# immunogenomics/cna

Measured on AMD Instinct MI355X. Metric: cells*permutations/sec end-to-end cna.tl.association, higher is better.
Workload: dtype f64

## Files before the change

cna_amd/_ffi.py:

```python
import ctypes as C
import os

_HERE = os.path.dirname(os.path.abspath(__file__))
LIB_PATH = os.path.join(_HERE, 'libcna_hip.so')

c_ctx = C.c_void_p
c_i64p = C.POINTER(C.c_int64)
c_i32p = C.POINTER(C.c_int32)
c_f64p = C.POINTER(C.c_double)
c_u8p = C.POINTER(C.c_uint8)

SIGNATURES = {
    'cna_last_error': (C.c_char_p, []),
    'cna_abi_version': (C.c_int, []),
    'cna_device_count': (C.c_int, [C.POINTER(C.c_int)]),
    'cna_ctx_create': (C.c_int, [C.c_int, C.POINTER(c_ctx)]),
    'cna_ctx_destroy': (C.c_int, [c_ctx]),
    'cna_ctx_sync': (C.c_int, [c_ctx]),
    'cna_ctx_device_bytes': (C.c_int, [c_ctx, c_i64p]),
    'cna_set_state_f32': (C.c_int, [c_ctx, C.c_int]),
    'cna_comm_unique_id': (C.c_int, [C.c_void_p]),
    'cna_comm_init': (C.c_int, [c_ctx, C.c_int, C.c_int, C.c_void_p]),
    'cna_graph_upload': (C.c_int, [c_ctx, C.c_int64, C.c_int64, C.c_int64, C.c_void_p, C.c_void_p,
                                   C.c_void_p, C.c_int]),
    'cna_comm_info': (C.c_int, [c_ctx, C.POINTER(C.c_int), C.POINTER(C.c_int)]),
    'cna_comm_selftest': (C.c_int, [c_ctx, C.c_double, C.POINTER(C.c_int)]),
    'cna_comm_init_shm': (C.c_int, [c_ctx, C.c_int, C.c_int, C.c_char_p, C.c_int64]),
    'cna_set_halo': (C.c_int, [c_ctx, C.c_void_p, C.c_void_p, C.c_void_p, C.c_void_p]),
    'cna_set_cell_order': (C.c_int, [c_ctx, C.c_void_p]),
    'cna_graph_reorder': (C.c_int, [c_ctx, C.c_void_p]),
    'cna_set_local_view': (C.c_int, [c_ctx, C.c_int]),
    'cna_colsums': (C.c_int, [c_ctx, C.c_double]),
    'cna_fetch_colsums': (C.c_int, [c_ctx, C.c_void_p]),
    'cna_set_samples': (C.c_int, [c_ctx, C.c_void_p, C.c_int, C.c_void_p]),
    'cna_restart_nam': (C.c_int, [c_ctx]),
    'cna_nam_step': (C.c_int, [c_ctx, C.c_int, C.c_int, C.c_int]),
    'cna_nam_select_hint': (C.c_int, [c_ctx, C.c_void_p, C.c_int]),
    'cna_nam_auto': (C.c_int, [c_ctx, C.c_int, C.POINTER(C.c_int), C.c_void_p]),
    'cna_nam_auto_launch': (C.c_int, [c_ctx, C.c_int]),
    'cna_nam_auto_finish': (C.c_int, [c_ctx, C.POINTER(C.c_int), C.c_void_p]),
    'cna_stat_qc': (C.c_int, [c_ctx, c_f64p, c_f64p, c_i64p]),
    'cna_fetch_cell_stat': (C.c_int, [c_ctx, C.c_void_p, C.c_int64]),
    'cna_load_cell_stat': (C.c_int, [c_ctx, C.c_void_p, C.c_int64]),
    'cna_dense_load': (C.c_int, [c_ctx, C.c_void_p, C.c_int]),
    'cna_dense_step': (C.c_int, [c_ctx]),
    'cna_dense_fetch': (C.c_int, [c_ctx, C.c_void_p]),
    'cna_batch_kurtosis': (C.c_int, [c_ctx, C.c_int, C.c_void_p, C.c_int]),
    'cna_zero_variance': (C.c_int, [c_ctx, C.c_void_p, C.c_int, C.c_void_p, c_i64p]),
    'cna_select': (C.c_int, [c_ctx, C.c_void_p, C.c_int64, C.c_void_p, C.c_int]),
    'cna_set_resid_factors': (C.c_int, [c_ctx, C.c_void_p, C.c_void_p, C.c_int, C.c_int]),
    'cna_select_checked': (C.c_int, [c_ctx, C.c_void_p, C.c_int64, C.c_void_p, C.c_int, C.POINTER(C.c_int64)]),
    'cna_select_standardized': (C.c_int, [c_ctx, C.c_void_p, C.c_int64, C.c_void_p, C.c_int, C.POINTER(C.c_int64),
                                          C.c_void_p, C.POINTER(C.c_double)]),
    'cna_upload_x': (C.c_int, [c_ctx, C.c_void_p, C.c_int64, C.c_int]),
    'cna_resid_apply': (C.c_int, [c_ctx, C.c_void_p, C.c_int]),
    'cna_resid_lowrank': (C.c_int, [c_ctx, C.c_void_p, C.c_void_p, C.c_int, C.c_int, C.c_int, C.c_void_p, c_f64p]),
    'cna_resid_lowrank_bk': (C.c_int, [c_ctx, C.c_void_p, C.c_void_p, C.c_int, C.c_void_p, c_f64p, C.c_void_p, C.c_int, c_f64p]),
    'cna_select_resid_bk': (C.c_int, [c_ctx, C.c_void_p, C.c_void_p, C.c_int, C.c_void_p, c_f64p, C.c_void_p, C.c_int, c_f64p,
                                      c_i64p, c_i64p, C.POINTER(C.c_int)]),
    'cna_standardize': (C.c_int, [c_ctx, C.c_int]),
    'cna_gram': (C.c_int, [c_ctx, C.c_void_p]),
    'cna_gram_launch': (C.c_int, [c_ctx]),
    'cna_gram_fetch': (C.c_int, [c_ctx, C.c_void_p]),
    'cna_project': (C.c_int, [c_ctx, C.c_void_p, C.c_int, C.c_void_p]),
    'cna_x_identity': (C.c_int, [c_ctx, C.POINTER(C.c_int)]),
    'cna_ncorrs': (C.c_int, [c_ctx, C.c_void_p, C.c_void_p, c_f64p]),
    'cna_null_local': (C.c_int, [c_ctx, C.c_void_p, C.c_int, C.c_void_p, C.c_int, C.c_void_p]),
    'cna_condition_phenotypes': (C.c_int, [c_ctx, C.c_void_p, C.c_void_p, C.c_int, C.c_int]),
    'cna_null_local_resident': (C.c_int, [c_ctx, C.c_int, C.c_int, C.c_void_p, C.c_int, C.c_void_p, C.c_void_p]),
    'cna_null_local_launch': (C.c_int, [c_ctx, C.c_int, C.c_int, C.c_void_p, C.c_int, C.c_int, C.c_void_p]),
    'cna_null_local_prepare': (C.c_int, [c_ctx, C.c_int, C.c_void_p, C.c_int, C.c_int, C.c_void_p]),
    'cna_null_local_fetch': (C.c_int, [c_ctx, C.c_void_p, C.c_void_p, C.c_void_p, C.c_void_p]),
    'cna_null_local_discard': (C.c_int, [c_ctx]),
    'cna_gram_pcs_tests': (C.c_int, [c_ctx, C.c_int, C.c_void_p, C.c_int, C.c_int, C.c_int, C.c_double, C.c_double, C.c_void_p,
                                     C.c_void_p, C.POINTER(C.c_int)]),
    'cna_host_top_eig': (C.c_int, [C.c_void_p, C.c_int, C.c_int, C.c_void_p, C.c_void_p, c_f64p, c_f64p]),
    'cna_host_eig_check': (C.c_int, [C.c_void_p, C.c_int, C.c_int, C.c_void_p, C.c_void_p, c_f64p, c_f64p]),
    'cna_null_local_i8_stats': (C.c_int, [c_ctx, C.POINTER(C.c_int), c_i64p, C.POINTER(C.c_int)]),
    'cna_percell_fdr_pinned': (C.c_int, [c_ctx, C.c_void_p, C.c_void_p, C.c_int, C.POINTER(C.c_void_p), C.POINTER(C.c_void_p)]),
    'cna_nam_steps': (C.c_int, [c_ctx, C.c_int]),
    'cna_host_legacy_randn': (C.c_int, [C.c_void_p, C.POINTER(C.c_int), C.POINTER(C.c_int), C.POINTER(C.c_double), C.c_int64, C.c_void_p]),
    'cna_knn_graph': (C.c_int, [c_ctx, C.c_void_p, C.c_int64, C.c_int, C.c_int, C.c_void_p, C.c_void_p, C.c_void_p, c_i64p]),
    'cna_host_hash64': (C.c_uint64, [C.c_void_p, C.c_int64, C.c_int]),
    'cna_host_copy': (C.c_int, [C.c_void_p, C.c_void_p, C.c_int64, C.c_int]),
    'cna_host_expand_u16': (C.c_int, [C.c_void_p, C.c_void_p, C.c_int64, C.c_void_p, C.c_int, C.c_int]),
    'cna_host_permuted_nnz': (C.c_int64, [C.c_void_p, C.c_int64, C.c_int64, C.c_void_p]),
    'cna_host_permute_rows': (C.c_int, [C.c_void_p, C.c_int64, C.c_int64, C.c_void_p, C.c_void_p, C.c_void_p, C.c_int, C.c_void_p,
                                        C.c_void_p, C.c_void_p, C.c_void_p, C.c_int]),
    'cna_host_cluster_order': (C.c_int64, [C.c_int64, C.c_void_p, C.c_void_p, C.c_int, C.c_void_p]),
    'cna_host_cluster_order_mt': (C.c_int64, [C.c_int64, C.c_void_p, C.c_void_p, C.c_int, C.c_int, C.c_void_p]),
    'cna_host_cluster_graph': (C.c_int64, [C.c_int64, C.c_void_p, C.c_void_p, C.c_void_p, C.c_int, C.c_void_p, C.c_void_p, C.c_void_p]),
    'cna_host_set_threads': (None, [C.c_int]),
    'cna_host_argsort_gather': (C.c_int, [C.c_void_p, C.c_int, C.c_int, C.c_void_p, C.c_void_p, C.c_int64, C.c_void_p]),
    'cna_host_draw_start': (C.c_int, [C.c_void_p, C.POINTER(C.c_int), C.c_void_p, C.c_int, C.c_int, C.c_int, C.c_void_p,
                                      C.c_void_p, C.c_void_p, C.c_int64, C.c_int]),
    'cna_host_draw_start_idx': (C.c_int, [C.c_void_p, C.POINTER(C.c_int), C.c_void_p, C.c_int, C.c_int, C.c_int, C.c_void_p,
                                          C.c_void_p, C.c_void_p, C.c_int64, C.c_int, C.c_void_p]),
    'cna_host_gather_rows': (C.c_int, [C.c_void_p, C.c_void_p, C.c_int, C.c_int, C.c_void_p, C.c_int64, C.c_int]),
    'cna_host_draw_wait': (C.c_int, []),
    'cna_host_draw_join': (C.c_int, []),
    'cna_host_draw_times': (None, [C.POINTER(C.c_double)]),
    'cna_assoc_begin': (C.c_int, [c_ctx, C.c_int, C.c_void_p, C.c_int]),
    'cna_assoc_begin_part': (C.c_int, [c_ctx, C.c_int, C.c_int, C.c_int, C.c_void_p, C.c_int]),
    'cna_assoc_finish': (C.c_int, [c_ctx, C.c_void_p, C.c_void_p]),
    'cna_assoc_run': (C.c_int, [c_ctx, C.c_int, C.c_void_p, C.c_int, C.c_void_p, C.c_void_p]),
    'cna_host_draw_then_condition': (C.c_int, [c_ctx, C.c_void_p, C.c_void_p, C.c_int, C.c_int, C.c_void_p]),
    'cna_global_test_launch': (C.c_int, [c_ctx, C.c_void_p, C.c_int, C.c_void_p, C.c_int, C.c_int]),
    'cna_global_test_fetch': (C.c_int, [c_ctx, C.c_void_p, C.c_void_p, C.c_void_p]),
    'cna_select_standardized_fused': (C.c_int, [c_ctx, C.c_void_p, C.c_int64, C.c_void_p, C.c_int, C.POINTER(C.c_int64), C.c_void_p, C.POINTER(C.c_double), C.c_int, C.POINTER(C.c_int), C.c_void_p, C.POINTER(C.c_int), C.POINTER(C.c_int), C.c_int, C.c_void_p, C.POINTER(C.c_int)]),
    'cna_reference_thresholds': (C.c_int, [C.c_double, C.c_int, C.c_void_p, C.c_void_p]),
    'cna_percell_coef_launch': (C.c_int, [c_ctx]),
    'cna_percell_coef_wait': (C.c_int, [c_ctx, C.POINTER(C.c_void_p)]),
    'cna_percell_fdr_copy_early': (C.c_int, [c_ctx, C.c_void_p, C.c_int64, C.c_int, C.POINTER(C.c_int)]),
    'cna_percell_fdr_copied_early': (C.c_int, [c_ctx, C.POINTER(C.c_int)]),
    'cna_fetch_rows': (C.c_int, [c_ctx, C.c_int, C.c_void_p, C.c_int64, C.c_void_p, C.c_int, C.c_void_p, C.c_int]),
    'cna_project_keep': (C.c_int, [c_ctx, C.c_void_p, C.c_int]),
    'cna_stat_median': (C.c_int, [c_ctx, C.POINTER(C.c_double)]),
    'cna_global_test': (C.c_int, [c_ctx, C.c_void_p, C.c_int, C.c_void_p, C.c_int, C.c_int, C.c_void_p, C.c_void_p,
                                  C.c_void_p]),
    'cna_obs_counts': (C.c_int, [c_ctx, C.c_void_p, C.c_void_p, C.c_int, C.c_void_p, C.c_void_p]),
    'cna_percell_fdr': (C.c_int, [c_ctx, C.c_void_p, C.c_void_p, C.c_int, C.c_void_p, C.c_void_p]),
    'cna_matrix_shape': (C.c_int, [c_ctx, C.c_int, c_i64p, C.POINTER(C.c_int)]),
    'cna_fetch_matrix': (C.c_int, [c_ctx, C.c_int, C.c_void_p, C.c_int]),
    'cna_allgather_host': (C.c_int, [c_ctx, C.c_void_p, C.c_int64, C.c_void_p, C.c_int64]),
    'cna_prof_enable': (C.c_int, [c_ctx, C.c_int]),
    'cna_prof_reset': (C.c_int, [c_ctx]),
    'cna_prof_get': (C.c_int, [c_ctx, C.c_int, c_f64p, c_i64p]),
    'cna_kernel_name': (C.c_char_p, [C.c_int]),
    'cna_expr_upload_dense': (C.c_int, [c_ctx, C.c_void_p, C.c_int64, C.c_int64, C.c_int]),
    'cna_expr_upload_sparse': (C.c_int, [c_ctx, C.c_void_p, C.c_void_p, C.c_void_p, C.c_int64, C.c_int64, C.c_int64,
                                         C.c_int, C.c_int, C.c_int]),
    'cna_expr_drop': (C.c_int, [c_ctx]),
    'cna_expr_shape': (C.c_int, [c_ctx, c_i64p, c_i64p, c_i64p, C.POINTER(C.c_int), C.POINTER(C.c_int), c_i64p]),
    'cna_gene_corr': (C.c_int, [c_ctx, C.c_void_p, C.c_int, C.c_void_p]),
    'cna_expr_to_bins': (C.c_int, [c_ctx, C.c_void_p, C.c_int, C.c_int, C.c_void_p, C.c_void_p]),
    'cna_expr_cross': (C.c_int, [c_ctx, C.c_void_p, C.c_int64, C.c_void_p, C.c_void_p, C.c_void_p, C.c_void_p,
                                 C.POINTER(C.c_int64)]),
    'cna_coef_strata': (C.c_int, [c_ctx, C.c_void_p, C.c_void_p, C.c_void_p, C.c_int64, C.c_int, C.c_int, C.c_int, C.c_double,
                                  C.c_double] + [C.c_void_p] * 10),
    'cna_gene_corr_by': (C.c_int, [c_ctx, C.c_void_p, C.c_int, C.c_void_p, C.c_int, C.c_void_p, C.c_void_p, C.c_void_p]),
    'cna_x_generation': (C.c_int, [c_ctx, C.POINTER(C.c_int64)]),
    'cna_matrix_to_bins': (C.c_int, [c_ctx, C.c_int, C.c_void_p, C.c_void_p, C.c_int, C.c_int64, C.c_int, C.c_void_p, C.c_void_p]),
    'cna_enrichment_extremes': (C.c_int, [c_ctx, C.c_void_p, C.c_int64, C.c_int64, C.c_void_p, C.c_void_p, C.c_int, C.c_int,
                                          C.c_void_p, C.c_void_p, C.c_void_p, C.c_void_p]),
    'cna_expr_cross_by': (C.c_int, [c_ctx, C.c_void_p, C.c_void_p, C.c_int64, C.c_int, C.c_int, C.c_int, C.c_void_p, C.c_void_p,
                                    C.c_void_p, C.c_void_p]),
    'cna_gram_by': (C.c_int, [c_ctx, C.c_void_p, C.c_void_p, C.c_int64, C.c_int, C.c_void_p, C.c_void_p]),
}

MAT_NAM, MAT_X, MAT_PROJ = 0, 1, 2
ASSOC_DONE, ASSOC_GENERAL, ASSOC_NEED_PCS, ASSOC_STALE = 0, 1, 2, 3
ASSOC_MAXT = 512


class AssocArgs(C.Structure):
    _fields_ = [('colmap', C.c_void_p), ('n_sel', C.c_int32), ('r', C.c_int32), ('y', C.c_void_p), ('M', C.c_void_p),
                ('resid_C', C.c_void_p), ('resid_W', C.c_void_p), ('ks', C.c_void_p), ('K', C.c_int32), ('Nnull', C.c_int32),
                ('table', C.c_void_p), ('draw_pending', C.c_int32), ('conditioned', C.c_int32), ('use_native_eig', C.c_int32),
                ('coef_first', C.c_int32), ('resid_tol', C.c_double), ('gap_tol', C.c_double), ('coef_dst', C.c_void_p),
                ('fdr_dst', C.c_void_p), ('n_dst', C.c_int64), ('copy_threads', C.c_int32), ('n_verify', C.c_int32),
                ('verify_ptr', C.c_void_p * 4), ('verify_bytes', C.c_int64 * 4), ('verify_hash', C.c_uint64 * 4),
                ('verify_threads', C.c_int32), ('reserved', C.c_int32),
                ('G', C.c_void_p), ('U', C.c_void_p), ('minp', C.c_void_p), ('r2', C.c_void_p), ('kidx', C.c_void_p)]


class AssocOut(C.Structure):
    _fields_ = [('status', C.c_int32), ('T', C.c_int32), ('eig_accepted', C.c_int32), ('null_fused', C.c_int32),
                ('coef_in_dst', C.c_int32), ('fdr_in_dst', C.c_int32), ('n_zero', C.c_int64), ('max_abs', C.c_double),
                ('coef_ptr', C.c_void_p), ('fdr_ptr', C.c_void_p), ('t_ms', C.c_double * 16),
                ('thr', C.c_double * ASSOC_MAXT), ('fdr', C.c_double * ASSOC_MAXT), ('runmin', C.c_double * ASSOC_MAXT),
                ('tail_sums', C.c_int64 * ASSOC_MAXT), ('ranks', C.c_int64 * ASSOC_MAXT), ('num_detected', C.c_int64 * ASSOC_MAXT)]

KERNELS = ['colsum', 'nam_first', 'nam_step', 'batch_kurtosis', 'zero_variance', 'select', 'resid_xb',
           'standardize', 'gram', 'gram_reduce', 'ncorrs', 'null_local', 'obs_counts', 'percell_fdr',
           'project_xb', 'transpose', 'rccl', 'condition', 'global_test', 'nam_step_sparse', 'halo_exchange', 'halo_wait',
           'matrix_bins_sort', 'matrix_bins_sum', 'enrich_positions', 'enrich_extremes', 'expr_cross_by', 'gram_by']

_lib = None


class CnaHipError(RuntimeError):
    """A libcna_hip.so entry point returned a non-zero status."""


def load():
    global _lib
    if _lib is not None:
        return _lib
    if not os.path.exists(LIB_PATH):
        raise CnaHipError(
            'libcna_hip.so is not built (%s).  cna_amd has no CPU path; build the HIP library with '
            '`python -c "import __graft_entry__ as g; g.build()"` or `make -C cna_amd/csrc`.' % LIB_PATH)
    lib = C.CDLL(LIB_PATH)
    for name, (res, args) in SIGNATURES.items():
        fn = getattr(lib, name)
        fn.restype = res
        fn.argtypes = args
    _lib = lib
    return lib


def check(status, what):
    if status != 0:
        msg = load().cna_last_error()
        raise CnaHipError('%s failed (status %d): %s' % (what, status, msg.decode() if msg else '?'))


def ptr(a):
    return None if a is None else a.ctypes.data_as(C.c_void_p)
```

cna_amd/csrc/c_api.hip:

```cpp
#include "common.h"
#include <sched.h>
#include <chrono>
#include <cmath>
#include <cstring>

int comm_destroy(cna_ctx* c);

static thread_local std::string g_err;
void cna_set_error(const std::string& msg) { g_err = msg; }

int dev_alloc(cna_ctx* c, void** p, size_t bytes) {
  std::lock_guard<std::recursive_mutex> lk(c->alloc_mu);
  *p = nullptr;
  if (bytes == 0) bytes = 256;
  hipError_t e = hipMalloc(p, bytes);
  if (e != hipSuccess) {
    cna_set_error(std::string("hipMalloc(") + std::to_string(bytes) + "): " + hipGetErrorString(e));
    return CNA_ENOMEM;
  }
  c->dev_bytes += (int64_t)bytes;
  return 0;
}
int dev_free(cna_ctx* c, void* p, size_t bytes) {
  std::lock_guard<std::recursive_mutex> lk(c->alloc_mu);
  if (p) {
    (void)hipFree(p);
    c->dev_bytes -= (int64_t)(bytes ? bytes : 256);
  }
  return 0;
}
static void halo_clear(cna_ctx* c);

int dev_reserve(cna_ctx* c, void** p, int64_t* cap, int64_t need) {
  std::lock_guard<std::recursive_mutex> lk(c->alloc_mu);
  if (need <= *cap && *p) return 0;
  if (*p) {
    HIP_TRY(hipStreamSynchronize(c->stream));
    dev_free(c, *p, (size_t)*cap);
    *p = nullptr;
    *cap = 0;
  }
  if (need < 256) need = 256;
  CNA_TRY(dev_alloc(c, p, (size_t)need));
  *cap = need;
  return 0;
}

static hipEvent_t ev_get(cna_ctx* c) {
  if (!c->ev_pool.empty()) {
    hipEvent_t e = c->ev_pool.back();
    c->ev_pool.pop_back();
    return e;
  }
  hipEvent_t e;
  (void)hipEventCreate(&e);
  return e;
}
void prof_begin(cna_ctx* c, int kid, hipStream_t st) {
  std::lock_guard<std::mutex> lock(c->prof_mu);
  ProfSpan s;
  s.kid = kid;
  s.a = ev_get(c);
  s.b = ev_get(c);
  (void)hipEventRecord(s.a, st);
  c->prof_pending.push_back(s);
}
void prof_end(cna_ctx* c, int kid, hipStream_t st) {
  std::lock_guard<std::mutex> lock(c->prof_mu);
  for (size_t i = c->prof_pending.size(); i-- > 0;) {
    if (c->prof_pending[i].kid == kid) {
      (void)hipEventRecord(c->prof_pending[i].b, st);
      return;
    }
  }
}
static void prof_flush(cna_ctx* c) {
  (void)hipStreamSynchronize(c->stream);
  (void)hipStreamSynchronize(c->copy_stream);
  if (c->coef_stream) (void)hipStreamSynchronize(c->coef_stream);
  if (c->gram_stream) (void)hipStreamSynchronize(c->gram_stream);
  if (c->halo_stream) (void)hipStreamSynchronize(c->halo_stream);
  std::lock_guard<std::mutex> lock(c->prof_mu);
  if (c->prof_pending.empty()) return;
  for (auto& s : c->prof_pending) {
    float ms = 0.f;
    if (hipEventElapsedTime(&ms, s.a, s.b) == hipSuccess) {
      c->prof_ms[s.kid] += ms;
      c->prof_n[s.kid] += 1;
    }
    c->ev_pool.push_back(s.a);
    c->ev_pool.push_back(s.b);
  }
  c->prof_pending.clear();
}

static const char* kKernelNames[CNA_K_COUNT] = {
    "colsum", "nam_first", "nam_step", "batch_kurtosis", "zero_variance", "select", "resid_xb",
    "standardize", "gram", "gram_reduce", "ncorrs", "null_local", "obs_counts", "percell_fdr",
    "project_xb", "transpose", "rccl", "condition", "global_test", "nam_step_sparse", "halo_exchange", "halo_wait",
    "matrix_bins_sort", "matrix_bins_sum", "enrich_positions", "enrich_extremes", "expr_cross_by", "gram_by"};

#define AUTO_FINISH(c)                                                   \
  do {                                                                   \
    if ((c)->auto_pending) CNA_TRY(cna_nam_auto_finish((c), nullptr, nullptr)); \
  } while (0)

static void void_x(cna_ctx* c) {
  c->x_valid = c->x_from_nam = c->x_ident = false;
  c->ncorrs_valid = c->xq_valid = c->byp_valid = c->gram_pre = c->proj_valid = false;
  c->gram_n = 0;
  c->cells.coef_early = false;
  c->cells.fdr_inline = false;
  c->x_gen = c->x_gen + 1;
}
static void void_walk(cna_ctx* c) {
  c->t_valid = c->nam_valid = c->nam_lazy = false;
  c->steps_done = 0;
  c->t_f32[0] = c->t_f32[1] = false;
  void_x(c);
}
static void void_cells(cna_ctx* c) {
  c->cellinfo_valid = false;
  void_walk(c);
}

static int x_begin(cna_ctx* c, const char* who) {
  NO_NULL_PENDING(c, who);
  void_x(c);
  return 0;
}
int x_ld(int Nx) {
  int ld = round_up(Nx, 4);
  if (ld > 128 && (ld * 8) % 256 == 0 && ld + 4 <= 256) ld += 4;
  return ld;
}
static int x_begin(cna_ctx* c, const char* who, int64_t nx, int Nx, const int64_t* keep_idx) {
  CNA_TRY(x_begin(c, who));
  c->nx = nx;
  c->Nx = Nx;
  c->ldx = x_ld(Nx);
  void* xp = c->X;
  CNA_TRY(dev_reserve(c, &xp, &c->x_cap, (int64_t)sizeof(double) * std::max<int64_t>(nx, 1) * c->ldx));
  c->X = (double*)xp;
  c->keep_idx = nullptr;
  if (keep_idx) {
    void* kp = c->keep_store;
    CNA_TRY(dev_reserve(c, &kp, &c->keep_cap, 8 * std::max<int64_t>(nx, 1)));
    c->keep_store = (int64_t*)kp;
    HIP_TRY(hipMemcpyAsync(c->keep_store, keep_idx, 8 * nx, hipMemcpyHostToDevice, c->stream));
    c->keep_idx = c->keep_store;
  }
  return 0;
}
static void x_commit(cna_ctx* c, bool from_nam, bool ncorrs, bool xq, bool ident) {
  c->x_valid = true;
  c->x_from_nam = from_nam;
  c->ncorrs_valid = ncorrs;
  c->xq_valid = xq;
  c->x_ident = ident;
}


static int ragged_gather(cna_ctx* c, const double* src_dev, int64_t count_local, double* out, int64_t n_expected) {
  NO_NULL_PENDING(c, "cna_fetch_cell_stat / cna_allgather_host");
  CNA_TRY(dev_reserve(c, &c->scratch, &c->scratch_cap, 256 * 2 + 8 * c->nranks));
  int64_t* cnt_dev = (int64_t*)c->scratch;
  std::vector<int64_t> cnt(c->nranks, 0);
  cnt[c->rank] = count_local;
  HIP_TRY(hipMemcpyAsync(cnt_dev, cnt.data(), 8 * c->nranks, hipMemcpyHostToDevice, c->stream));
  CNA_TRY(comm_allreduce_i64_sum(c, cnt_dev, c->nranks));
  HIP_TRY(hipMemcpyAsync(cnt.data(), cnt_dev, 8 * c->nranks, hipMemcpyDeviceToHost, c->stream));
  HIP_TRY(hipStreamSynchronize(c->stream));
  int64_t mx = 1, tot = 0;
  for (auto v : cnt) { mx = std::max(mx, v); tot += v; }
  if (tot != n_expected) CNA_FAIL(CNA_EINVAL, "ragged gather: expected total does not match the ranks' counts");
  CNA_TRY(dev_reserve(c, &c->scratch2, &c->scratch2_cap, 8 * mx * c->nranks));
  double* all = (double*)c->scratch2;
  if (count_local > 0)
    HIP_TRY(hipMemcpyAsync(all + mx * c->rank, src_dev, 8 * count_local, hipMemcpyDeviceToDevice, c->stream));
  CNA_TRY(comm_allgather_bytes(c, all + mx * c->rank, all, 8 * mx));
  std::vector<double> host(mx * c->nranks);
  HIP_TRY(hipMemcpyAsync(host.data(), all, 8 * mx * c->nranks, hipMemcpyDeviceToHost, c->stream));
  HIP_TRY(hipStreamSynchronize(c->stream));
  int64_t o = 0;
  for (int r = 0; r < c->nranks; ++r) {
    std::memcpy(out + o, host.data() + mx * r, 8 * cnt[r]);
    o += cnt[r];
  }
  return 0;
}

int halo_settle(cna_ctx* c) {
  if (!c->halo_wait_pending) return 0;
  c->halo_wait_pending = false;
  ProfScope ps(c, CNA_K_HALO_WAIT);
  HIP_TRY(hipStreamWaitEvent(c->stream, c->halo_e2, 0));
  return 0;
}

extern "C" {

const char* cna_last_error(void) { return g_err.c_str(); }
int cna_abi_version(void) { return 1; }
const char* cna_kernel_name(int k) { return (k >= 0 && k < CNA_K_COUNT) ? kKernelNames[k] : "?"; }

int cna_device_count(int* count) {
  int n = 0;
  hipError_t e = hipGetDeviceCount(&n);
  if (e != hipSuccess) {
    *count = 0;
    cna_set_error(std::string("hipGetDeviceCount: ") + hipGetErrorString(e));
    return (int)e;
  }
  *count = n;
  return 0;
}

int cna_ctx_create(int device, cna_ctx** out) {
  if (!out) CNA_FAIL(CNA_EINVAL, "null out pointer");
  *out = nullptr;
  int n = 0;
  CNA_TRY(cna_device_count(&n));
  if (n <= 0) CNA_FAIL(CNA_EINVAL, "no HIP device visible: cna_amd has no CPU fallback");
  if (device < 0 || device >= n) CNA_FAIL(CNA_EINVAL, "device index out of range");
  HIP_TRY(hipSetDevice(device));
  cna_ctx* c = new cna_ctx();
  c->device = device;
  hipError_t e = hipStreamCreateWithFlags(&c->stream, hipStreamNonBlocking);
  if (e == hipSuccess) {
    int lo = 0, hi = 0;
    (void)hipDeviceGetStreamPriorityRange(&lo, &hi);
    e = hipStreamCreateWithPriority(&c->copy_stream, hipStreamNonBlocking, hi);
    if (e == hipSuccess) e = hipStreamCreateWithFlags(&c->coef_stream, hipStreamNonBlocking);
  }
  if (e == hipSuccess) e = hipEventCreateWithFlags(&c->gram_done, hipEventDisableTiming);
  if (e == hipSuccess) e = hipEventCreateWithFlags(&c->cells.coef_ready, hipEventDisableTiming);
  if (e == hipSuccess) e = hipEventCreateWithFlags(&c->gt_done, hipEventDisableTiming);
  if (e == hipSuccess) e = hipEventCreateWithFlags(&c->scal_ready, hipEventDisableTiming);
  if (e == hipSuccess) e = hipEventCreateWithFlags(&c->stage_done, hipEventDisableTiming);
  if (e == hipSuccess) e = hipEventCreateWithFlags(&c->cells.coef_copied, hipEventDisableTiming);
  if (e == hipSuccess) e = hipEventCreateWithFlags(&c->null_done, hipEventDisableTiming);
  if (e == hipSuccess) e = hipEventCreateWithFlags(&c->cells.bins_copied, hipEventDisableTiming);
  if (e != hipSuccess) {
    delete c;
    cna_set_error(std::string("hipStreamCreate: ") + hipGetErrorString(e));
    return (int)e;
  }
  *out = c;
  return 0;
}

int cna_ctx_destroy(cna_ctx* c) {
  if (!c) return 0;
  (void)hipSetDevice(c->device);
  (void)hipStreamSynchronize(c->stream);
  if (c->gram_stream) (void)hipStreamSynchronize(c->gram_stream);
  if (c->auto_state) { (void)hipFree(c->auto_state); c->auto_state = nullptr; }
  if (c->byp_buf) { (void)hipFree(c->byp_buf); c->byp_buf = nullptr; }
  if (c->pair_buf) { (void)hipFree(c->pair_buf); c->pair_buf = nullptr; }
  prof_flush(c);
  comm_destroy(c);
  expr_destroy(c);
  void* bufs[] = {c->halo_rows_safe, c->halo_rows_need, c->idx_t, c->i8_buf, c->xq, c->xq_scale, c->cells.coef_dev, c->proj, c->sp_pair, c->sp_cnt, c->null_part, c->rp16_buf, c->halo_send_idx, c->halo_recv_idx, c->halo_rows_b, c->halo_rows_i, c->halo_sbuf, c->halo_rbuf, c->orig_idx, c->indptr, c->indices, c->data, c->colsum, c->sid, c->counts, c->T[0], c->T[1], c->dense_s,
                  c->nam, c->X, c->X2, c->resid_f, c->keep_store, c->stat, c->ncorrs, c->scratch, c->scratch2, c->cellinfo, c->zc, c->gt, c->gram_tiles_ptr, c->gram_buf, c->gram_part, c->cells.bins_dev};
  for (void* b : bufs)
    if (b) (void)hipFree(b);
  for (auto e : c->ev_pool) (void)hipEventDestroy(e);
  (void)hipStreamDestroy(c->stream);
  if (c->copy_stream) (void)hipStreamDestroy(c->copy_stream);
  if (c->coef_stream) (void)hipStreamDestroy(c->coef_stream);
  if (c->gram_done) (void)hipEventDestroy(c->gram_done);
  if (c->gt_done) (void)hipEventDestroy(c->gt_done);
  if (c->scal_ready) (void)hipEventDestroy(c->scal_ready);
  if (c->stage_done) (void)hipEventDestroy(c->stage_done);
  if (c->h_gt) (void)hipHostFree(c->h_gt);
  if (c->null_done) (void)hipEventDestroy(c->null_done);
  if (c->gram_stream) (void)hipStreamDestroy(c->gram_stream);
  for (hipEvent_t e : {c->gram_pre_done, c->range_done, c->cells.coef_ready, c->cells.coef_copied, c->cells.bins_copied})
    if (e) (void)hipEventDestroy(e);
  if (c->halo_stream) (void)hipStreamDestroy(c->halo_stream);
  if (c->halo_e1) (void)hipEventDestroy(c->halo_e1);
  if (c->halo_e2) (void)hipEventDestroy(c->halo_e2);
  if (c->cells.h_bins) (void)hipHostFree(c->cells.h_bins);
  if (c->cells.h_tab) (void)hipHostFree(c->cells.h_tab);
  if (c->h_res) (void)hipHostFree(c->h_res);
  if (c->h_scal) (void)hipHostFree(c->h_scal);
  if (c->h_gram) (void)hipHostFree(c->h_gram);
  if (c->h_hint) (void)hipHostFree(c->h_hint);
  if (c->cells.h_cell) (void)hipHostFree(c->cells.h_cell);
  delete c;
  return 0;
}

int cna_ctx_sync(cna_ctx* c) {
  CHECK_CTX(c);
  AUTO_FINISH(c);
  CNA_TRY(halo_settle(c));
  HIP_TRY(hipStreamSynchronize(c->stream));
  if (c->gram_stream && c->gram_pre_pending) HIP_TRY(hipStreamSynchronize(c->gram_stream));
  return 0;
}

int cna_ctx_device_bytes(cna_ctx* c, int64_t* bytes) {
  if (!c || !bytes) CNA_FAIL(CNA_EINVAL, "null argument");
  *bytes = c->dev_bytes.load();
  return 0;
}

int cna_x_generation(cna_ctx* c, int64_t* gen) {
  if (!c || !gen) CNA_FAIL(CNA_EINVAL, "null argument");
  *gen = c->x_gen;
  return 0;
}

int cna_set_state_f32(cna_ctx* c, int on) {
  CHECK_CTX(c);
  c->state_f32_mode = on != 0;
  return 0;
}

int cna_graph_upload(cna_ctx* c, int64_t n_global, int64_t row0, int64_t n_local, const int64_t* indptr,
                     const int32_t* indices, const void* data, int data_is_f64) {
  CHECK_CTX(c);
  AUTO_FINISH(c);
  if (n_global <= 0 || n_local < 0 || row0 < 0 || row0 + n_local > n_global || !indptr)
    CNA_FAIL(CNA_EINVAL, "cna_graph_upload: bad shape");
  const int64_t rpr = (n_global + c->nranks - 1) / c->nranks;
  if (row0 != (int64_t)c->rank * rpr && !(n_local == 0))
    CNA_FAIL(CNA_EINVAL, "cna_graph_upload: row0 must be rank*ceil(n/nranks)");
  const int64_t want_local = std::max<int64_t>(0, std::min(rpr, n_global - (int64_t)c->rank * rpr));
  if (n_local != want_local) CNA_FAIL(CNA_EINVAL, "cna_graph_upload: n_local must be the rank's block size");
  if (indptr[0] != 0) CNA_FAIL(CNA_EINVAL, "cna_graph_upload: indptr must be rebased to start at 0");
  const int64_t nnz = indptr[n_local];
  HIP_TRY(hipStreamSynchronize(c->stream));
  void_cells(c);
  if (c->indptr) dev_free(c, c->indptr, sizeof(int64_t) * (c->n_local + 1));
  if (c->indices) dev_free(c, c->indices, sizeof(int32_t) * c->nnz);
  if (c->data) dev_free(c, c->data, (c->data_f64 ? 8 : 4) * c->nnz);
  if (c->colsum) dev_free(c, c->colsum, sizeof(double) * c->n_pad);
  if (c->stat) dev_free(c, c->stat, sizeof(double) * c->n_pad);
  if (c->orig_idx) dev_free(c, c->orig_idx, sizeof(int64_t) * c->n_local);
  c->indptr = nullptr; c->indices = nullptr; c->data = nullptr; c->colsum = nullptr; c->stat = nullptr;
  c->orig_idx = nullptr;
  halo_clear(c);
  c->n_global = n_global;
  c->row0 = (int64_t)c->rank * rpr;
  c->n_local = n_local;
  c->rows_per_rank = rpr;
  c->n_pad = rpr * c->nranks;
  c->nnz = nnz;
  c->data_f64 = data_is_f64 ? 1 : 0;
  const size_t vb = data_is_f64 ? 8 : 4;
  CNA_TRY(dev_alloc(c, (void**)&c->indptr, sizeof(int64_t) * (n_local + 1)));
  CNA_TRY(dev_alloc(c, (void**)&c->indices, sizeof(int32_t) * nnz));
  CNA_TRY(dev_alloc(c, (void**)&c->data, vb * nnz));
  CNA_TRY(dev_alloc(c, (void**)&c->colsum, sizeof(double) * c->n_pad));
  CNA_TRY(dev_alloc(c, (void**)&c->stat, sizeof(double) * c->n_pad));
  HIP_TRY(hipMemcpy(c->indptr, indptr, sizeof(int64_t) * (n_local + 1), hipMemcpyHostToDevice));
  if (nnz > 0) {
    HIP_TRY(hipMemcpy(c->indices, indices, sizeof(int32_t) * nnz, hipMemcpyHostToDevice));
    HIP_TRY(hipMemcpy(c->data, data, vb * nnz, hipMemcpyHostToDevice));
  }
  HIP_TRY(hipMemset(c->stat, 0, sizeof(double) * c->n_pad));
  c->have_colsum = false;
  return 0;
}

int cna_set_cell_order(cna_ctx* c, const int64_t* orig_index) {
  CHECK_CTX(c);
  if (!c->indptr) CNA_FAIL(CNA_ESTATE, "cna_set_cell_order before cna_graph_upload");
  HIP_TRY(hipStreamSynchronize(c->stream));
  if (!orig_index) {
    if (c->orig_idx) dev_free(c, c->orig_idx, sizeof(int64_t) * c->n_local);
    c->orig_idx = nullptr;
    return 0;
  }
  const int64_t lim = c->local_view ? c->n_local : c->n_global;
  for (int64_t i = 0; i < c->n_local; ++i)
    if (orig_index[i] < 0 || orig_index[i] >= lim)
      CNA_FAIL(CNA_EINVAL, "cna_set_cell_order: index out of range");
  if (!c->orig_idx && c->n_local > 0) CNA_TRY(dev_alloc(c, (void**)&c->orig_idx, sizeof(int64_t) * c->n_local));
  if (c->n_local > 0)
    HIP_TRY(hipMemcpy(c->orig_idx, orig_index, sizeof(int64_t) * c->n_local, hipMemcpyHostToDevice));
  return 0;
}

int cna_graph_reorder(cna_ctx* c, const int64_t* perm) {
  CHECK_CTX(c);
  AUTO_FINISH(c);
  if (!c->indptr || !perm) CNA_FAIL(CNA_ESTATE, "cna_graph_reorder before cna_graph_upload");
  if (c->nranks != 1 || c->halo_on || c->local_view || c->n_local != c->n_global || c->n_pad != c->n_global)
    CNA_FAIL(CNA_ESTATE, "cna_graph_reorder: one rank holding the whole graph only");
  if (c->orig_idx) CNA_FAIL(CNA_ESTATE, "cna_graph_reorder: the resident graph already has a device cell order");
  CNA_TRY(halo_settle(c));
  HIP_TRY(hipStreamSynchronize(c->stream));
  if (c->gram_stream && c->gram_pre_pending) HIP_TRY(hipStreamSynchronize(c->gram_stream));
  const int64_t n = c->n_global;
  int64_t* pd = nullptr;
  CNA_TRY(dev_alloc(c, (void**)&pd, sizeof(int64_t) * n));
  hipError_t e = hipMemcpyAsync(pd, perm, sizeof(int64_t) * n, hipMemcpyHostToDevice, c->stream);
  int rc = e == hipSuccess ? graph_reorder_device(c, pd) : (int)e;
  if (rc) {
    (void)hipStreamSynchronize(c->stream);
    dev_free(c, pd, sizeof(int64_t) * n);
    if (e != hipSuccess) cna_set_error(hipGetErrorString(e));
    return rc;
  }
  c->orig_idx = pd;
  HIP_TRY(hipMemsetAsync(c->stat, 0, sizeof(double) * c->n_pad, c->stream));
  void_cells(c);
  return 0;
}

int cna_set_local_view(cna_ctx* c, int on) {
  CHECK_CTX(c);
  HIP_TRY(hipStreamSynchronize(c->stream));
  if ((on != 0) != c->local_view) {
    void_x(c);
    if (c->orig_idx) dev_free(c, c->orig_idx, sizeof(int64_t) * c->n_local);
    c->orig_idx = nullptr;
  }
  c->local_view = on != 0;
  return 0;
}

int cna_colsums(cna_ctx* c, double self_weight) {
  CHECK_CTX(c);
  if (!c->indptr) CNA_FAIL(CNA_ESTATE, "cna_colsums before cna_graph_upload");
  c->self_weight = self_weight;
  CNA_TRY(launch_colsum(c));
  CNA_TRY(comm_allreduce_f64_sum(c, c->colsum, (size_t)c->n_pad));
  CNA_TRY(launch_add_scalar(c, c->colsum, c->n_global, self_weight));
  c->have_colsum = true;
  c->cellinfo_valid = false;
  return 0;
}

int cna_fetch_colsums(cna_ctx* c, double* out) {
  CHECK_CTX(c);
  if (!c->have_colsum) CNA_FAIL(CNA_ESTATE, "colsums not computed");
  HIP_TRY(hipMemcpyAsync(out, c->colsum, sizeof(double) * c->n_global, hipMemcpyDeviceToHost, c->stream));
  HIP_TRY(hipStreamSynchronize(c->stream));
  return 0;
}

static int64_t state_rows(const cna_ctx* c) { return c->t_compact ? c->t_rows : c->n_pad; }

static int ensure_T(cna_ctx* c, int ld) {
  const int64_t need = (int64_t)sizeof(double) * (state_rows(c) * ld + 64);
  if (need > c->t_cap || !c->T[0] || (c->t_compact && c->t_cap > need + need / 2 + (1 << 20))) {
    HIP_TRY(hipStreamSynchronize(c->stream));
    if (c->halo_wait_pending && c->halo_stream) { HIP_TRY(hipStreamSynchronize(c->halo_stream)); c->halo_wait_pending = false; }
    for (int i = 0; i < 2; ++i) {
      if (c->T[i]) dev_free(c, c->T[i], (size_t)c->t_cap);
      c->T[i] = nullptr;
    }
    for (int i = 0; i < 2; ++i) {
      CNA_TRY(dev_alloc(c, (void**)&c->T[i], (size_t)need));
      HIP_TRY(hipMemsetAsync(c->T[i], 0, (size_t)need, c->stream));
    }
    c->t_cap = need;
  }
  return 0;
}

static int ensure_sparse_state(cna_ctx* c) {
  int min_n = 96;
  if (const char* e = getenv("CNA_SPARSE_MIN_N")) min_n = atoi(e);
  const bool multi = c->nranks > 1 || comm_active(c);
  const bool want = min_n > 0 && c->N >= min_n && (!multi || c->halo_on);
  if (!want) {
    if (c->sp_cnt) {
      HIP_TRY(hipStreamSynchronize(c->stream));
      dev_free(c, c->sp_pair, 16 * 64 * (size_t)c->sp_pair_rows);
      dev_free(c, c->sp_cnt, (size_t)c->sp_rows);
      c->sp_pair = c->sp_cnt = nullptr;
      c->sp_rows = c->sp_pair_rows = 0;
    }
    return 0;
  }
  const int64_t cnt_rows = state_rows(c), pair_rows = c->t_compact ? std::max<int64_t>(c->n_local, 1) : c->n_pad;
  if (c->sp_cnt && c->sp_rows == cnt_rows && c->sp_pair_rows == pair_rows) return 0;
  if (c->sp_cnt) {
    HIP_TRY(hipStreamSynchronize(c->stream));
    dev_free(c, c->sp_pair, 16 * 64 * (size_t)c->sp_pair_rows);
    dev_free(c, c->sp_cnt, (size_t)c->sp_rows);
    c->sp_pair = c->sp_cnt = nullptr;
  }
  c->sp_rows = cnt_rows;
  c->sp_pair_rows = pair_rows;
  CNA_TRY(dev_alloc(c, &c->sp_pair, 16 * 64 * (size_t)c->sp_pair_rows));
  CNA_TRY(dev_alloc(c, &c->sp_cnt, (size_t)c->sp_rows));
  HIP_TRY(hipMemsetAsync(c->sp_cnt, 0xff, (size_t)c->sp_rows, c->stream));
  return 0;
}

int cna_set_samples(cna_ctx* c, const int32_t* codes, int n_samples, const double* counts) {
  CHECK_CTX(c);
  AUTO_FINISH(c);
  if (!c->indptr) CNA_FAIL(CNA_ESTATE, "cna_set_samples before cna_graph_upload");
  if (n_samples < 1 || n_samples > 1024) CNA_FAIL(CNA_EINVAL, "n_samples must be in [1, 1024]");
  HIP_TRY(hipStreamSynchronize(c->stream));
  if (!c->sid || !c->counts || c->N != n_samples || c->sid_n != c->n_global) {
    if (c->sid) dev_free(c, c->sid, sizeof(int32_t) * c->sid_n);
    if (c->counts) dev_free(c, c->counts, sizeof(double) * c->N);
    c->sid = nullptr; c->counts = nullptr;
    CNA_TRY(dev_alloc(c, (void**)&c->sid, sizeof(int32_t) * c->n_global));
    CNA_TRY(dev_alloc(c, (void**)&c->counts, sizeof(double) * n_samples));
    c->sid_n = c->n_global;
  }
  c->N = n_samples;
  int ld_align = 4;
  c->ld = round_up(n_samples, ld_align);
  HIP_TRY(hipMemcpyAsync(c->sid, codes, sizeof(int32_t) * c->n_global, hipMemcpyHostToDevice, c->stream));
  HIP_TRY(hipMemcpyAsync(c->counts, counts, sizeof(double) * n_samples, hipMemcpyHostToDevice, c->stream));
  HIP_TRY(hipStreamSynchronize(c->stream));
  void_cells(c);
  CNA_TRY(ensure_T(c, c->ld));
  void* nm = c->nam;
  CNA_TRY(dev_reserve(c, &nm, &c->nam_cap, (int64_t)sizeof(double) * std::max<int64_t>(c->n_local, 1) * c->ld));
  c->nam = (double*)nm;
  c->t_width = c->N;
  c->t_ld = c->ld;
  c->t_cur = 0;
  CNA_TRY(ensure_sparse_state(c));
  return 0;
}

int cna_restart_nam(cna_ctx* c) {
  CHECK_CTX(c);
  AUTO_FINISH(c);
  if (!c->sid || !c->counts) CNA_FAIL(CNA_ESTATE, "cna_restart_nam needs cna_set_samples first");
  void_walk(c);
  CNA_TRY(ensure_T(c, c->ld));
  c->t_width = c->N;
  c->t_ld = c->ld;
  c->t_cur = 0;
  return 0;
}

static void halo_clear(cna_ctx* c) {
  if (c->halo_wait_pending && c->halo_stream) (void)hipStreamSynchronize(c->halo_stream);
  c->halo_wait_pending = false;
  if (c->halo_rows_safe) dev_free(c, c->halo_rows_safe, sizeof(int32_t) * std::max<int64_t>(c->halo_nsafe, 1));
  if (c->halo_rows_need) dev_free(c, c->halo_rows_need, sizeof(int32_t) * std::max<int64_t>(c->halo_nneed, 1));
  c->halo_rows_safe = c->halo_rows_need = nullptr;
  c->halo_nsafe = c->halo_nneed = 0;
  if (c->idx_t) dev_free(c, c->idx_t, sizeof(int32_t) * std::max<int64_t>(c->idx_t_n, 1));
  c->idx_t = nullptr;
  c->idx_t_n = 0;
  if (c->t_compact) {
    c->t_compact = false;
    c->t_rows = 0;
    void_cells(c);
  }
  if (c->halo_send_idx) dev_free(c, c->halo_send_idx, sizeof(int64_t) * std::max<int64_t>(c->halo_ns, 1));
  if (c->halo_recv_idx) dev_free(c, c->halo_recv_idx, sizeof(int64_t) * std::max<int64_t>(c->halo_nr, 1));
  c->halo_send_idx = c->halo_recv_idx = nullptr;
  c->halo_ns = c->halo_nr = 0;
  c->halo_on = false;
  if (c->halo_rows_b) dev_free(c, c->halo_rows_b, sizeof(int32_t) * std::max<int64_t>(c->halo_nb, 1));
  if (c->halo_rows_i) dev_free(c, c->halo_rows_i, sizeof(int32_t) * std::max<int64_t>(c->halo_ni, 1));
  c->halo_rows_b = c->halo_rows_i = nullptr;
  c->halo_nb = c->halo_ni = 0;
}

int cna_set_halo(cna_ctx* c, const int64_t* send_rows, const int64_t* send_counts, const int64_t* recv_rows,
                 const int64_t* recv_counts) {
  CHECK_CTX(c);
  if (!c->indptr) CNA_FAIL(CNA_ESTATE, "cna_set_halo before cna_graph_upload");
  HIP_TRY(hipStreamSynchronize(c->stream));
  halo_clear(c);
  if (!send_counts || !recv_counts) return 0;
  if (!comm_active(c)) CNA_FAIL(CNA_ESTATE, "cna_set_halo needs cna_comm_init");
  int64_t ns = 0, nr = 0;
  for (int p = 0; p < c->nranks; ++p) {
    if (send_counts[p] < 0 || recv_counts[p] < 0) CNA_FAIL(CNA_EINVAL, "cna_set_halo: negative count");
    ns += send_counts[p];
    nr += recv_counts[p];
  }
  if ((ns > 0 && !send_rows) || (nr > 0 && !recv_rows)) CNA_FAIL(CNA_EINVAL, "cna_set_halo: missing row list");
  for (int64_t k = 0; k < ns; ++k)
    if (send_rows[k] < 0 || send_rows[k] >= c->n_local) CNA_FAIL(CNA_EINVAL, "cna_set_halo: send row outside the local block");
  for (int64_t k = 0; k < nr; ++k)
    if (recv_rows[k] < 0 || recv_rows[k] >= c->n_global) CNA_FAIL(CNA_EINVAL, "cna_set_halo: recv row out of range");
  CNA_TRY(dev_alloc(c, (void**)&c->halo_send_idx, sizeof(int64_t) * std::max<int64_t>(ns, 1)));
  c->halo_ns = ns;
// ... 1404 lines not shown
```

cna_amd/csrc/common.h:

```cpp
#pragma once
#include <hip/hip_runtime.h>
#include <stdint.h>
#include <string>
#include <mutex>
#include <atomic>
#include <vector>
#include "../../include/cna_hip.h"

#define WAVE 64
#define I8_QMAX 8355000.0

void cna_set_error(const std::string& msg);

#define HIP_TRY(expr)                                                                      \
  do {                                                                                     \
    hipError_t _e = (expr);                                                                \
    if (_e != hipSuccess) {                                                                \
      cna_set_error(std::string(#expr) + ": " + hipGetErrorString(_e) + " (" + __FILE__ +  \
                    ":" + std::to_string(__LINE__) + ")");                               \
      return (int)_e;                                                                      \
    }                                                                                      \
  } while (0)

#define CNA_TRY(expr)            \
  do {                           \
    int _r = (expr);             \
    if (_r != 0) return _r;      \
  } while (0)

#define CNA_FAIL(code, msg)      \
  do {                           \
    cna_set_error(msg);          \
    return (code);               \
  } while (0)

static inline int round_up(int x, int m) { return (x + m - 1) / m * m; }
static inline int64_t round_up64(int64_t x, int64_t m) { return (x + m - 1) / m * m; }

struct ProfSpan {
  int kid;
  hipEvent_t a, b;
};

struct GramPlan {
  int Nx = 0, nt = 0, ntri = 0, ldp = 0, slab_rows = 32, nblocks = 1, nw = 16;
  bool use_blk = false;
  int64_t nslab = 0;
  int32_t* tiles_dev = nullptr;
  double* partial = nullptr;
  size_t smem = 0;
};

struct NullCarve {
  double *cuts, *obs_edges, *obs_thr;
  unsigned long long *hist, *obs_hist;
  int64_t *tails, *sums, *obs_tails;
};
struct NullHostLayout { int64_t sums = 0, tails = 0, obs = 0, stage = 0, status = 0, bytes = 0; };
enum NullPhase : int { NULL_IDLE = 0, NULL_PREPARED, NULL_PENDING };
struct NullPass {
  int P = 0, T = 0, col0 = 0, has_tails = 0, has_obs = 0;
  double cut0 = 0, inv_step = 0, eps = 0;
  double thr0 = 0, thr_step = 0;
  bool i8_last = false;
  NullHostLayout host;
  std::atomic<int> phase{NULL_IDLE};
  std::atomic<int64_t> status_off{-1};
};
struct CellColumns {
  std::atomic<bool> coef_early{false};
  std::atomic<bool> fdr_inline{false};
  std::atomic<bool> fdr_early_copied{false};
  std::atomic<bool> fdr_early_served{false};
  std::atomic<int> fdr_early_inflight{0};
  double* fdr_early_dst = nullptr;
  double* coef_dev = nullptr;
  unsigned short* bins_dev = nullptr;
  unsigned short* h_bins = nullptr;
  bool bins_pending = false;
  double* h_tab = nullptr;
  void* h_cell = nullptr;
  int64_t coef_dev_cap = 0, bins_cap = 0, h_bins_cap = 0, h_cell_cap = 0;
  hipEvent_t coef_ready = nullptr, coef_copied = nullptr, bins_copied = nullptr;
};

struct cna_ctx {
  int device = 0;
  hipStream_t stream = nullptr;
  hipStream_t copy_stream = nullptr;
  hipStream_t coef_stream = nullptr;
  hipEvent_t gram_done = nullptr;
  hipEvent_t scal_ready = nullptr;
  double* gram_buf = nullptr;
  hipEvent_t null_done = nullptr;
  void* h_hint = nullptr;
  void* h_gram = nullptr;
  int64_t h_gram_cap = 0;
  double* gram_mirror = nullptr;
  bool gram_mirrored = false;
  double t_gram_fetched = 0.0;
  void* h_scal = nullptr;
  void* h_res = nullptr;
  int64_t h_res_cap = 0;
  NullPass null;
  CellColumns cells;
  int64_t gram_cap = 0;
  int gram_n = 0;
  std::atomic<int64_t> dev_bytes{0};
  std::recursive_mutex alloc_mu;

  int rank = 0, nranks = 1;
  void* comm = nullptr;
  void* comm_halo = nullptr;
  void* shm = nullptr;
  bool halo_on = false;
  int64_t* halo_send_idx = nullptr;
  int64_t* halo_recv_idx = nullptr;
  std::vector<int64_t> halo_send_cnt, halo_recv_cnt;
  int64_t halo_ns = 0, halo_nr = 0;
  int32_t* halo_rows_b = nullptr;
  int32_t* halo_rows_i = nullptr;
  int64_t halo_nb = 0, halo_ni = 0;
  hipStream_t halo_stream = nullptr;
  hipEvent_t halo_e1 = nullptr, halo_e2 = nullptr;
  void* halo_sbuf = nullptr;
  void* halo_rbuf = nullptr;
  int64_t halo_sbuf_cap = 0, halo_rbuf_cap = 0;

  int64_t n_global = 0, row0 = 0, n_local = 0, rows_per_rank = 0, n_pad = 0, nnz = 0;
  int64_t* indptr = nullptr;
  int32_t* indices = nullptr;
  void* data = nullptr;
  int data_f64 = 0;
  double self_weight = 1.0;
  double* colsum = nullptr;
  int64_t* orig_idx = nullptr;
  bool local_view = false;
  bool have_colsum = false;

  int N = 0, ld = 0;
  int32_t* sid = nullptr;
  int64_t sid_n = 0;
  double* counts = nullptr;
  void* cellinfo = nullptr;
  int64_t cellinfo_cap = 0;
  bool cellinfo_valid = false;

  bool t_compact = false;
  int64_t t_rows = 0;
  int32_t* idx_t = nullptr;
  int64_t idx_t_n = 0;
  int32_t* halo_rows_safe = nullptr;
  int32_t* halo_rows_need = nullptr;
  int64_t halo_nsafe = 0, halo_nneed = 0;
  bool halo_wait_pending = false;
  bool halo_safe_launch = false;
  bool sp_dense_interior_off = false;
  int64_t sp_pair_rows = 0;
  double* T[2] = {nullptr, nullptr};
  int64_t t_cap = 0;
  int t_cur = 0, t_width = 0, t_ld = 0, steps_done = 0;
  bool t_valid = false;
  bool state_f32_mode = false;
  bool t_f32[2] = {false, false};
  double* dense_s = nullptr;
  int64_t dense_cap = 0;

  double* nam = nullptr;
  int64_t nam_cap = 0;
  bool nam_valid = false;

  double* X = nullptr;
  int64_t x_cap = 0;
  double* resid_f = nullptr;
  int64_t resid_f_cap = 0;
  int resid_rk = 0, resid_n = 0;
  double* X2 = nullptr;
  int64_t x2_cap = 0;
  int64_t nx = 0;
  int Nx = 0, ldx = 0;
  int64_t* keep_idx = nullptr;
  int64_t* keep_store = nullptr;
  int64_t keep_cap = 0;
  bool x_valid = false, x_from_nam = false;
  int64_t x_gen = 0;
  bool x_ident = false;
  std::vector<double> byp_hint;
  std::vector<double> byp_y;
  bool byp_valid = false;
  bool byp_with_q = false;
  bool byp_skip_nam = false;
  bool nam_lazy = false;
  int lazy_steps_before = 0;
  bool byp_arm = false;
  void* pair_buf = nullptr;
  void* byp_buf = nullptr;

  double* stat = nullptr;
  int stat_space = -1;
  void* auto_state = nullptr;
  const int* auto_stop = nullptr;
  bool auto_pending = false;
  int auto_max = 0, auto_queued = 0;
  double* ncorrs = nullptr;
  int64_t ncorrs_cap = 0;
  bool ncorrs_valid = false;

  double* zc = nullptr;
  int64_t zc_cap = 0;
  int zc_ld = 0, zc_cols = 0, zc_rows = 0;
  void* gt = nullptr;
  int64_t gt_cap = 0;

  void* scratch = nullptr;
  int64_t scratch_cap = 0;
  void* proj = nullptr;
  int64_t proj_cap = 0, proj_rows = 0;
  int proj_ld = 0, proj_cols = 0;
  bool proj_valid = false;
  void* h_gt = nullptr;
  int64_t h_gt_cap = 0;
  hipEvent_t gt_done = nullptr;
  hipEvent_t stage_done = nullptr;
  int gt_pending_P = 0;
  int64_t gt_off_out = 0;
  void* sp_pair = nullptr;
  void* sp_cnt = nullptr;
  int64_t sp_rows = 0;
  void* i8_buf = nullptr;
  int64_t i8_cap = 0;
  void* xq = nullptr;
  int64_t xq_cap = 0;
  void* xq_scale = nullptr;
  int64_t xq_scale_cap = 0;
  bool xq_valid = false;
  int64_t xq_rows = 0;
  int xq_KS = 0;
  unsigned long long* i8_qcount = nullptr;
  void* null_part = nullptr;
  int64_t null_part_cap = 0;
  void* rp16_buf = nullptr;
  int64_t rp16_cap = 0;
  void* scratch2 = nullptr;
  int64_t scratch2_cap = 0;
  hipStream_t gram_stream = nullptr;
  int gram_stream_state = 0;
  hipEvent_t gram_pre_done = nullptr, range_done = nullptr;
  bool gram_pre = false;
  bool gram_pre_pending = false;
  void* gram_part = nullptr;
  int64_t gram_part_cap = 0;
  GramPlan gram_pre_plan;
  int gram_tiles_nt = -1;
  void* gram_tiles_ptr = nullptr;
  int64_t gram_tiles_cap = 0;

  void* expr = nullptr;

  bool prof = false;
  uint64_t prof_mask = ~0ull;
  double prof_ms[CNA_K_COUNT] = {0};
  int64_t prof_n[CNA_K_COUNT] = {0};
  std::vector<ProfSpan> prof_pending;
  std::vector<hipEvent_t> ev_pool;
  std::mutex prof_mu;
};

void prof_begin(cna_ctx* c, int kid, hipStream_t st);
void prof_end(cna_ctx* c, int kid, hipStream_t st);
struct ProfScope {
  cna_ctx* c;
  int kid;
  hipStream_t st;
  ProfScope(cna_ctx* c_, int k, hipStream_t s = nullptr) : c(c_), kid(k), st(s ? s : c_->stream) {
    if (c->prof && kid >= 0 && (c->prof_mask >> kid & 1)) prof_begin(c, kid, st);
  }
  ~ProfScope() { if (c->prof && kid >= 0 && (c->prof_mask >> kid & 1)) prof_end(c, kid, st); }
};

int dev_alloc(cna_ctx* c, void** p, size_t bytes);
int dev_free(cna_ctx* c, void* p, size_t bytes);
int dev_reserve(cna_ctx* c, void** p, int64_t* cap_bytes, int64_t need_bytes);

#define CHECK_CTX(c)                                        \
  do {                                                      \
    if (!(c)) CNA_FAIL(CNA_EINVAL, "null context");         \
    HIP_TRY(hipSetDevice((c)->device));                     \
  } while (0)

#define NO_NULL_PENDING(c, who)                                                                      \
  do {                                                                                               \
    if ((c)->null.phase == NULL_PENDING)                                                             \
      CNA_FAIL(CNA_ESTATE, std::string(who) + ": a local-null pass is still pending: fetch it first"); \
  } while (0)

struct Carver {
  char* base;
  int64_t off = 0;
  explicit Carver(void* p) : base((char*)p) {}
  template <typename T>
  T* take(int64_t count) {
    T* r = (T*)(base + off);
    off += round_up64((int64_t)sizeof(T) * count, 256);
    return r;
  }
};
inline int64_t carve_bytes(std::initializer_list<int64_t> sizes) {
  int64_t t = 0;
  for (auto s : sizes) t += round_up64(s, 256);
  return t;
}

int x_ld(int Nx);
int null_local_prepare(cna_ctx* c, int P, const double* edges, int T, int want_tails, const double* thr);
int null_local_go(cna_ctx* c, int col0);

void expr_destroy(cna_ctx* c);

inline bool comm_active(const cna_ctx* c) { return c->comm != nullptr || c->shm != nullptr; }
int comm_halo_exchange(cna_ctx* c, const double* sendbuf, double* recvbuf, int64_t doubles_per_row, hipStream_t st = nullptr);
int halo_settle(cna_ctx* c);
int launch_rows_need_halo(cna_ctx* c, unsigned char* flags_dev);
int launch_remap_indices(cna_ctx* c, const int64_t* recv_rows_dev, int64_t nr, int32_t* out, int* bad);
int launch_pack_rows(cna_ctx* c, const double* src, const int64_t* idx, int64_t nrows, int ld, double* dst, hipStream_t st = nullptr);
int launch_unpack_rows(cna_ctx* c, const double* src, const int64_t* idx, int64_t nrows, int ld, double* dst, hipStream_t st = nullptr);
int comm_allreduce_f64_sum(cna_ctx* c, double* buf, size_t count);
int comm_allreduce_f64_max(cna_ctx* c, double* buf, size_t count);
int comm_allreduce_i64_sum(cna_ctx* c, int64_t* buf, size_t count);
int comm_allgather_bytes(cna_ctx* c, const void* send, void* recv, size_t bytes_per_rank);

int launch_colsum(cna_ctx* c);
int graph_reorder_device(cna_ctx* c, const int64_t* perm_dev);
int launch_add_scalar(cna_ctx* c, double* v, int64_t n, double s);
int launch_nam_step(cna_ctx* c, bool first, bool want_kurt, bool write_t, bool write_nam, bool dense,
                    const int32_t* rows = nullptr, int64_t n_rows = 0,
                    int64_t base = 0, int64_t count = -1,
                    hipStream_t st = nullptr, bool timed = true);
int64_t nam_step_turn_rows(const cna_ctx* c, int64_t n_rows);
int launch_scale_rows(cna_ctx* c, const double* s_local, double* t_global, int m, int ld);
int launch_batch_kurtosis(cna_ctx* c, const double* mat, int64_t rows, int ncols, int ld,
                          const int32_t* order_dev, const int32_t* boff_dev, int n_batches, double* out);
int launch_zero_variance(cna_ctx* c, const int32_t* colmap_dev, int n_sel, uint8_t* flags_dev,
                         unsigned long long* count_dev);
int launch_select(cna_ctx* c, const int32_t* colmap_dev);
int launch_select_zv(cna_ctx* c, const int32_t* colmap_dev, unsigned long long* count_dev);
int launch_gather_rows(cna_ctx* c, const double* src, int ld, const int64_t* rows_dev, int64_t n_out,
                       const int32_t* cols_dev, int n_cols, double* dst, int transposed);
int launch_digit_hist(cna_ctx* c, const double* v, int64_t n, unsigned long long prefix, int shift,
                      unsigned long long* hist_dev);
int launch_max_fold(cna_ctx* c, const unsigned long long* blockmax, int nblocks, unsigned long long* out);
int launch_pair_pack(cna_ctx* c, const unsigned long long* cnt, const unsigned long long* maxbits, unsigned long long* slot);
int launch_pair_fold(cna_ctx* c, const unsigned long long* slots, int nranks, unsigned long long* cnt, unsigned long long* maxbits);
int launch_auto_median(cna_ctx* c, const double* v, int64_t n, void* state, unsigned long long* hist, int step, int min_steps,
                       bool sum_over_ranks = false);
int launch_qc_count(cna_ctx* c, const double* v, int64_t n, void* state);
int auto_state_result_offset();
size_t auto_state_bytes();
int auto_state_stopped_offset();
int launch_select_std(cna_ctx* c, const int32_t* colmap_dev, unsigned long long* nzero_dev, const double* y_dev,
                      unsigned long long* maxbits_dev, const double* W_dev, const double* Ct_dev, int rk,
                      unsigned char* xq = nullptr, void* xscale = nullptr, int Kp = 0);
int launch_standardize(cna_ctx* c, int center);
int launch_ncorrs(cna_ctx* c, const double* y_dev, unsigned long long* maxbits_dev);
int launch_resid_lowrank(cna_ctx* c, const double* W_dev, const double* Ct_dev, int r, int center, int standardize,
                         const double* y_dev, unsigned long long* maxbits_dev, const int32_t* bk_order = nullptr,
                         const int32_t* bk_boff = nullptr, int nb = 0, double* bk_out = nullptr);
int launch_obs_counts(cna_ctx* c, const double* edges_dev, const double* thr_dev, int T, double thr0,
                      double inv_step, unsigned long long* hist_dev );
int launch_suffix_sum(cna_ctx* c, const unsigned long long* hist, int P, int T, int64_t* tails);
int launch_tail_sums(cna_ctx* c, const int64_t* tails, int P, int T, int64_t* sums);
int launch_fdr_table(cna_ctx* c, const int64_t* sums, const int64_t* ranks, int T, int P, double* fdr, double* runmin);
int launch_rowpass16(cna_ctx* c, const double* src, int lds, double* dst, int ldd, int64_t nrows, int N, const double* W_dev,
                     const double* Ct_dev, int r, int center, int standardize, int write_out, const double* y_dev,
                     unsigned long long* maxword, const int32_t* bk_order, const int32_t* bk_boff, int nb, double* bk_out,
                     unsigned long long* qc_counters = nullptr);
int launch_percell_bins(cna_ctx* c, hipStream_t st, const double* coef_local, const double* thr_dev, int T, double thr0,
                        double inv_step, unsigned short* bins);
extern "C" int cna_host_expand_u16(double* dst, const uint16_t* bins, int64_t n, const double* runmin, int T, int nthreads);
int launch_unpermute2(cna_ctx* c, const double* a, const double* b, const int64_t* idx, int64_t n, double* oa,
                      double* ob);
int launch_percell_fdr(cna_ctx* c, const double* thr_dev, const double* runmin_dev, int T, double thr0,
                       double inv_step, double* coef_local, double* fdr_local);
int launch_transpose(cna_ctx* c, const double* in, int64_t rows, int cols, int ld, double* out);
int launch_xb(cna_ctx* c, const double* B_dev, int ldb, int n_out, bool center, double* out, int ld_out);
int launch_gram(cna_ctx* c, double* G_dev);
int launch_copy_f64(cna_ctx* c, const double* src, double* dst, int64_t n);
int gram_pre_begin(cna_ctx* c, int64_t* unit_rows);
int gram_pre_range(cna_ctx* c, int64_t row0, int64_t row1, hipStream_t st);
int gram_pre_finish(cna_ctx* c, double* G_dev, hipStream_t st);
bool gram_fused_ok(const cna_ctx* c, int Nx, int ldx, int Kp);
int launch_selgram(cna_ctx* c, double* G_dev, unsigned long long* nzero, const double* y, unsigned long long* maxbits,
                   unsigned char* xq, void* xscale, int Kp);
int launch_null_local(cna_ctx* c, const double* Yc_dev, int ldy, int P, const double* cuts_dev, int T,
                      double cut0, double inv_step, double eps, unsigned long long* hist_dev, const int* guard = nullptr);
bool null_i8_eligible(const cna_ctx* c, int P, int T, double cut0, double inv_step, double eps);
bool null_i8_enabled();
int ensure_xq(cna_ctx* c, int KS);
int launch_null_local_i8(cna_ctx* c, const double* Yc_dev, int ldy, int P, const double* cuts_dev, int T, double cut0,
                         double inv_step, double eps, int64_t** sums_out, int** status_out);

int launch_condition(cna_ctx* c, hipStream_t st, const double* M_dev, const double* Y_dev, int N, int P,
                     double* Zc_dev, int ldy);
int64_t global_test_scratch_doubles(int P, int kmax, int K);
int launch_global_test(cna_ctx* c, hipStream_t st, const double* Zc_dev, int ldy, int N, int P, const double* U_dev,
                       int kmax, const int32_t* ks_dev, int K, int r, double* work, double* minp_dev, double* r2_dev,
                       int32_t* kidx_dev);

#ifdef __HIPCC__
__device__ __forceinline__ double dpp_add(double v, const int ctrl_sel) {
  int lo = __double2loint(v), hi = __double2hiint(v);
  int lo2, hi2;
  switch (ctrl_sel) {
    case 0: lo2 = __builtin_amdgcn_update_dpp(0, lo, 0xB1, 0xF, 0xF, true); hi2 = __builtin_amdgcn_update_dpp(0, hi, 0xB1, 0xF, 0xF, true); break;
    case 1: lo2 = __builtin_amdgcn_update_dpp(0, lo, 0x4E, 0xF, 0xF, true); hi2 = __builtin_amdgcn_update_dpp(0, hi, 0x4E, 0xF, 0xF, true); break;
    case 2: lo2 = __builtin_amdgcn_update_dpp(0, lo, 0x141, 0xF, 0xF, true); hi2 = __builtin_amdgcn_update_dpp(0, hi, 0x141, 0xF, 0xF, true); break;
    default: lo2 = __builtin_amdgcn_update_dpp(0, lo, 0x140, 0xF, 0xF, true); hi2 = __builtin_amdgcn_update_dpp(0, hi, 0x140, 0xF, 0xF, true); break;
  }
  return v + __hiloint2double(hi2, lo2);
}
__device__ __forceinline__ double dpp_partner(double v, const int ctrl_sel) {
  int lo = __double2loint(v), hi = __double2hiint(v);
  int lo2, hi2;
  switch (ctrl_sel) {
    case 0: lo2 = __builtin_amdgcn_update_dpp(0, lo, 0xB1, 0xF, 0xF, true); hi2 = __builtin_amdgcn_update_dpp(0, hi, 0xB1, 0xF, 0xF, true); break;
    case 1: lo2 = __builtin_amdgcn_update_dpp(0, lo, 0x4E, 0xF, 0xF, true); hi2 = __builtin_amdgcn_update_dpp(0, hi, 0x4E, 0xF, 0xF, true); break;
    case 2: lo2 = __builtin_amdgcn_update_dpp(0, lo, 0x141, 0xF, 0xF, true); hi2 = __builtin_amdgcn_update_dpp(0, hi, 0x141, 0xF, 0xF, true); break;
    default: lo2 = __builtin_amdgcn_update_dpp(0, lo, 0x140, 0xF, 0xF, true); hi2 = __builtin_amdgcn_update_dpp(0, hi, 0x140, 0xF, 0xF, true); break;
  }
  return __hiloint2double(hi2, lo2);
}
__device__ __forceinline__ double wave_max_d(double v) {
  v = fmax(v, dpp_partner(v, 0));
  v = fmax(v, dpp_partner(v, 1));
  v = fmax(v, dpp_partner(v, 2));
  v = fmax(v, dpp_partner(v, 3));
  const int lo = __double2loint(v), hi = __double2hiint(v);
  const double r0 = __hiloint2double(__builtin_amdgcn_readlane(hi, 0), __builtin_amdgcn_readlane(lo, 0));
  const double r1 = __hiloint2double(__builtin_amdgcn_readlane(hi, 16), __builtin_amdgcn_readlane(lo, 16));
  const double r2 = __hiloint2double(__builtin_amdgcn_readlane(hi, 32), __builtin_amdgcn_readlane(lo, 32));
  const double r3 = __hiloint2double(__builtin_amdgcn_readlane(hi, 48), __builtin_amdgcn_readlane(lo, 48));
  return fmax(fmax(r0, r1), fmax(r2, r3));
}
__device__ __forceinline__ double wave_sum(double v) {
  v = dpp_add(v, 0);
  v = dpp_add(v, 1);
  v = dpp_add(v, 2);
  v = dpp_add(v, 3);
  const int lo = __double2loint(v), hi = __double2hiint(v);
  const double r0 = __hiloint2double(__builtin_amdgcn_readlane(hi, 0), __builtin_amdgcn_readlane(lo, 0));
  const double r1 = __hiloint2double(__builtin_amdgcn_readlane(hi, 16), __builtin_amdgcn_readlane(lo, 16));
  const double r2 = __hiloint2double(__builtin_amdgcn_readlane(hi, 32), __builtin_amdgcn_readlane(lo, 32));
  const double r3 = __hiloint2double(__builtin_amdgcn_readlane(hi, 48), __builtin_amdgcn_readlane(lo, 48));
  return (r0 + r1) + (r2 + r3);
}
__device__ __forceinline__ double row16_sum(double v) {
  v = dpp_add(v, 0);
  v = dpp_add(v, 1);
  v = dpp_add(v, 2);
  return dpp_add(v, 3);
}
__device__ __forceinline__ double row16_max(double v) {
  v = fmax(v, dpp_partner(v, 0));
  v = fmax(v, dpp_partner(v, 1));
  v = fmax(v, dpp_partner(v, 2));
  return fmax(v, dpp_partner(v, 3));
}
__device__ __forceinline__ int64_t uniform64(int64_t v) {
  int lo = __builtin_amdgcn_readfirstlane((int)(v & 0xffffffffll));
  int hi = __builtin_amdgcn_readfirstlane((int)(v >> 32));
  return ((int64_t)hi << 32) | (uint32_t)lo;
}
__device__ __forceinline__ void digits3(int q, unsigned& d0, unsigned& d1, unsigned& d2) {
  const int q1 = (q + 128) >> 8;
  d0 = (unsigned)q & 255u;
  d1 = (unsigned)q1 & 255u;
  d2 = (unsigned)((q1 + 128) >> 8) & 255u;
}
#endif
```

cna_amd/csrc/host_graph.c:

```c
#include <pthread.h>
#include <sched.h>
#include <stdint.h>
#include <stdlib.h>
#include <string.h>

#define P1 0x9E3779B185EBCA87ull
#define P2 0xC2B2AE3D27D4EB4Full
#define P3 0x165667B19E3779F9ull

static inline uint64_t rotl(uint64_t x, int r) { return (x << r) | (x >> (64 - r)); }
static inline uint64_t mixin(uint64_t acc, uint64_t w) { return rotl(acc + w * P2, 31) * P1; }
static inline uint64_t fin(uint64_t h) {
  h ^= h >> 33; h *= P2; h ^= h >> 29; h *= P3; h ^= h >> 32;
  return h;
}

static uint64_t hash_chunk(const unsigned char* p, size_t n, uint64_t seed) {
  uint64_t a = seed + P1, b = seed ^ P2, c = seed + P3, d = seed - P1;
  size_t i = 0;
  for (; i + 32 <= n; i += 32) {
    uint64_t w[4];
    memcpy(w, p + i, 32);
    a = mixin(a, w[0]); b = mixin(b, w[1]); c = mixin(c, w[2]); d = mixin(d, w[3]);
  }
  uint64_t h = rotl(a, 1) + rotl(b, 7) + rotl(c, 12) + rotl(d, 18) + (uint64_t)n;
  for (; i + 8 <= n; i += 8) {
    uint64_t w;
    memcpy(&w, p + i, 8);
    h = mixin(h, w);
  }
  for (; i < n; ++i) h = mixin(h, (uint64_t)p[i] + 0x100);
  return fin(h);
}

#define HASH_CHUNK ((size_t)1 << 20)

struct hash_job {
  const unsigned char* p;
  size_t n, nchunks;
  uint64_t* out;
  int tid, nthreads;
};

static void* hash_worker(void* arg) {
  struct hash_job* j = (struct hash_job*)arg;
  for (size_t c = (size_t)j->tid; c < j->nchunks; c += (size_t)j->nthreads) {
    const size_t off = c * HASH_CHUNK;
    const size_t len = j->n - off < HASH_CHUNK ? j->n - off : HASH_CHUNK;
    j->out[c] = hash_chunk(j->p + off, len, (uint64_t)c);
  }
  return NULL;
}

uint64_t cna_host_hash64(const void* p, int64_t nbytes, int nthreads) {
  if (nbytes <= 0 || !p) return fin(P3);
  const size_t n = (size_t)nbytes;
  const size_t nchunks = (n + HASH_CHUNK - 1) / HASH_CHUNK;
  uint64_t* dig = (uint64_t*)malloc(8 * nchunks);
  if (!dig) return 0;
  if (nthreads > 64) nthreads = 64;
  if ((size_t)nthreads > nchunks) nthreads = (int)nchunks;
  if (nthreads < 1) nthreads = 1;
  struct hash_job jobs[64];
  pthread_t th[64];
  int started[64];
  for (int t = 0; t < nthreads; ++t) {
    jobs[t].p = (const unsigned char*)p; jobs[t].n = n; jobs[t].nchunks = nchunks; jobs[t].out = dig;
    jobs[t].tid = t; jobs[t].nthreads = nthreads;
    started[t] = 0;
  }
  for (int t = 1; t < nthreads; ++t) started[t] = pthread_create(&th[t], NULL, hash_worker, &jobs[t]) == 0;
  hash_worker(&jobs[0]);
  for (int t = 1; t < nthreads; ++t) {
    if (started[t]) pthread_join(th[t], NULL);
    else hash_worker(&jobs[t]);
  }
  uint64_t h = P1 ^ (uint64_t)n;
  for (size_t c = 0; c < nchunks; ++c) h = mixin(h, dig[c]);
  free(dig);
  return fin(h);
}

struct copy_job { char* d; const char* s; size_t n; };
static void* copy_worker(void* a) {
  struct copy_job* j = (struct copy_job*)a;
  memcpy(j->d, j->s, j->n);
  return NULL;
}
int cna_host_copy(void* dst, const void* src, int64_t nbytes, int nthreads) {
  if (nbytes <= 0) return 0;
  if (!dst || !src) return 1;
  if (nthreads > 16) nthreads = 16;
  if ((int64_t)nthreads > nbytes / (1 << 20)) nthreads = (int)(nbytes / (1 << 20));
  if (nthreads < 1) nthreads = 1;
  struct copy_job jobs[16];
  pthread_t th[16];
  int started[16];
  const size_t part = (((size_t)nbytes / nthreads) + 63) & ~(size_t)63;
  for (int t = 0; t < nthreads; ++t) {
    const size_t b = (size_t)t * part;
    jobs[t].d = (char*)dst + b; jobs[t].s = (const char*)src + b;
    jobs[t].n = b >= (size_t)nbytes ? 0 : ((size_t)nbytes - b < part || t == nthreads - 1 ? (size_t)nbytes - b : part);
    started[t] = 0;
  }
  for (int t = 1; t < nthreads; ++t) started[t] = pthread_create(&th[t], NULL, copy_worker, &jobs[t]) == 0;
  copy_worker(&jobs[0]);
  for (int t = 1; t < nthreads; ++t) {
    if (started[t]) pthread_join(th[t], NULL);
    else copy_worker(&jobs[t]);
  }
  return 0;
}

struct expand_job { double* d; const uint16_t* b; size_t n; const double* tab; int T; };
#ifndef CNA_NO_CLONES
__attribute__((target_clones("avx2", "default")))
#endif
static void expand_span(double* d, const uint16_t* b, size_t n, const double* t2) {
  for (size_t i = 0; i < n; ++i) d[i] = t2[b[i] & 1023u];
}
static void* expand_worker(void* a) {
  struct expand_job* j = (struct expand_job*)a;
  expand_span(j->d, j->b, j->n, j->tab);
  return NULL;
}
int cna_host_expand_u16(double* dst, const uint16_t* bins, int64_t n, const double* runmin, int T, int nthreads) {
  if (n <= 0) return 0;
  if (!dst || !bins || !runmin) return 1;
  if (nthreads > 16) nthreads = 16;
  if ((int64_t)nthreads > n / (1 << 17)) nthreads = (int)(n / (1 << 17));
  if (nthreads < 1) nthreads = 1;
  struct expand_job jobs[16];
  pthread_t th[16];
  int started[16];
  double t2[1024];
  for (int h = 0; h < 1024; ++h) t2[h] = (h > 0 && h <= T && h <= 512) ? runmin[h - 1] : 1.0;
  const size_t part = (((size_t)n / nthreads) + 63) & ~(size_t)63;
  for (int t = 0; t < nthreads; ++t) {
    const size_t b = (size_t)t * part;
    jobs[t].d = dst + b; jobs[t].b = bins + b; jobs[t].tab = t2; jobs[t].T = T;
    jobs[t].n = b >= (size_t)n ? 0 : ((size_t)n - b < part || t == nthreads - 1 ? (size_t)n - b : part);
    started[t] = 0;
  }
  for (int t = 1; t < nthreads; ++t) started[t] = pthread_create(&th[t], NULL, expand_worker, &jobs[t]) == 0;
  expand_worker(&jobs[0]);
  for (int t = 1; t < nthreads; ++t) {
    if (started[t]) pthread_join(th[t], NULL);
    else expand_worker(&jobs[t]);
  }
  return 0;
}

int64_t cna_host_cluster_order(int64_t n, const int64_t* indptr, const int32_t* indices, int B, int64_t* order_out) {
  if (n <= 0) return 0;
  if (B < 1) B = 1;
  int32_t* state = (int32_t*)calloc((size_t)n, 4);
  int32_t* touched = (int32_t*)malloc(4 * (size_t)n);
  int32_t* fifo = (int32_t*)malloc(4 * (size_t)n);
  unsigned char* queued = (unsigned char*)calloc((size_t)n, 1);
  int64_t* shorts = (int64_t*)malloc(8 * (size_t)n);
  int32_t* members = (int32_t*)malloc(4 * (size_t)B);
  int32_t** level = (int32_t**)calloc((size_t)B + 2, sizeof(int32_t*));
  int64_t* lsize = (int64_t*)calloc((size_t)B + 2, 8);
  int64_t* lcap = (int64_t*)calloc((size_t)B + 2, 8);
  int64_t n_full = 0, n_short = 0, fifo_head = 0, fifo_tail = 0, next_index = 0;
  int64_t rc = -1;
  if (!state || !touched || !fifo || !queued || !shorts || !members || !level || !lsize || !lcap) goto done;
  for (;;) {
    int64_t seed = -1;
    while (fifo_head < fifo_tail) {
      const int32_t c = fifo[fifo_head++];
      if (state[c] >= 0) { seed = c; break; }
    }
    if (seed < 0) {
      while (next_index < n && state[next_index] < 0) ++next_index;
      if (next_index >= n) break;
      seed = next_index;
    }
    int m = 0, top = 0;
    int64_t ntouched = 0;
    int32_t cur = (int32_t)seed;
    for (;;) {
      if (state[cur] == 0) touched[ntouched++] = cur;
      state[cur] = -1;
      members[m++] = cur;
      if (m == B) break;
      for (int64_t e = indptr[cur]; e < indptr[cur + 1]; ++e) {
        const int32_t j = indices[e];
        if (j < 0 || j >= n) continue;
        const int32_t sj = state[j];
        if (sj < 0) continue;
        if (sj == 0) touched[ntouched++] = j;
        state[j] = sj + 1;
        const int c = sj + 1 > B + 1 ? B + 1 : sj + 1;
        if (lsize[c] == lcap[c]) {
          lcap[c] = lcap[c] ? 2 * lcap[c] : 256;
          int32_t* grown = (int32_t*)realloc(level[c], 4 * (size_t)lcap[c]);
          if (!grown) goto done;
          level[c] = grown;
        }
        level[c][lsize[c]++] = j;
        if (c > top) top = c;
      }
      int32_t pick = -1;
      while (top > 0) {
        if (lsize[top] == 0) { --top; continue; }
        const int32_t j = level[top][--lsize[top]];
        const int32_t sj = state[j];
        if (sj >= 0 && (sj > B + 1 ? B + 1 : sj) == top) { pick = j; break; }
      }
      if (pick < 0) break;
      cur = pick;
    }
    for (int c = 0; c <= B + 1; ++c) lsize[c] = 0;
    for (int64_t t = 0; t < ntouched; ++t) {
      const int32_t j = touched[t];
      if (state[j] >= 0) {
        state[j] = 0;
        if (!queued[j]) { queued[j] = 1; fifo[fifo_tail++] = j; }
      }
    }
    if (m == B) {
      for (int i = 0; i < m; ++i) order_out[n_full + i] = members[i];
      n_full += m;
    } else {
      for (int i = 0; i < m; ++i) shorts[n_short + i] = members[i];
      n_short += m;
    }
  }
  for (int64_t i = 0; i < n_short; ++i) order_out[n_full + i] = shorts[i];
  rc = n_full;
done:
  if (level) for (int c = 0; c <= B + 1; ++c) free(level[c]);
  free(level); free(lsize); free(lcap); free(state); free(touched); free(fifo); free(queued);
  free(shorts); free(members);
  return rc;
}

struct co_shared {
  int64_t n; const int64_t* indptr; const int32_t* indices; int B, P, nthreads;
  int32_t* region; int32_t* cand;
  int32_t* frontier; int64_t nfront;
  int32_t** next; int64_t* nnext; int64_t* capnext;
  pthread_barrier_t bar;
  int64_t* rstart; int32_t* members;
  int32_t* state; unsigned char* queued;
  int64_t* out_full; int64_t* n_full; int64_t* out_short; int64_t* n_short;
  volatile int failed; volatile int64_t next_region;
  int gate;
};
struct co_job { struct co_shared* sh; int tid; };

static int co_grow(struct co_shared* sh, int p) {
  const int B = sh->B;
  const int64_t r0 = sh->rstart[p], cnt = sh->rstart[p + 1] - r0;
  if (cnt == 0) { sh->n_full[p] = sh->n_short[p] = 0; return 0; }
  const int32_t* mem = sh->members + r0;
  int32_t* state = sh->state;
  const int32_t* region = sh->region;
  int32_t* touched = (int32_t*)malloc(4 * (size_t)cnt);
  int32_t* fifo = (int32_t*)malloc(4 * (size_t)cnt);
  int32_t* cl = (int32_t*)malloc(4 * (size_t)B);
  int32_t** level = (int32_t**)calloc((size_t)B + 2, sizeof(int32_t*));
  int64_t* lsize = (int64_t*)calloc((size_t)B + 2, 8);
  int64_t* lcap = (int64_t*)calloc((size_t)B + 2, 8);
  int64_t* full = sh->out_full + r0;
  int64_t* shorts = sh->out_short + r0;
  int64_t n_full = 0, n_short = 0, fifo_head = 0, fifo_tail = 0, next_i = 0;
  int rc = -1;
  if (!touched || !fifo || !cl || !level || !lsize || !lcap) goto done;
  for (;;) {
    int64_t seed = -1;
    while (fifo_head < fifo_tail) {
      const int32_t c = fifo[fifo_head++];
      if (state[c] >= 0) { seed = c; break; }
    }
    if (seed < 0) {
      while (next_i < cnt && state[mem[next_i]] < 0) ++next_i;
      if (next_i >= cnt) break;
      seed = mem[next_i];
    }
    int m = 0, top = 0;
    int64_t ntouched = 0;
    int32_t cur = (int32_t)seed;
    for (;;) {
      if (state[cur] == 0) touched[ntouched++] = cur;
      state[cur] = -1;
      cl[m++] = cur;
      if (m == B) break;
      for (int64_t e = sh->indptr[cur]; e < sh->indptr[cur + 1]; ++e) {
        const int32_t j = sh->indices[e];
        if (j < 0 || j >= sh->n || region[j] != p) continue;
        const int32_t sj = state[j];
        if (sj < 0) continue;
        if (sj == 0) touched[ntouched++] = j;
        state[j] = sj + 1;
        const int c = sj + 1 > B + 1 ? B + 1 : sj + 1;
        if (lsize[c] == lcap[c]) {
          lcap[c] = lcap[c] ? 2 * lcap[c] : 256;
          int32_t* grown = (int32_t*)realloc(level[c], 4 * (size_t)lcap[c]);
          if (!grown) goto done;
          level[c] = grown;
        }
        level[c][lsize[c]++] = j;
        if (c > top) top = c;
      }
      int32_t pick = -1;
      while (top > 0) {
        if (lsize[top] == 0) { --top; continue; }
        const int32_t j = level[top][--lsize[top]];
        const int32_t sj = state[j];
        if (sj >= 0 && (sj > B + 1 ? B + 1 : sj) == top) { pick = j; break; }
      }
      if (pick < 0) break;
      cur = pick;
    }
    for (int c = 0; c <= B + 1; ++c) lsize[c] = 0;
    for (int64_t t = 0; t < ntouched; ++t) {
      const int32_t j = touched[t];
      if (state[j] >= 0) {
        state[j] = 0;
        if (!sh->queued[j]) { sh->queued[j] = 1; fifo[fifo_tail++] = j; }
      }
    }
    if (m == B) { for (int i = 0; i < m; ++i) full[n_full + i] = cl[i]; n_full += m; }
    else { for (int i = 0; i < m; ++i) shorts[n_short + i] = cl[i]; n_short += m; }
  }
  sh->n_full[p] = n_full;
  sh->n_short[p] = n_short;
  rc = 0;
done:
  if (level) for (int c = 0; c <= B + 1; ++c) free(level[c]);
  free(level); free(lsize); free(lcap); free(touched); free(fifo); free(cl);
  return rc;
}

static void* co_worker(void* arg) {
  struct co_job* jb = (struct co_job*)arg;
  struct co_shared* sh = jb->sh;
  const int t = jb->tid, T = sh->nthreads;
  for (;;) {
    const int g = __atomic_load_n(&sh->gate, __ATOMIC_ACQUIRE);
    if (g > 0) break;
    if (g < 0) return NULL;
    sched_yield();
  }
  for (;;) {
    const int64_t nf = sh->nfront;
    if (nf == 0) break;
    const int64_t a = nf * t / T, b = nf * (t + 1) / T;
    for (int64_t i = a; i < b; ++i) {
      const int32_t u = sh->frontier[i], ru = sh->region[u];
      for (int64_t e = sh->indptr[u]; e < sh->indptr[u + 1]; ++e) {
        const int32_t v = sh->indices[e];
        if (v < 0 || v >= sh->n || __atomic_load_n(&sh->region[v], __ATOMIC_RELAXED) >= 0) continue;
        int32_t c = __atomic_load_n(&sh->cand[v], __ATOMIC_RELAXED);
        while (ru < c && !__atomic_compare_exchange_n(&sh->cand[v], &c, ru, 1, __ATOMIC_RELAXED, __ATOMIC_RELAXED)) {}
      }
    }
    pthread_barrier_wait(&sh->bar);
    sh->nnext[t] = 0;
    for (int64_t i = a; i < b && !sh->failed; ++i) {
      const int32_t u = sh->frontier[i];
      for (int64_t e = sh->indptr[u]; e < sh->indptr[u + 1]; ++e) {
        const int32_t v = sh->indices[e];
        if (v < 0 || v >= sh->n) continue;
        int32_t expect = -1;
        const int32_t c = sh->cand[v];
        if (c == 0x7fffffff) continue;
        if (__atomic_compare_exchange_n(&sh->region[v], &expect, c, 0, __ATOMIC_RELAXED, __ATOMIC_RELAXED)) {
          if (sh->nnext[t] == sh->capnext[t]) {
            sh->capnext[t] = sh->capnext[t] ? 2 * sh->capnext[t] : 4096;
            int32_t* g = (int32_t*)realloc(sh->next[t], 4 * (size_t)sh->capnext[t]);
            if (!g) { sh->failed = 1; break; }
            sh->next[t] = g;
          }
          sh->next[t][sh->nnext[t]++] = v;
        }
      }
    }
    pthread_barrier_wait(&sh->bar);
    if (t == 0) {
      int64_t tot = 0;
      for (int k = 0; k < T; ++k) { if (sh->nnext[k]) memcpy(sh->frontier + tot, sh->next[k], 4 * (size_t)sh->nnext[k]); tot += sh->nnext[k]; }
      sh->nfront = sh->failed ? 0 : tot;
    }
    pthread_barrier_wait(&sh->bar);
  }
  pthread_barrier_wait(&sh->bar);
  if (t == 0 && !sh->failed) {
    const int64_t n = sh->n;
    for (int64_t i = 0; i < n; ++i) if (sh->region[i] < 0) sh->region[i] = (int32_t)(i * sh->P / n);
    for (int p = 0; p <= sh->P; ++p) sh->rstart[p] = 0;
    for (int64_t i = 0; i < n; ++i) sh->rstart[sh->region[i] + 1]++;
    for (int p = 0; p < sh->P; ++p) sh->rstart[p + 1] += sh->rstart[p];
    int64_t* cur = (int64_t*)malloc(8 * (size_t)sh->P);
    if (!cur) sh->failed = 1;
    else {
      memcpy(cur, sh->rstart, 8 * (size_t)sh->P);
      for (int64_t i = 0; i < n; ++i) sh->members[cur[sh->region[i]]++] = (int32_t)i;
      free(cur);
    }
  }
  pthread_barrier_wait(&sh->bar);
  while (!sh->failed) {
    const int64_t p = __atomic_fetch_add(&sh->next_region, 1, __ATOMIC_RELAXED);
    if (p >= sh->P) break;
    if (co_grow(sh, (int)p) != 0) sh->failed = 1;
  }
  return NULL;
}

int64_t cna_host_cluster_order_mt(int64_t n, const int64_t* indptr, const int32_t* indices, int B, int nthreads,
                                  int64_t* order_out) {
  if (n <= 0) return 0;
  int P = (int)(n / 65536);
  if (P > 64) P = 64;
  if (P < 2 || nthreads < 1) return cna_host_cluster_order(n, indptr, indices, B, order_out);
  if (B < 1) B = 1;
  if (nthreads > 64) nthreads = 64;
  struct co_shared sh;
  memset(&sh, 0, sizeof(sh));
  sh.n = n; sh.indptr = indptr; sh.indices = indices; sh.B = B; sh.P = P; sh.nthreads = nthreads;
  sh.region = (int32_t*)malloc(4 * (size_t)n);
  sh.cand = (int32_t*)malloc(4 * (size_t)n);
  sh.frontier = (int32_t*)malloc(4 * (size_t)n);
  sh.next = (int32_t**)calloc((size_t)nthreads, sizeof(int32_t*));
  sh.nnext = (int64_t*)calloc((size_t)nthreads, 8);
  sh.capnext = (int64_t*)calloc((size_t)nthreads, 8);
  sh.rstart = (int64_t*)calloc((size_t)P + 1, 8);
  sh.members = (int32_t*)malloc(4 * (size_t)n);
  sh.state = (int32_t*)calloc((size_t)n, 4);
  sh.queued = (unsigned char*)calloc((size_t)n, 1);
  sh.out_full = (int64_t*)malloc(8 * (size_t)n);
  sh.out_short = (int64_t*)malloc(8 * (size_t)n);
  sh.n_full = (int64_t*)calloc((size_t)P, 8);
  sh.n_short = (int64_t*)calloc((size_t)P, 8);
  int64_t rc = -1;
  pthread_t th[64];
  struct co_job jobs[64];
  int started = 0, bar_ok = 0, seq_fallback = 0;
  if (!sh.region || !sh.cand || !sh.frontier || !sh.next || !sh.nnext || !sh.capnext || !sh.rstart || !sh.members ||
      !sh.state || !sh.queued || !sh.out_full || !sh.out_short || !sh.n_full || !sh.n_short) goto done;
  for (int64_t i = 0; i < n; ++i) { sh.region[i] = -1; sh.cand[i] = 0x7fffffff; }
  for (int p = 0; p < P; ++p) {
    const int64_t sidx = (int64_t)p * n / P;
    sh.region[sidx] = p;
    sh.frontier[p] = (int32_t)sidx;
  }
  sh.nfront = P;
  if (pthread_barrier_init(&sh.bar, NULL, (unsigned)nthreads) != 0) goto done;
// ... 130 lines not shown
```

cna_amd/csrc/local_null.hip:

```cpp
#include "common.h"
#include <sched.h>
#include <cmath>
#include <cstring>

static void guess_from_thr(const double* thr, int T, double* thr0, double* inv_step) {
  *thr0 = T > 0 ? thr[0] : 0.0;
  const double step = T > 1 ? thr[1] - thr[0] : 0.0;
  *inv_step = step > 0 ? 1.0 / step : 0.0;
}

static void exact_cuts(const double* edges, int T, int Nx, std::vector<double>& cuts, double* cut0,
                       double* inv_step, double* eps) {
  cuts.resize(T);
  const double dn = (double)Nx;
  for (int t = 0; t < T; ++t) {
    const double e = edges[t];
    auto ok = [&](double a) { volatile double z = a / dn; volatile double z2 = z * z; return z2 >= e; };
    if (e <= 0.0 || ok(0.0)) { cuts[t] = 0.0; continue; }
    uint64_t lo = 0, hi = 0x7ff0000000000000ull;
    const double guess = dn * std::sqrt(e);
    uint64_t g;
    std::memcpy(&g, &guess, 8);
    if (guess > 0.0 && g > 64 && g < hi - 64) {
      double a;
      uint64_t b = g - 64;
      std::memcpy(&a, &b, 8);
      if (!ok(a)) lo = b;
      b = g + 64;
      std::memcpy(&a, &b, 8);
      if (ok(a)) hi = b;
    }
    while (hi - lo > 1) {
      const uint64_t mid = lo + (hi - lo) / 2;
      double a;
      std::memcpy(&a, &mid, 8);
      if (ok(a)) hi = mid; else lo = mid;
    }
    std::memcpy(&cuts[t], &hi, 8);
  }
  *cut0 = cuts[0];
  *inv_step = 0.0;
  *eps = 2.0;
  if (T >= 3 && cuts[T - 1] > cuts[0]) {
    const double step = (cuts[T - 1] - cuts[0]) / (T - 1);
    double dev = 0.0;
    for (int t = 0; t < T; ++t) dev = std::max(dev, std::fabs(cuts[t] - (*cut0 + t * step)) / step);
    *inv_step = 1.0 / step;
    *eps = 2.0 * dev + 1e-9;
    if (!(*eps < 0.25)) *eps = 2.0;
  }
}

static int ensure_zc(cna_ctx* c, int N, int P, hipStream_t st) {
  const int ldy = round_up(P, 64) + 64;
  const int rows = x_ld(N);
  void* p = c->zc;
  CNA_TRY(dev_reserve(c, &p, &c->zc_cap, (int64_t)sizeof(double) * rows * ldy));
  c->zc = (double*)p;
  HIP_TRY(hipMemsetAsync(c->zc, 0, sizeof(double) * rows * ldy, st));
  c->zc_ld = ldy;
  c->zc_cols = P;
  c->zc_rows = N;
  return 0;
}

static NullCarve null_carve(void* scratch, int P, int T) {
  Carver cv(scratch);
  NullCarve k;
  k.cuts = cv.take<double>(T);
  k.hist = cv.take<unsigned long long>((int64_t)P * T);
  k.tails = cv.take<int64_t>((int64_t)P * T);
  k.sums = cv.take<int64_t>(T);
  k.obs_edges = cv.take<double>(T);
  k.obs_thr = cv.take<double>(T);
  k.obs_hist = cv.take<unsigned long long>(2 * (int64_t)T);
  k.obs_tails = cv.take<int64_t>(2 * (int64_t)T);
  return k;
}
static int64_t null_carve_bytes(int P, int T) {
  const int64_t t = 8 * (int64_t)T, pt = t * P;
  return carve_bytes({t, pt, pt, t, t, t, 2 * t, 2 * t});
}
static NullHostLayout null_host_layout(int P, int T, int want_tails) {
  NullHostLayout h;
  h.tails = h.sums + 8 * (int64_t)T;
  h.obs = h.tails + (want_tails ? 8 * (int64_t)P * T : 0);
  h.stage = h.obs + 16 * (int64_t)T;
  h.status = h.stage + 24 * (int64_t)T;
  h.bytes = h.status + 16;
  return h;
}

int null_local_prepare(cna_ctx* c, int P, const double* edges, int T, int want_tails, const double* thr) {
  NullPass& np = c->null;
  CellColumns& cc = c->cells;
  if (cc.bins_pending) {
    HIP_TRY(hipStreamWaitEvent(c->stream, cc.bins_copied, 0));
    cc.bins_pending = false;
  }
  if (P < 1 || T < 1) CNA_FAIL(CNA_EINVAL, "cna_null_local: P and T must be positive");
  if (np.phase == NULL_PENDING) CNA_FAIL(CNA_ESTATE, "a local-null pass is still pending: fetch it first");
  for (int t = 1; t < T; ++t)
    if (!(edges[t] >= edges[t - 1])) CNA_FAIL(CNA_EINVAL, "cna_null_local: edges must ascend");
  np.phase = NULL_IDLE;
  cc.fdr_inline = false;
  std::vector<double> cuts;
  exact_cuts(edges, T, c->Nx, cuts, &np.cut0, &np.inv_step, &np.eps);
  const NullHostLayout h = null_host_layout(P, T, want_tails);
  HIP_TRY(hipEventSynchronize(c->stage_done));
  if (h.bytes > c->h_res_cap) {
    HIP_TRY(hipStreamSynchronize(c->stream));
    if (c->h_res) HIP_TRY(hipHostFree(c->h_res));
    c->h_res = nullptr;
    HIP_TRY(hipHostMalloc(&c->h_res, (size_t)h.bytes, hipHostMallocDefault));
    c->h_res_cap = h.bytes;
  }
  CNA_TRY(dev_reserve(c, &c->scratch, &c->scratch_cap, null_carve_bytes(P, T)));
  const NullCarve k = null_carve(c->scratch, P, T);
  char* hr = (char*)c->h_res;
  double* st = (double*)(hr + h.stage);
  np.has_obs = 0;
  if (thr) {
    if (!c->ncorrs_valid) CNA_FAIL(CNA_ESTATE, "threshold counts need cna_ncorrs");
    guess_from_thr(thr, T, &np.thr0, &np.thr_step);
    std::memcpy(st + T, edges, 8 * (size_t)T);
    std::memcpy(st + 2 * T, thr, 8 * (size_t)T);
    HIP_TRY(hipMemcpyAsync(k.obs_edges, st + T, 8 * T, hipMemcpyHostToDevice, c->stream));
    HIP_TRY(hipMemcpyAsync(k.obs_thr, st + 2 * T, 8 * T, hipMemcpyHostToDevice, c->stream));
    CNA_TRY(launch_obs_counts(c, k.obs_edges, k.obs_thr, T, np.thr0, np.thr_step, k.obs_hist));
    CNA_TRY(comm_allreduce_i64_sum(c, (int64_t*)k.obs_hist, (size_t)2 * T));
    CNA_TRY(launch_suffix_sum(c, k.obs_hist, 2, T, k.obs_tails));
    HIP_TRY(hipMemcpyAsync(hr + h.obs, k.obs_tails, 16 * (size_t)T, hipMemcpyDeviceToHost, c->stream));
    np.has_obs = 1;
  }
  std::memcpy(st, cuts.data(), 8 * (size_t)T);
  HIP_TRY(hipMemcpyAsync(k.cuts, st, 8 * T, hipMemcpyHostToDevice, c->stream));
  HIP_TRY(hipEventRecord(c->stage_done, c->stream));
  np.host = h;
  np.P = P;
  np.T = T;
  np.has_tails = want_tails;
  np.phase = NULL_PREPARED;
  return 0;
}

int null_local_go(cna_ctx* c, int col0) {
  NullPass& np = c->null;
  CellColumns& cc = c->cells;
  if (np.phase != NULL_PREPARED) CNA_FAIL(CNA_ESTATE, "local-null pass not prepared");
  np.phase = NULL_IDLE;
  const int P = np.P, T = np.T;
  if (!c->zc || col0 < 0 || col0 + P > c->zc_cols || c->zc_rows != c->Nx ||
      c->zc_cap < (int64_t)sizeof(double) * c->ldx * c->zc_ld)
    CNA_FAIL(CNA_ESTATE, "no conditioned phenotypes resident for these columns");
  const NullCarve k = null_carve(c->scratch, P, T);
  char* hr = (char*)c->h_res;
  const bool inline_fdr = cc.coef_early && np.has_obs && T <= 512;
  if (inline_fdr) {
    const int64_t n_out = c->local_view ? c->n_local : c->n_global;
    void* bp = cc.bins_dev;
    CNA_TRY(dev_reserve(c, &bp, &cc.bins_cap, 2 * std::max<int64_t>(std::max(c->n_pad, n_out), 1)));
    cc.bins_dev = (unsigned short*)bp;
    if (2 * n_out > cc.h_bins_cap) {
      if (cc.h_bins) HIP_TRY(hipHostFree(cc.h_bins));
      cc.h_bins = nullptr;
      HIP_TRY(hipHostMalloc((void**)&cc.h_bins, (size_t)std::max<int64_t>(2 * n_out, 64), hipHostMallocDefault));
      cc.h_bins_cap = 2 * n_out;
    }
    hipStream_t cs = c->coef_stream;
    CNA_TRY(launch_percell_bins(c, c->stream, cc.coef_dev, k.obs_thr, T, np.thr0, np.thr_step, cc.bins_dev));
    HIP_TRY(hipEventRecord(c->stage_done, c->stream));
    HIP_TRY(hipStreamWaitEvent(cs, c->stage_done, 0));
    if (n_out > 0) HIP_TRY(hipMemcpyAsync(cc.h_bins, cc.bins_dev, 2 * (size_t)n_out, hipMemcpyDeviceToHost, cs));
    HIP_TRY(hipEventRecord(cc.bins_copied, cs));
    cc.bins_pending = true;
  }
  int* i8_status = nullptr;
  int64_t* sums = k.sums;
  np.i8_last = false;
  if (!np.has_tails && null_i8_eligible(c, P, T, np.cut0, np.inv_step, np.eps))
    CNA_TRY(launch_null_local_i8(c, c->zc + col0, c->zc_ld, P, k.cuts, T, np.cut0, np.inv_step, np.eps, &sums, &i8_status));
  np.i8_last = i8_status != nullptr;
  np.col0 = col0;
  np.status_off = -1;
  if (i8_status) {
    CNA_TRY(comm_allreduce_i64_sum(c, sums, (size_t)T));
    int64_t* stw = (int64_t*)i8_status;
    CNA_TRY(comm_allreduce_i64_sum(c, stw, 1));
    np.status_off = np.host.status;
    HIP_TRY(hipMemcpyAsync(hr + np.host.status, stw, 8, hipMemcpyDeviceToHost, c->stream));
  } else {
    CNA_TRY(launch_null_local(c, c->zc + col0, c->zc_ld, P, k.cuts, T, np.cut0, np.inv_step, np.eps, k.hist, nullptr));
    if (np.has_tails) CNA_TRY(comm_allreduce_i64_sum(c, (int64_t*)k.hist, (size_t)P * T));
    CNA_TRY(launch_suffix_sum(c, k.hist, P, T, k.tails));
    CNA_TRY(launch_tail_sums(c, k.tails, P, T, sums));
    if (!np.has_tails) CNA_TRY(comm_allreduce_i64_sum(c, sums, (size_t)T));
  }
  HIP_TRY(hipMemcpyAsync(hr + np.host.sums, sums, 8 * (size_t)T, hipMemcpyDeviceToHost, c->stream));
  if (inline_fdr) {
    double* tab = cc.coef_dev + 4 * c->n_pad;
    CNA_TRY(launch_fdr_table(c, sums, k.obs_tails, T, P, tab, tab + 512));
    if (!cc.h_tab) HIP_TRY(hipHostMalloc((void**)&cc.h_tab, 8 * 512, hipHostMallocDefault));
    HIP_TRY(hipMemcpyAsync(cc.h_tab, tab + 512, 8 * (size_t)T, hipMemcpyDeviceToHost, c->stream));
    cc.fdr_inline = true;
  }
  if (np.has_tails)
    HIP_TRY(hipMemcpyAsync(hr + np.host.tails, k.tails, 8 * (size_t)P * T, hipMemcpyDeviceToHost, c->stream));
  HIP_TRY(hipEventRecord(c->null_done, c->stream));
  cc.fdr_early_copied = false;
  cc.fdr_early_dst = nullptr;
  cc.fdr_early_served = false;
  np.phase = NULL_PENDING;
  return 0;
}

static int null_local_collect(cna_ctx* c, int64_t* tails_out, int64_t* sums_out, int64_t* ranks_out = nullptr,
                              int64_t* numdet_out = nullptr) {
  NullPass& np = c->null;
  if (np.phase != NULL_PENDING) CNA_FAIL(CNA_ESTATE, "no local-null pass pending");
  np.phase = NULL_IDLE;
  HIP_TRY(hipEventSynchronize(c->null_done));
  const int P = np.P, T = np.T;
  char* hr = (char*)c->h_res;
  const int64_t status_off = np.status_off;
  if (status_off >= 0 && *(volatile const int64_t*)(hr + status_off) != 0) {
    c->cells.fdr_inline = false;
    const NullCarve k = null_carve(c->scratch, P, T);
    HIP_TRY(hipMemcpyAsync(k.cuts, hr + np.host.stage, 8 * (size_t)T, hipMemcpyHostToDevice, c->stream));
    CNA_TRY(launch_null_local(c, c->zc + np.col0, c->zc_ld, P, k.cuts, T, np.cut0, np.inv_step, np.eps, k.hist, nullptr));
    CNA_TRY(launch_suffix_sum(c, k.hist, P, T, k.tails));
    CNA_TRY(launch_tail_sums(c, k.tails, P, T, k.sums));
    CNA_TRY(comm_allreduce_i64_sum(c, k.sums, (size_t)T));
    HIP_TRY(hipMemcpyAsync(hr + np.host.sums, k.sums, 8 * (size_t)T, hipMemcpyDeviceToHost, c->stream));
    HIP_TRY(hipStreamSynchronize(c->stream));
  }
  np.status_off = -1;
  if (ranks_out || numdet_out) {
    if (!np.has_obs) CNA_FAIL(CNA_EINVAL, "the pending pass was launched without thresholds");
    if (ranks_out) std::memcpy(ranks_out, hr + np.host.obs, 8 * (size_t)T);
    if (numdet_out) std::memcpy(numdet_out, hr + np.host.obs + 8 * (size_t)T, 8 * (size_t)T);
  }
  if (sums_out) std::memcpy(sums_out, hr + np.host.sums, 8 * (size_t)T);
  if (tails_out) {
    if (!np.has_tails) CNA_FAIL(CNA_EINVAL, "the pending pass was launched without want_tails");
    std::memcpy(tails_out, hr + np.host.tails, 8 * (size_t)P * T);
  }
  return 0;
}

static int null_local_on_resident(cna_ctx* c, int col0, int P, const double* edges, int T, int64_t* tails_out,
                                  int64_t* sums_out) {
  CNA_TRY(null_local_prepare(c, P, edges, T, tails_out != nullptr, nullptr));
  CNA_TRY(null_local_go(c, col0));
  return null_local_collect(c, tails_out, sums_out);
}

extern "C" {

int cna_reference_thresholds(double maxabs, int cap, double* thr, double* edges) {
#pragma clang fp contract(off)
  const double maxcorr = maxabs > 0.001 ? maxabs : 0.001;
  if (!(maxcorr < 1e300)) return 0;
  const double start = maxcorr / 4, stop = maxcorr, step = maxcorr / 400;
  const double len = std::ceil((stop - start) / step);
  if (!(len >= 1) || len > cap) return 0;
  const int T = (int)len;
  const double next = start + step;
  const double delta = next - start;
  for (int i = 0; i < T; ++i) {
    volatile double t = i == 0 ? start : (i == 1 ? next : start + (double)i * delta);
    thr[i] = t;
    volatile double z2 = t * t;
    volatile double a = z2 - 1e-8;
    volatile double b = 1e-5 * z2;
    edges[i] = a - b;
  }
  return T;
}

int cna_null_local_prepare(cna_ctx* c, int P, const double* edges, int T, int want_tails, const double* thr) {
  CHECK_CTX(c);
  if (!c->x_valid) CNA_FAIL(CNA_ESTATE, "X not available");
  if (!edges) CNA_FAIL(CNA_EINVAL, "cna_null_local_prepare: edges required");
  return null_local_prepare(c, P, edges, T, want_tails, thr);
}

int cna_null_local_launch(cna_ctx* c, int col0, int P, const double* edges, int T, int want_tails, const double* thr) {
  CHECK_CTX(c);
  if (!c->x_valid) CNA_FAIL(CNA_ESTATE, "X not available");
  if (edges) CNA_TRY(null_local_prepare(c, P, edges, T, want_tails, thr));
  else if (c->null.phase != NULL_PREPARED || P != c->null.P || T != c->null.T)
    CNA_FAIL(CNA_ESTATE, "cna_null_local_launch without edges needs a matching cna_null_local_prepare");
  return null_local_go(c, col0);
}

int cna_null_local_fetch(cna_ctx* c, int64_t* tails_out, int64_t* tail_sums_out, int64_t* ranks_out,
                         int64_t* num_detected_out) {
  CHECK_CTX(c);
  return null_local_collect(c, tails_out, tail_sums_out, ranks_out, num_detected_out);
}

int cna_null_local_discard(cna_ctx* c) {
  CHECK_CTX(c);
  if (c->null.phase.exchange(NULL_IDLE) != NULL_PENDING) return 0;
  HIP_TRY(hipEventSynchronize(c->null_done));
  return 0;
}

int cna_null_local_i8_stats(cna_ctx* c, int* used_out, int64_t* rechecked_out, int* fallback_out) {
  CHECK_CTX(c);
  unsigned long long v[2] = {0, 0};
  if (c->null.i8_last) {
    HIP_TRY(hipStreamSynchronize(c->stream));
    HIP_TRY(hipMemcpy(v, c->i8_qcount, 16, hipMemcpyDeviceToHost));
  }
  if (used_out) *used_out = c->null.i8_last ? 1 : 0;
  if (rechecked_out) *rechecked_out = (int64_t)v[0];
  if (fallback_out) *fallback_out = (int)(v[1] & 0xffffffffull) != 0;
  return 0;
}

int cna_null_local(cna_ctx* c, const double* Yc, int P, const double* edges, int T, int64_t* tails_out) {
  CHECK_CTX(c);
  if (!c->x_valid) CNA_FAIL(CNA_ESTATE, "X not available");
  if (P < 1) CNA_FAIL(CNA_EINVAL, "cna_null_local: P must be positive");
  CNA_TRY(ensure_zc(c, c->Nx, P, c->stream));
  HIP_TRY(hipMemcpy2DAsync(c->zc, sizeof(double) * c->zc_ld, Yc, sizeof(double) * P, sizeof(double) * P, c->Nx,
                           hipMemcpyHostToDevice, c->stream));
  return null_local_on_resident(c, 0, P, edges, T, tails_out, nullptr);
}

int cna_null_local_resident(cna_ctx* c, int col0, int P, const double* edges, int T, int64_t* tails_out,
                            int64_t* tail_sums_out) {
  CHECK_CTX(c);
  if (!c->x_valid) CNA_FAIL(CNA_ESTATE, "X not available");
  return null_local_on_resident(c, col0, P, edges, T, tails_out, tail_sums_out);
}

int cna_condition_phenotypes(cna_ctx* c, const double* M, const double* Y, int N, int P) {
  CHECK_CTX(c);
  if (P < 1) CNA_FAIL(CNA_EINVAL, "P must be positive");
  if (N < 2) CNA_FAIL(CNA_EINVAL, "need at least two samples");
  if (c->null.phase == NULL_PENDING) CNA_FAIL(CNA_ESTATE, "a local-null pass is still pending: fetch it first");
  hipStream_t st = c->copy_stream;
  CNA_TRY(ensure_zc(c, N, P, st));
  void* g = c->gt;
  CNA_TRY(dev_reserve(c, &g, &c->gt_cap, carve_bytes({8 * (int64_t)N * N, 8 * (int64_t)N * P})));
  c->gt = g;
  Carver cv(c->gt);
  double* Md = cv.take<double>((int64_t)N * N);
  double* Yd = cv.take<double>((int64_t)N * P);
  HIP_TRY(hipMemcpyAsync(Md, M, 8 * (size_t)N * N, hipMemcpyHostToDevice, st));
  HIP_TRY(hipMemcpyAsync(Yd, Y, 8 * (size_t)N * P, hipMemcpyHostToDevice, st));
  CNA_TRY(launch_condition(c, st, Md, Yd, N, P, c->zc, c->zc_ld));
  HIP_TRY(hipStreamSynchronize(st));
  return 0;
}

int cna_obs_counts(cna_ctx* c, const double* edges, const double* thr, int T, int64_t* ranks_out,
                   int64_t* num_detected_out) {
  CHECK_CTX(c);
  NO_NULL_PENDING(c, "cna_obs_counts");
  if (!c->ncorrs_valid) CNA_FAIL(CNA_ESTATE, "cna_obs_counts needs cna_ncorrs");
  if (T < 1) CNA_FAIL(CNA_EINVAL, "T < 1");
  double thr0, inv_step;
  guess_from_thr(thr, T, &thr0, &inv_step);
  CNA_TRY(dev_reserve(c, &c->scratch, &c->scratch_cap, carve_bytes({8 * (int64_t)T, 8 * (int64_t)T, 16 * (int64_t)T, 16 * (int64_t)T})));
  Carver cv(c->scratch);
  double* ed = cv.take<double>(T);
  double* td = cv.take<double>(T);
  unsigned long long* hist = cv.take<unsigned long long>(2 * T);
  int64_t* tails = cv.take<int64_t>(2 * T);
  HIP_TRY(hipMemcpyAsync(ed, edges, 8 * T, hipMemcpyHostToDevice, c->stream));
  HIP_TRY(hipMemcpyAsync(td, thr, 8 * T, hipMemcpyHostToDevice, c->stream));
  CNA_TRY(launch_obs_counts(c, ed, td, T, thr0, inv_step, hist));
  CNA_TRY(comm_allreduce_i64_sum(c, (int64_t*)hist, (size_t)2 * T));
  CNA_TRY(launch_suffix_sum(c, hist, 2, T, tails));
  std::vector<int64_t> h(2 * T);
  HIP_TRY(hipMemcpyAsync(h.data(), tails, 16 * T, hipMemcpyDeviceToHost, c->stream));
  HIP_TRY(hipStreamSynchronize(c->stream));
  if (ranks_out) std::memcpy(ranks_out, h.data(), 8 * T);
  if (num_detected_out) std::memcpy(num_detected_out, h.data() + T, 8 * T);
  return 0;
}

static int ensure_cell_pinned(cna_ctx* c, int64_t n_out) {
  const int64_t need = 16 * std::max<int64_t>(n_out, 1);
  if (need > c->cells.h_cell_cap) {
    if (c->cells.h_cell) HIP_TRY(hipHostFree(c->cells.h_cell));
    c->cells.h_cell = nullptr;
    c->cells.coef_early = false;
    c->cells.fdr_inline = false;
    HIP_TRY(hipHostMalloc(&c->cells.h_cell, (size_t)need, hipHostMallocDefault));
    c->cells.h_cell_cap = need;
  }
  return 0;
}

int cna_percell_coef_launch(cna_ctx* c) {
  CHECK_CTX(c);
  if (!c->ncorrs_valid || !c->x_from_nam) CNA_FAIL(CNA_ESTATE, "cna_percell_coef_launch needs cna_select + cna_ncorrs");
  if ((c->nranks > 1 || comm_active(c)) && !c->local_view)
    CNA_FAIL(CNA_ESTATE, "cna_percell_coef_launch: replicated multi-rank outputs are assembled by cna_percell_fdr");
  const int64_t n_out = c->local_view ? c->n_local : c->n_global;
  CNA_TRY(ensure_cell_pinned(c, n_out));
  void* p = c->cells.coef_dev;
  CNA_TRY(dev_reserve(c, &p, &c->cells.coef_dev_cap, 32 * std::max<int64_t>(c->n_pad, 1) + 16 * 512));
  c->cells.coef_dev = (double*)p;
  double* tmp = c->cells.coef_dev;
  double* out = tmp;
  CNA_TRY(launch_percell_fdr(c, nullptr, nullptr, 0, 0.0, 0.0, tmp, nullptr));
  if (c->orig_idx) {
    out = c->cells.coef_dev + c->n_pad;
    CNA_TRY(launch_unpermute2(c, tmp, nullptr, c->orig_idx, c->n_local, out, nullptr));
  }
  HIP_TRY(hipEventRecord(c->cells.coef_ready, c->stream));
  hipStream_t cs = c->coef_stream;
  HIP_TRY(hipStreamWaitEvent(cs, c->cells.coef_ready, 0));
  if (n_out > 0)
    HIP_TRY(hipMemcpyAsync(c->cells.h_cell, out, 8 * n_out, hipMemcpyDeviceToHost, cs));
  HIP_TRY(hipEventRecord(c->cells.coef_copied, cs));
  c->cells.coef_early = true;
  return 0;
}

int cna_percell_coef_wait(cna_ctx* c, double** coef_ptr) {
  CHECK_CTX(c);
  if (!coef_ptr) CNA_FAIL(CNA_EINVAL, "cna_percell_coef_wait: coef_ptr is required");
  if (!c->cells.coef_early) CNA_FAIL(CNA_ESTATE, "cna_percell_coef_wait without cna_percell_coef_launch");
  HIP_TRY(hipEventSynchronize(c->cells.coef_copied));
  *coef_ptr = (double*)c->cells.h_cell;
  return 0;
}

int cna_percell_fdr_copy_early(cna_ctx* c, double* dst, int64_t n, int nthreads, int* done) {
  CHECK_CTX(c);
  if (!dst || !done) CNA_FAIL(CNA_EINVAL, "cna_percell_fdr_copy_early: dst and done are required");
  *done = 0;
  const int64_t n_out = c->local_view ? c->n_local : c->n_global;
  if (!c->cells.coef_early || !c->cells.fdr_inline || c->null.phase != NULL_PENDING || !c->cells.h_cell || n != n_out) return 0;
  struct Flight { std::atomic<int>& f; Flight(std::atomic<int>& f_) : f(f_) { f.store(1); } ~Flight() { f.store(0); } } flight(c->cells.fdr_early_inflight);
  HIP_TRY(hipEventSynchronize(c->cells.bins_copied));
  HIP_TRY(hipEventSynchronize(c->null_done));
  const int64_t status_off = c->null.status_off;
  if (status_off >= 0 && *(volatile int64_t*)((char*)c->h_res + status_off) != 0)
    return 0;
  if (!c->cells.fdr_inline) return 0;
  if (cna_host_expand_u16(dst, c->cells.h_bins, n, c->cells.h_tab, c->null.T, nthreads) != 0)
    CNA_FAIL(CNA_ESTATE, "cna_percell_fdr_copy_early: expansion failed");
  c->cells.fdr_early_dst = dst;
  c->cells.fdr_early_copied = true;
  *done = 1;
  return 0;
}

int cna_percell_fdr_copied_early(cna_ctx* c, int* yes) {
  CHECK_CTX(c);
  if (!yes) CNA_FAIL(CNA_EINVAL, "cna_percell_fdr_copied_early: yes is required");
  *yes = c->cells.fdr_early_copied && c->cells.fdr_inline && c->cells.fdr_early_served;
  return 0;
}

int cna_percell_fdr_pinned(cna_ctx* c, const double* thr, const double* runmin_fdr, int T, double** coef_ptr,
                           double** fdr_ptr) {
  CHECK_CTX(c);
  NO_NULL_PENDING(c, "cna_percell_fdr_pinned");
  if (!coef_ptr) CNA_FAIL(CNA_EINVAL, "cna_percell_fdr_pinned: coef_ptr is required");
  const int64_t n_out = c->local_view ? c->n_local : c->n_global;
  CNA_TRY(ensure_cell_pinned(c, n_out));
  double* hc = (double*)c->cells.h_cell;
  const bool want_fdr = fdr_ptr && thr && runmin_fdr && T > 0;
  if (c->cells.coef_early) HIP_TRY(hipEventSynchronize(c->cells.coef_copied));
  if (c->cells.coef_early && c->cells.fdr_inline && want_fdr && T == c->null.T && c->null.phase != NULL_PENDING) {
    HIP_TRY(hipEventSynchronize(c->cells.bins_copied));
    HIP_TRY(hipEventSynchronize(c->null_done));
    while (c->cells.fdr_early_inflight.load()) sched_yield();
    *coef_ptr = hc;
    if (c->cells.fdr_early_copied && c->cells.fdr_early_dst) {
      *fdr_ptr = c->cells.fdr_early_dst;
    } else {
      if (cna_host_expand_u16(hc + n_out, c->cells.h_bins, n_out, c->cells.h_tab, T, 4) != 0)
        CNA_FAIL(CNA_ESTATE, "cna_percell_fdr_pinned: expansion failed");
      *fdr_ptr = hc + n_out;
    }
    c->cells.fdr_early_served = true;
    return 0;
  }
  c->cells.fdr_early_served = false;
  CNA_TRY(cna_percell_fdr(c, thr, runmin_fdr, T, c->cells.coef_early ? nullptr : hc, want_fdr ? hc + n_out : nullptr));
  *coef_ptr = hc;
  if (fdr_ptr) *fdr_ptr = want_fdr ? hc + n_out : nullptr;
  return 0;
}

int cna_percell_fdr(cna_ctx* c, const double* thr, const double* runmin_fdr, int T, double* coef_out,
                    double* fdr_out) {
  CHECK_CTX(c);
  NO_NULL_PENDING(c, "cna_percell_fdr");
  if (!c->ncorrs_valid || !c->x_from_nam) CNA_FAIL(CNA_ESTATE, "cna_percell_fdr needs cna_select + cna_ncorrs");
  const bool want_fdr = fdr_out && thr && runmin_fdr && T > 0;
  double thr0 = 0, inv_step = 0;
  if (want_fdr) guess_from_thr(thr, T, &thr0, &inv_step);
  const int64_t Tn = want_fdr ? T : 1;
  CNA_TRY(dev_reserve(c, &c->scratch, &c->scratch_cap,
                      carve_bytes({8 * Tn, 8 * Tn, 8 * c->n_pad, 8 * c->n_pad, 8 * c->n_pad, 8 * c->n_pad})));
  Carver cv(c->scratch);
  double* td = cv.take<double>(Tn);
  double* rd = cv.take<double>(Tn);
  double* coef = cv.take<double>(c->n_pad);
  double* fdr = cv.take<double>(c->n_pad);
  double* coef_u = cv.take<double>(c->n_pad);
  double* fdr_u = cv.take<double>(c->n_pad);
  if (want_fdr) {
    HIP_TRY(hipMemcpyAsync(td, thr, 8 * T, hipMemcpyHostToDevice, c->stream));
    HIP_TRY(hipMemcpyAsync(rd, runmin_fdr, 8 * T, hipMemcpyHostToDevice, c->stream));
  }
  CNA_TRY(launch_percell_fdr(c, td, rd, want_fdr ? T : 0, thr0, inv_step, coef + c->row0, want_fdr ? fdr + c->row0 : nullptr));
  const bool sharded = (c->nranks > 1 || comm_active(c)) && !c->local_view;
  int64_t n_out = c->n_global;
  if (c->local_view) {
    n_out = c->n_local;
    if (c->orig_idx) {
      CNA_TRY(launch_unpermute2(c, coef + c->row0, want_fdr ? fdr + c->row0 : nullptr, c->orig_idx, c->n_local, coef_u,
                                fdr_u));
      coef = coef_u;
      fdr = fdr_u;
    } else {
      coef += c->row0;
      fdr += c->row0;
    }
  } else if (c->orig_idx) {
    if (sharded) {
      HIP_TRY(hipMemsetAsync(coef_u, 0, 8 * c->n_pad, c->stream));
      if (want_fdr) HIP_TRY(hipMemsetAsync(fdr_u, 0, 8 * c->n_pad, c->stream));
    }
    CNA_TRY(launch_unpermute2(c, coef + c->row0, want_fdr ? fdr + c->row0 : nullptr, c->orig_idx, c->n_local, coef_u,
                              fdr_u));
    if (sharded) {
      CNA_TRY(comm_allreduce_f64_sum(c, coef_u, (size_t)c->n_global));
      if (want_fdr) CNA_TRY(comm_allreduce_f64_sum(c, fdr_u, (size_t)c->n_global));
    }
    coef = coef_u;
    fdr = fdr_u;
  } else if (c->nranks > 1) {
    const size_t block = 8 * (size_t)c->rows_per_rank;
    CNA_TRY(comm_allgather_bytes(c, (char*)coef + block * c->rank, coef, block));
    if (want_fdr) CNA_TRY(comm_allgather_bytes(c, (char*)fdr + block * c->rank, fdr, block));
  }
  if (coef_out && n_out > 0) HIP_TRY(hipMemcpyAsync(coef_out, coef, 8 * n_out, hipMemcpyDeviceToHost, c->stream));
  if (want_fdr && n_out > 0) HIP_TRY(hipMemcpyAsync(fdr_out, fdr, 8 * n_out, hipMemcpyDeviceToHost, c->stream));
  HIP_TRY(hipStreamSynchronize(c->stream));
  return 0;
}

}
```

cna_amd/csrc/null_i8.hip:

```cpp
#include "common.h"
#include <algorithm>

typedef int v4i __attribute__((ext_vector_type(4)));
typedef int v16i __attribute__((ext_vector_type(16)));

#define I8_Q I8_QMAX
#define I8_DROP (2.0 * 128 * 128 * 256 + 128.0 * 128 + 0.25)
#define I8_QBUF 192

__global__ __launch_bounds__(1024) void k_y_absmax(const double* __restrict__ Y, int ldy, int N, int P,
                                                   unsigned long long* __restrict__ scal) {
  __shared__ double red[16];
  double m = 0.0;
  const int64_t tot = (int64_t)N * P;
  for (int64_t i = (int64_t)blockIdx.x * 1024 + threadIdx.x; i < tot; i += (int64_t)gridDim.x * 1024) {
    const int k = (int)(i / P), p = (int)(i - (int64_t)k * P);
    m = fmax(m, fabs(Y[(size_t)k * ldy + p]));
  }
  m = wave_max_d(m);
  if ((threadIdx.x & 63) == 0) red[threadIdx.x >> 6] = m;
  __syncthreads();
  if (threadIdx.x == 0) {
    for (int w = 1; w < 16; ++w) m = fmax(m, red[w]);
    atomicMax(&scal[0], (unsigned long long)__double_as_longlong(m));
// ... 39 lines not shown
  for (int p = threadIdx.x; p < P; p += 1024) m = colL1[p] > m ? colL1[p] : m;
#pragma unroll
  for (int o = 32; o > 0; o >>= 1) {
    const unsigned long long v = __shfl_xor(m, o);
    m = v > m ? v : m;
  }
  if ((threadIdx.x & 63) == 0) red[threadIdx.x >> 6] = m;
  __syncthreads();
  if (threadIdx.x == 0) {
    for (int w = 1; w < 16; ++w) m = red[w] > m ? red[w] : m;
    scal[1] = m;
  }
}

__global__ __launch_bounds__(256) void k_quant_x(const double* __restrict__ X, int ldx, int64_t nx, int N, int Kp,
                                                 unsigned char* __restrict__ Xq, double2* __restrict__ xscale) {
  const int lane = threadIdx.x & 63, wv = threadIdx.x >> 6;
  const int k0 = 4 * lane;
  const bool act = k0 < Kp;
  for (int r = 0; r < 8; ++r) {
    const int64_t row = (int64_t)blockIdx.x * 32 + wv * 8 + r;
    if (row >= nx) return;
    double x[4] = {0.0, 0.0, 0.0, 0.0};
    if (act) {
      const double* xr = X + (size_t)row * ldx;
#pragma unroll
      for (int j = 0; j < 4; ++j)
        if (k0 + j < N) x[j] = xr[k0 + j];
    }
    const double rmax = wave_max_d(fmax(fmax(fabs(x[0]), fabs(x[1])), fmax(fabs(x[2]), fabs(x[3]))));
    const double inv = rmax > 0.0 ? I8_Q / rmax : 0.0;
    unsigned w0 = 0, w1 = 0, w2 = 0;
    double l1 = 0.0;
#pragma unroll
    for (int j = 0; j < 4; ++j) {
      const double v = x[j] * inv;
      const int q = v == v ? (int)rint(v) : 0;
      l1 += (double)(q < 0 ? -q : q);
      unsigned d0, d1, d2;
      digits3(q, d0, d1, d2);
      w0 |= d0 << (8 * j);
      w1 |= d1 << (8 * j);
      w2 |= d2 << (8 * j);
    }
    l1 = wave_sum(l1);
    if (act) {
      unsigned* rq = (unsigned*)(Xq + (size_t)row * 3 * Kp);
      rq[lane] = w0;
      rq[Kp / 4 + lane] = w1;
      rq[2 * (Kp / 4) + lane] = w2;
    }
    if (lane == 0) xscale[row] = make_double2(rmax, l1);
  }
}

__global__ void k_rowinfo(const double2* __restrict__ xscale, int64_t nx, int64_t nrows, int N,
                          const unsigned long long* __restrict__ scal, double inv_step, double slack,
                          float2* __restrict__ rowinfo) {
  const int64_t row = (int64_t)blockIdx.x * blockDim.x + threadIdx.x;
  if (row >= nrows) return;
  float a = 0.f, m = 0.f;
  if (row < nx) {
    const double2 sc = xscale[row];
    if (sc.x > 0.0) {
      const double ymax = __longlong_as_double((long long)scal[0]);
      const double l1y = (double)scal[1];
      const double unit = (sc.x / I8_Q) * (ymax / I8_Q) * inv_step;
      const double U = 0.5 * sc.y + 0.5 * l1y + (double)N * I8_DROP + 2.0 * 16777216.0;
      a = (float)(unit * 16777216.0);
      m = (float)((unit * U + slack) * 1.0001);
    }
  }
  rowinfo[row] = make_float2(a, m);
}

template <int KS, int G, int MODE = 0>
__global__ __launch_bounds__(512) void k_null_i8(const unsigned char* __restrict__ Xq, const float2* __restrict__ rowinfo,
                                                 int64_t ntiles, const v4i* __restrict__ Yq, int nstages, int nsplit,
                                                 int spp, int T, float bconst, unsigned int* __restrict__ partial,
                                                 uint2* __restrict__ queue, unsigned long long* __restrict__ qcount,
                                                 unsigned long long qcap, int* __restrict__ status, int rotate) {
  extern __shared__ v4i sm[];
  constexpr int SB = 3 * KS * 128;
  constexpr int SG = G * SB;
  constexpr int LPT = (SG + 511) / 512;
  constexpr int NCT = 2 * G;
  const int TW = T + 1;
  v4i* bbuf = sm;
  unsigned* hist = (unsigned*)(sm + 2 * SG);
  uint2* qb_all = (uint2*)(hist + (size_t)TW * 32 + 64);
  const int tid = threadIdx.x, lane = tid & 63;
  const int wv = __builtin_amdgcn_readfirstlane(tid >> 6);
  const int j = lane & 31, kh = lane >> 5;
  uint2* qb = qb_all + wv * I8_QBUF;
  const float Thi = (float)T + 0.5f;
  const bool rot = rotate != 0 && wv >= 4;
  unsigned* histj = hist + j;
  for (int i = tid; i < TW * 32 + 64; i += 512) hist[i] = 0u;

  const int64_t nitems = ((ntiles + 7) / 8) * nsplit;
  int wcount = 0;

  auto flush = [&]() {
    __builtin_amdgcn_fence(__ATOMIC_RELEASE, "wavefront");
    unsigned long long base = 0;
    if (lane == 0) base = atomicAdd(qcount, (unsigned long long)wcount);
    base = ((unsigned long long)__builtin_amdgcn_readfirstlane((int)(base >> 32)) << 32) |
           (unsigned)__builtin_amdgcn_readfirstlane((int)(base & 0xffffffffu));
    if (base + (unsigned long long)wcount <= qcap) {
      for (int i = lane; i < wcount; i += 64) queue[base + i] = qb[i];
    } else if (lane == 0) {
      atomicOr(status, 1);
    }
    __builtin_amdgcn_fence(__ATOMIC_ACQUIRE, "wavefront");
    wcount = 0;
  };

  if (blockIdx.x < nitems) {
    auto stage = [&](int st, int b) {
      const v4i* src = Yq + (size_t)st * SG;
      __attribute__((address_space(3))) v4i* dst = (__attribute__((address_space(3))) v4i*)sm + b * SG;
#pragma unroll
      for (int u = 0; u < LPT; ++u) {
        const int ch = (u * 8 + wv) * 64;
        if (ch < SG)
          __builtin_amdgcn_global_load_lds((const void __attribute__((address_space(1)))*)(src + ch + lane),
                                           (__attribute__((address_space(3))) void*)(dst + ch), 16, 0, 0);
      }
    };
    stage((int)(blockIdx.x % nsplit) * spp, 0);
    asm volatile("s_waitcnt vmcnt(0)" ::: "memory");
    __syncthreads();
    int it = 0;
    v16i S2, S3, S4;
    bool carry = false;
    unsigned carry_perm0 = 0;
    for (int64_t item = blockIdx.x; item < nitems; item += gridDim.x) {
      const int64_t tile = (item / nsplit) * 8 + wv;
      const int st0 = (int)(item % nsplit) * spp;
      const int st1 = st0 + spp < nstages ? st0 + spp : nstages;
      const bool last = item + gridDim.x >= nitems;
      const int nxt0 = (int)((item + gridDim.x) % nsplit) * spp;
      const bool have = tile < ntiles;
      v4i a[3][KS];
      float ai[16], mi[16];
      {
        const unsigned char* ap = Xq + ((size_t)(have ? tile : 0) * 32 + j) * (3 * 32 * KS) + 16 * kh;
#pragma unroll
        for (int d = 0; d < 3; ++d)
#pragma unroll
          for (int s = 0; s < KS; ++s) a[d][s] = have ? *(const v4i*)(ap + d * 32 * KS + 32 * s) : (v4i){0, 0, 0, 0};
        const float2* rp = rowinfo + (size_t)(have ? tile : 0) * 32 + 4 * kh;
#pragma unroll
        for (int r = 0; r < 16; ++r) {
          const float2 ri = rp[(r & 3) + 8 * (r >> 2)];
          ai[r] = have ? ri.x : 0.f;
          mi[r] = have ? 0.5f - ri.y : 0.5f;
        }
      }
      auto epilogue = [&](unsigned perm0) {
        unsigned long long nm[16], anym = 0ull;
#pragma unroll
        for (int r = 0; r < 16; ++r) {
          const int w = S2[r] * 256 + S3[r] + (S4[r] >> 8);
          const float t = fmaf(fabsf((float)w), ai[r], bconst);
          const float u = __builtin_amdgcn_fmed3f(t, 0.5f, Thi);
          const bool near = fabsf(__builtin_amdgcn_fractf(u) - 0.5f) > mi[r];
          nm[r] = __ballot(near);
          anym |= nm[r];
          if (MODE == 2) { if ((int)u == 0x7fffff) atomicAdd(&hist[j], 1u); }
          else atomicAdd(&histj[(int)u * 32], 1u);
        }
        if (__builtin_expect(anym != 0ull, 0)) {
          const unsigned perm = perm0 + (unsigned)j;
#pragma unroll
          for (int r = 0; r < 16; ++r) {
            const unsigned long long bal = nm[r];
            if (bal == 0ull) continue;
            if ((bal >> lane) & 1ull) {
              const int pos = wcount + __builtin_amdgcn_mbcnt_hi((unsigned)(bal >> 32), __builtin_amdgcn_mbcnt_lo((unsigned)bal, 0u));
              qb[pos].x = (unsigned)(tile * 32 + (r & 3) + 8 * (r >> 2) + 4 * kh);
              const int w = S2[r] * 256 + S3[r] + (S4[r] >> 8);
              const int h = (int)__builtin_amdgcn_fmed3f(fmaf(fabsf((float)w), ai[r], bconst), 0.5f, Thi);
              qb[pos].y = perm | ((unsigned)h << 16);
            }
            wcount += __popcll(bal);
            if (wcount > I8_QBUF - 64) flush();
          }
        }
      };
      for (int st = st0; st < st1; ++st, ++it) {
        const bool more = st + 1 < st1 || !last;
        const int nst = st + 1 < st1 ? st + 1 : nxt0;
        if (more) stage(nst, (it + 1) & 1);
        if (carry) {
          epilogue(carry_perm0);
          carry = false;
        }
        const v4i* buf = bbuf + ((it & 1) * SG + kh * 64 + j);
        v4i bq[2][3];
#pragma unroll
        for (int d = 0; d < 3; ++d) bq[0][d] = buf[((d * KS) * 2) * 64];
        if (MODE != 3) __builtin_amdgcn_sched_group_barrier(0x100, 3, 0);
#pragma unroll
        for (int c = 0; c < NCT; ++c) {
#pragma unroll
          for (int r = 0; r < 16; ++r) { S2[r] = 0; S3[r] = 0; S4[r] = 0; }
#pragma unroll
          for (int s = 0; s < KS; ++s) {
            const int cs = c * KS + s;
            if (cs + 1 < NCT * KS) {
              const int c1 = (cs + 1) / KS, s1 = (cs + 1) % KS;
#pragma unroll
              for (int d = 0; d < 3; ++d)
                bq[(cs + 1) & 1][d] = buf[(c1 >> 1) * SB + ((d * KS + s1) * 2) * 64 + (c1 & 1) * 32];
            }
            const v4i b0 = bq[cs & 1][0], b1 = bq[cs & 1][1], b2 = bq[cs & 1][2];
            if (MODE == 3) { S4[0] += b0[0] + a[0][s][0]; S3[1] += b1[1] + a[1][s][1]; S2[2] += b2[2] + a[2][s][2]; }
            else {
              S4 = __builtin_amdgcn_mfma_i32_32x32x32_i8(a[0][s], b2, S4, 0, 0, 0);
              S3 = __builtin_amdgcn_mfma_i32_32x32x32_i8(a[1][s], b2, S3, 0, 0, 0);
              S2 = __builtin_amdgcn_mfma_i32_32x32x32_i8(a[2][s], b2, S2, 0, 0, 0);
              S4 = __builtin_amdgcn_mfma_i32_32x32x32_i8(a[1][s], b1, S4, 0, 0, 0);
              S3 = __builtin_amdgcn_mfma_i32_32x32x32_i8(a[2][s], b1, S3, 0, 0, 0);
              S4 = __builtin_amdgcn_mfma_i32_32x32x32_i8(a[2][s], b0, S4, 0, 0, 0);
              if (cs + 1 < NCT * KS) __builtin_amdgcn_sched_group_barrier(0x100, 3, 0);
              __builtin_amdgcn_sched_group_barrier(0x008, 6, 0);
            }
          }
          if (MODE == 1) {
            int z = 0;
#pragma unroll
            for (int r = 0; r < 16; ++r) z |= S2[r] ^ S3[r] ^ S4[r];
            if (z == 0x12345678) atomicAdd(&hist[j], 1u);
            continue;
          }
          const unsigned perm0 = (unsigned)((st * G + (c >> 1)) * 64 + (c & 1) * 32);
          if (c == NCT - 1 && rot && st + 1 < st1) {
            carry = true;
            carry_perm0 = perm0;
          } else {
            epilogue(perm0);
          }
        }
        asm volatile("s_waitcnt vmcnt(0)" ::: "memory");
        __syncthreads();
      }
    }
    if (wcount > 0) flush();
  }
  __syncthreads();
  for (int t = tid; t < TW; t += 512) {
    unsigned s = 0;
#pragma unroll 8
    for (int q = 0; q < 32; ++q) s += hist[t * 32 + q];
    partial[(size_t)blockIdx.x * TW + t] = s;
  }
}

__global__ __launch_bounds__(256) void k_null_recheck(const double* __restrict__ X, int ldx, int N,
                                                      const double* __restrict__ Yt, int ldt,
                                                      const uint2* __restrict__ queue,
                                                      const unsigned long long* __restrict__ qcount,
                                                      unsigned long long qcap, const double* __restrict__ cuts, int T,
                                                      double cut0, double inv_step,
                                                      unsigned int* __restrict__ partial) {
  extern __shared__ unsigned rh[];
  const int TW = T + 1;
  for (int i = threadIdx.x; i < TW; i += 256) rh[i] = 0u;
  __syncthreads();
  unsigned long long cnt = *qcount;
  if (cnt > qcap) cnt = 0;
  const int sub = threadIdx.x & 15;
  const unsigned long long ngrp = (unsigned long long)gridDim.x * 16;
  for (unsigned long long e = (unsigned long long)blockIdx.x * 16 + (threadIdx.x >> 4); e < cnt; e += ngrp) {
    const uint2 en = queue[e];
    const double* xr = X + (size_t)en.x * ldx;
    const double* yr = Yt + (size_t)(en.y & 0xffffu) * ldt;
    const unsigned counted = en.y >> 16;
    double s = 0.0;
    for (int k = sub; k < N; k += 16) s = fma(xr[k], yr[k], s);
#pragma unroll
    for (int o = 8; o > 0; o >>= 1) s += __shfl_xor(s, o);
    if (sub == 0) {
      const double x = fabs(s);
      int h = 0;
      if (x >= cut0) {
        double g = (x - cut0) * inv_step;
        h = g < (double)T ? (int)g + 1 : T;
        if (h > T) h = T;
      }
      while (h < T && cuts[h] <= x) ++h;
      while (h > 0 && cuts[h - 1] > x) --h;
      if (h != (int)counted) {
        if (h > 0) atomicAdd(&rh[h], 1u);
        if (counted > 0) atomicSub(&rh[counted], 1u);
      }
    }
  }
  __syncthreads();
  for (int i = threadIdx.x; i < TW; i += 256) partial[(size_t)blockIdx.x * TW + i] = rh[i];
}

__global__ __launch_bounds__(256) void k_i8_reduce(const unsigned int* __restrict__ partial, int nslabs, int nplain, int T,
                                                   unsigned long long* __restrict__ hist) {
  const int t = blockIdx.x * 4 + (threadIdx.x >> 6), lane = threadIdx.x & 63;
  if (t >= T) return;
  unsigned long long s = 0;
  for (int b = lane; b < nslabs; b += 64) {
    const unsigned v = partial[(size_t)b * (T + 1) + t + 1];
    s += b < nplain ? (unsigned long long)v : (unsigned long long)(long long)(int)v;
  }
#pragma unroll
  for (int o = 32; o > 0; o >>= 1) s += __shfl_xor(s, o);
  if (lane == 0) hist[t] = s;
}

typedef int (*i8_launch_fn)(cna_ctx*, unsigned, size_t, const unsigned char*, const float2*, int64_t, const v4i*, int, int, int, int, float,
                            unsigned int*, uint2*, unsigned long long*, unsigned long long, int*);
constexpr int i8_stage_strips(int KS) { return KS >= 5 ? 1 : (KS >= 3 ? 2 : 4); }
template <int KS>
static int launch_i8_t(cna_ctx* c, unsigned grid, size_t smem, const unsigned char* Xq, const float2* rowinfo, int64_t ntiles,
                       const v4i* Yq, int nstages, int nsplit, int spp, int T, float bconst, unsigned int* partial, uint2* queue,
                       unsigned long long* qcount, unsigned long long qcap, int* status) {
  constexpr int G = i8_stage_strips(KS);
  static bool attr_set = false;
  if (!attr_set) {
    HIP_TRY(hipFuncSetAttribute((const void*)k_null_i8<KS, G>, hipFuncAttributeMaxDynamicSharedMemorySize, 160 * 1024));
    attr_set = true;
  }
  const int rotate = 0;
  hipLaunchKernelGGL((k_null_i8<KS, G>), dim3(grid), dim3(512), smem, c->stream, Xq, rowinfo, ntiles, Yq, nstages, nsplit, spp, T,
                     bconst, partial, queue, qcount, qcap, status, rotate);
  HIP_TRY(hipGetLastError());
  return 0;
}
static const i8_launch_fn kI8[8] = {launch_i8_t<1>, launch_i8_t<2>, launch_i8_t<3>, launch_i8_t<4>,
                                    launch_i8_t<5>, launch_i8_t<6>, launch_i8_t<7>, launch_i8_t<8>};

static size_t i8_lds(int KS, int T) {
  return (size_t)2 * i8_stage_strips(KS) * 3 * KS * 128 * 16 + (size_t)(T + 1) * 32 * 4 + 256 + (size_t)8 * I8_QBUF * 8;
}

bool null_i8_enabled() {
  const char* e = getenv("CNA_NULL_F64");
  return !(e && atoi(e) != 0);
}
bool null_i8_eligible(const cna_ctx* c, int P, int T, double cut0, double inv_step, double eps) {
  if (!null_i8_enabled()) return false;
  if (c->Nx > 256 || c->Nx < 2 || c->nx < 1) return false;
  if (P > 65535 - 64 || T > 65535) return false;
  if (!(inv_step > 0.0) || !(eps < 0.05) || !(cut0 * inv_step > 2.0) || !(cut0 * inv_step + T < 5e4)) return false;
  const int KS = (c->Nx + 31) / 32;
  return i8_lds(KS, T) <= 160 * 1024 && c->nx < (int64_t)1 << 31;
}

int ensure_xq(cna_ctx* c, int KS) {
  const int64_t rows = (c->nx + 31) / 32 * 32;
  const int64_t need = rows * 3 * 32 * KS, need_s = rows * 16;
  if (c->xq_valid && (c->xq_rows != rows || c->xq_KS != KS)) c->xq_valid = false;
  if (c->xq_valid) return 0;
  CNA_TRY(dev_reserve(c, &c->xq, &c->xq_cap, std::max<int64_t>(need, 256)));
  CNA_TRY(dev_reserve(c, &c->xq_scale, &c->xq_scale_cap, std::max<int64_t>(need_s, 256)));
  if (rows > c->nx) {
    HIP_TRY(hipMemsetAsync((char*)c->xq + c->nx * 3 * 32 * KS, 0, (size_t)(rows - c->nx) * 3 * 32 * KS, c->stream));
    HIP_TRY(hipMemsetAsync((char*)c->xq_scale + c->nx * 16, 0, (size_t)(rows - c->nx) * 16, c->stream));
  }
  c->xq_rows = rows;
  c->xq_KS = KS;
  return 0;
}

int launch_null_local_i8(cna_ctx* c, const double* Yc_dev, int ldy, int P, const double* cuts_dev, int T, double cut0,
                         double inv_step, double eps, int64_t** sums_out, int** status_out) {
  const int N = c->Nx, KS = (N + 31) / 32;
  const int64_t ntiles = (c->nx + 31) / 32;
  const int nstrips = (P + 63) / 64, Ppad = nstrips * 64;
  const int ldt = round_up(N, 16);
  const int nrecheck = 1024;
  const double slack = eps + (cut0 * inv_step + T + 2.0) * 5e-7 + 1e-6;
  const int64_t ngroups = (ntiles + 7) / 8;
  const int G = i8_stage_strips(KS);
  const int nstages = (nstrips + G - 1) / G;
  int nsplit = (int)((12 * 256 + ngroups - 1) / ngroups);
  if (nsplit > nstages) nsplit = nstages;
  if (nsplit < 1) nsplit = 1;
  const int spp = (nstages + nsplit - 1) / nsplit;
  nsplit = (nstages + spp - 1) / spp;
  const int64_t nitems = ngroups * nsplit;
  const unsigned grid = (unsigned)(nitems < 256 ? nitems : 256);
  const int nslabs = (int)grid + nrecheck;
  uint64_t qcap = (uint64_t)(c->nx / 16) * (uint64_t)Ppad / 4;
  if (qcap < ((uint64_t)1 << 20)) qcap = (uint64_t)1 << 20;
  if (const char* e = getenv("CNA_I8_QCAP")) qcap = (uint64_t)atoll(e) > 0 ? (uint64_t)atoll(e) : qcap;
  const int64_t sizes[] = {
      (int64_t)256,
      (int64_t)8 * 32 * ntiles,
      (int64_t)16 * 3 * KS * 128 * nstages * G,
      (int64_t)8 * Ppad * ldt,
      (int64_t)8 * Ppad + 64,
      (int64_t)8 * (int64_t)qcap,
      (int64_t)4 * nslabs * (T + 1),
      (int64_t)8 * T, (int64_t)8 * T};
  int64_t need = 0;
  for (int64_t s : sizes) need += round_up64(s, 256);
  CNA_TRY(dev_reserve(c, &c->i8_buf, &c->i8_cap, need));
  char* base = (char*)c->i8_buf;
  int64_t off = 0;
  auto take = [&](int idx) { char* p = base + off; off += round_up64(sizes[idx], 256); return p; };
  take(0);
  CNA_TRY(ensure_xq(c, KS));
  const unsigned char* Xq = (const unsigned char*)c->xq;
  float2* rowinfo = (float2*)take(1);
  v4i* Yq = (v4i*)take(2);
  double* Yt = (double*)take(3);
  unsigned long long* colL1 = (unsigned long long*)take(4);
  unsigned long long* scal = colL1 + Ppad;
  unsigned long long* qcount = scal + 2;
  int* status = (int*)(scal + 3);
  uint2* queue = (uint2*)take(5);
  unsigned int* slabs = (unsigned int*)take(6);
  unsigned long long* hist = (unsigned long long*)take(7);
  int64_t* sums_dev = (int64_t*)take(8);
  ProfScope ps(c, CNA_K_NULL_LOCAL);
  HIP_TRY(hipMemsetAsync(colL1, 0, (size_t)8 * Ppad + 64, c->stream));
  if (nstages * G > nstrips)
    HIP_TRY(hipMemsetAsync(Yq + (size_t)nstrips * 3 * KS * 128, 0, (size_t)16 * 3 * KS * 128 * (nstages * G - nstrips), c->stream));
  hipLaunchKernelGGL(k_y_absmax, dim3(16), dim3(1024), 0, c->stream, Yc_dev, ldy, N, P, scal);
  {
    const int64_t nthr = (int64_t)Ppad * 2 * KS;
    hipLaunchKernelGGL(k_quant_y, dim3((unsigned)((nthr + 255) / 256)), dim3(256), 0, c->stream, Yc_dev, ldy, N, P, KS, Ppad,
                       scal, Yq, Yt, ldt, colL1);
  }
  hipLaunchKernelGGL(k_y_finish, dim3(1), dim3(1024), 0, c->stream, colL1, P, scal);
  if (!c->xq_valid) {
    hipLaunchKernelGGL(k_quant_x, dim3((unsigned)ntiles), dim3(256), 0, c->stream, c->X, c->ldx, c->nx, N, 32 * KS,
                       (unsigned char*)c->xq, (double2*)c->xq_scale);
    c->xq_valid = true;
  }
  hipLaunchKernelGGL(k_rowinfo, dim3((unsigned)((ntiles * 32 + 255) / 256)), dim3(256), 0, c->stream, (const double2*)c->xq_scale,
                     c->nx, ntiles * 32, N, scal, inv_step, slack, rowinfo);
  const float bconst = (float)(1.0 - cut0 * inv_step);
  CNA_TRY(kI8[KS - 1](c, grid, i8_lds(KS, T), Xq, rowinfo, ntiles, Yq, nstages, nsplit, spp, T, bconst, slabs, queue, qcount, qcap, status));
  hipLaunchKernelGGL(k_null_recheck, dim3(nrecheck), dim3(256), (size_t)4 * (T + 1), c->stream, c->X, c->ldx, N, Yt, ldt, queue,
                     qcount, qcap, cuts_dev, T, cut0, inv_step, slabs + (size_t)grid * (T + 1));
  hipLaunchKernelGGL(k_i8_reduce, dim3((unsigned)((T + 3) / 4)), dim3(256), 0, c->stream, slabs, nslabs, (int)grid, T, hist);
  HIP_TRY(hipGetLastError());
  CNA_TRY(launch_suffix_sum(c, hist, 1, T, sums_dev));
  *sums_out = sums_dev;
  *status_out = status;
  c->i8_qcount = qcount;
  return 0;
}
```

include/cna_hip.h:

```cpp
#ifndef CNA_HIP_H
#define CNA_HIP_H

#include <stdint.h>

#ifdef __cplusplus
extern "C" {
#endif

typedef struct cna_ctx cna_ctx;

#define CNA_EINVAL  (-1)
#define CNA_ENOMEM  (-2)
#define CNA_ERCCL   (-3)
#define CNA_ESTATE  (-4)

#define CNA_MAT_NAM   0
#define CNA_MAT_X     1
#define CNA_MAT_PROJ  2

enum {
  CNA_K_COLSUM = 0, CNA_K_NAM_FIRST, CNA_K_NAM_STEP, CNA_K_BATCH_KURT, CNA_K_ZEROVAR,
  CNA_K_SELECT, CNA_K_RESID, CNA_K_STANDARDIZE, CNA_K_GRAM, CNA_K_GRAM_REDUCE, CNA_K_NCORRS,
  CNA_K_NULL_LOCAL, CNA_K_OBS_COUNTS, CNA_K_PERCELL_FDR, CNA_K_PROJECT, CNA_K_TRANSPOSE,
  CNA_K_ALLGATHER, CNA_K_CONDITION, CNA_K_GLOBAL_TEST,
  CNA_K_NAM_STEP_SPARSE,
  CNA_K_HALO_EXCHANGE, CNA_K_HALO_WAIT,
  CNA_K_MATRIX_BINS_SORT, CNA_K_MATRIX_BINS_SUM,
  CNA_K_ENRICH_POSITIONS, CNA_K_ENRICH_EXTREMES,
  CNA_K_EXPR_CROSS_BY, CNA_K_GRAM_BY,
  CNA_K_COUNT
};

const char* cna_last_error(void);
int  cna_abi_version(void);
int  cna_device_count(int* count);
int  cna_ctx_create(int device, cna_ctx** out);
int  cna_ctx_destroy(cna_ctx* ctx);
int  cna_ctx_sync(cna_ctx* ctx);
int  cna_ctx_device_bytes(cna_ctx* ctx, int64_t* bytes);
int  cna_set_state_f32(cna_ctx* ctx, int on);

int  cna_comm_unique_id(void* id128);
int  cna_comm_init(cna_ctx* ctx, int rank, int nranks, const void* id128);
int  cna_comm_init_shm(cna_ctx* ctx, int rank, int nranks, const char* name, int64_t slot_bytes);
int  cna_comm_info(cna_ctx* ctx, int* backend, int* nranks);
int  cna_comm_selftest(cna_ctx* ctx, double timeout_s, int* halo_ok);

int  cna_set_halo(cna_ctx* ctx, const int64_t* send_rows, const int64_t* send_counts,
                  const int64_t* recv_rows, const int64_t* recv_counts);

int  cna_graph_upload(cna_ctx* ctx, int64_t n_global, int64_t row0, int64_t n_local,
                      const int64_t* indptr, const int32_t* indices,
                      const void* data, int data_is_f64);
int  cna_set_cell_order(cna_ctx* ctx, const int64_t* orig_index);
int  cna_graph_reorder(cna_ctx* ctx, const int64_t* perm);
int  cna_set_local_view(cna_ctx* ctx, int on);
int  cna_colsums(cna_ctx* ctx, double self_weight);
int  cna_fetch_colsums(cna_ctx* ctx, double* out_n_global);

int  cna_set_samples(cna_ctx* ctx, const int32_t* codes, int n_samples, const double* counts);
int  cna_restart_nam(cna_ctx* ctx);
int  cna_nam_step(cna_ctx* ctx, int want_kurt, int may_continue, int may_stop);
int  cna_nam_steps(cna_ctx* ctx, int nsteps);
int  cna_nam_select_hint(cna_ctx* ctx, const double* y, int n_samples);
int  cna_nam_auto(cna_ctx* ctx, int maxnsteps, int* steps_out, double* medkurt_out);
int  cna_nam_auto_launch(cna_ctx* ctx, int maxnsteps);
int  cna_nam_auto_finish(cna_ctx* ctx, int* steps_out, double* medkurt_out);
int  cna_stat_qc(cna_ctx* ctx, double* median_out, double* threshold_out, int64_t* n_dropped_out);
int  cna_fetch_cell_stat(cna_ctx* ctx, double* out, int64_t n_expected);
int  cna_stat_median(cna_ctx* ctx, double* median_out);
int  cna_load_cell_stat(cna_ctx* ctx, const double* v, int64_t n);

int  cna_dense_load(cna_ctx* ctx, const double* s_local, int m);
int  cna_dense_step(cna_ctx* ctx);
int  cna_dense_fetch(cna_ctx* ctx, double* s_local_out);

int  cna_batch_kurtosis(cna_ctx* ctx, int which, const int32_t* batch_codes, int n_batches);
int  cna_zero_variance(cna_ctx* ctx, const int32_t* colmap, int n_sel, uint8_t* flags_out,
                       int64_t* n_zero_out);
int  cna_select(cna_ctx* ctx, const int64_t* keep_idx, int64_t n_keep,
                const int32_t* colmap, int n_sel);
int  cna_set_resid_factors(cna_ctx* ctx, const double* C, const double* W, int r, int N);
int  cna_select_checked(cna_ctx* ctx, const int64_t* keep_idx, int64_t n_keep, const int32_t* colmap, int n_sel,
                        int64_t* n_zero_out);
int  cna_select_standardized(cna_ctx* ctx, const int64_t* keep_idx, int64_t n_keep,
                             const int32_t* colmap, int n_sel, int64_t* n_zero_out,
                             const double* y , double* max_abs_out );
int  cna_select_standardized_fused(cna_ctx* ctx, const int64_t* keep_idx, int64_t n_keep, const int32_t* colmap,
                                   int n_sel, int64_t* n_zero_out, const double* y, double* max_abs_out,
                                   int null_P, int* T_out, double* thr_out, int* gram_queued, int* coef_queued,
                                   int null_col0, const int* null_flag, int* null_launched);
int  cna_reference_thresholds(double maxabs, int cap, double* thr, double* edges);
int  cna_upload_x(cna_ctx* ctx, const double* x_local, int64_t n_rows, int n_cols);

int  cna_resid_apply(cna_ctx* ctx, const double* M, int center);
int  cna_resid_lowrank(cna_ctx* ctx, const double* C, const double* W, int r, int center, int standardize,
                       const double* y, double* max_abs_out);
int  cna_resid_lowrank_bk(cna_ctx* ctx, const double* C, const double* W, int r, const double* y, double* max_abs_out,
                          const int32_t* batch_codes, int n_batches, double* median_out);
int  cna_select_resid_bk(cna_ctx* ctx, const double* C, const double* W, int r, const double* y, double* max_abs_out,
                         const int32_t* batch_codes, int n_batches, double* median_out, int64_t* n_qc_failed,
                         int64_t* n_zero, int* done);
int  cna_standardize(cna_ctx* ctx, int center);
int  cna_gram(cna_ctx* ctx, double* G_out);
int  cna_gram_launch(cna_ctx* ctx);
int  cna_gram_fetch(cna_ctx* ctx, double* G_out);
int  cna_gram_pcs_tests(cna_ctx* ctx, int kmax, const int32_t* ks, int K, int r, int use_native, double resid_tol,
                        double gap_tol, double* G_out , double* U_out , int* accepted);
int  cna_project(cna_ctx* ctx, const double* W, int n_w, double* out_local);
int  cna_project_keep(cna_ctx* ctx, const double* W, int n_w);

int  cna_x_identity(cna_ctx* ctx, int* yes);
int  cna_ncorrs(cna_ctx* ctx, const double* y, double* out_local, double* max_abs);
int  cna_null_local(cna_ctx* ctx, const double* Yc, int P, const double* edges, int T,
                    int64_t* tails_out);
int  cna_condition_phenotypes(cna_ctx* ctx, const double* M, const double* Y, int N, int P);
int  cna_null_local_resident(cna_ctx* ctx, int col0, int P, const double* edges, int T, int64_t* tails_out,
                             int64_t* tail_sums_out);
int  cna_null_local_launch(cna_ctx* ctx, int col0, int P, const double* edges, int T, int want_tails,
                           const double* thr );
int  cna_null_local_prepare(cna_ctx* ctx, int P, const double* edges, int T, int want_tails, const double* thr);
int  cna_null_local_fetch(cna_ctx* ctx, int64_t* tails_out, int64_t* tail_sums_out,
                          int64_t* ranks_out, int64_t* num_detected_out );
int  cna_null_local_discard(cna_ctx* ctx);
int  cna_null_local_i8_stats(cna_ctx* ctx, int* used_out, int64_t* rechecked_out, int* fallback_out);
int  cna_global_test(cna_ctx* ctx, const double* U, int kmax, const int32_t* ks, int K, int r,
                     double* minp_out, double* r2_out, int32_t* kidx_out);
int  cna_global_test_launch(cna_ctx* ctx, const double* U, int kmax, const int32_t* ks, int K, int r);
int  cna_global_test_fetch(cna_ctx* ctx, double* minp_out, double* r2_out, int32_t* kidx_out);
int  cna_obs_counts(cna_ctx* ctx, const double* edges, const double* thr, int T,
                    int64_t* ranks_out, int64_t* num_detected_out);
int  cna_percell_fdr(cna_ctx* ctx, const double* thr, const double* runmin_fdr, int T,
                     double* coef_out_global, double* fdr_out_global);
int  cna_percell_fdr_pinned(cna_ctx* ctx, const double* thr, const double* runmin_fdr, int T,
                            double** coef_ptr, double** fdr_ptr);
int  cna_percell_coef_launch(cna_ctx* ctx);
int  cna_percell_coef_wait(cna_ctx* ctx, double** coef_ptr);
int  cna_percell_fdr_copy_early(cna_ctx* ctx, double* dst, int64_t n, int nthreads, int* done);
int  cna_percell_fdr_copied_early(cna_ctx* ctx, int* yes);

#define CNA_ASSOC_DONE      0
#define CNA_ASSOC_GENERAL   1
#define CNA_ASSOC_NEED_PCS  2
#define CNA_ASSOC_STALE     3
#define CNA_ASSOC_MAXT      512
typedef struct cna_assoc_args {
  const int32_t* colmap;
  int32_t n_sel;
  int32_t r;
  const double* y;
  const double* M;
  const double* resid_C;
  const double* resid_W;
  const int32_t* ks;
  int32_t K;
  int32_t Nnull;
  const double* table;
  int32_t draw_pending;
  int32_t conditioned;
  int32_t use_native_eig;
  int32_t coef_first;
  double resid_tol, gap_tol;
  double* coef_dst;
  double* fdr_dst;
  int64_t n_dst;
  int32_t copy_threads;
  int32_t n_verify;
  const void* verify_ptr[4];
  int64_t verify_bytes[4];
  uint64_t verify_hash[4];
  int32_t verify_threads;
  int32_t reserved;
  double* G;
  double* U;
  double* minp;
  double* r2;
  int32_t* kidx;
} cna_assoc_args;
typedef struct cna_assoc_out {
  int32_t status, T, eig_accepted, null_fused;
  int32_t coef_in_dst, fdr_in_dst;
  int64_t n_zero;
  double max_abs;
  double* coef_ptr;
  double* fdr_ptr;
  double t_ms[16];
  double thr[CNA_ASSOC_MAXT], fdr[CNA_ASSOC_MAXT], runmin[CNA_ASSOC_MAXT];
  int64_t tail_sums[CNA_ASSOC_MAXT], ranks[CNA_ASSOC_MAXT], num_detected[CNA_ASSOC_MAXT];
} cna_assoc_out;
int  cna_assoc_begin(cna_ctx* ctx, int nsteps, const double* y_hint, int n_hint);
int  cna_assoc_begin_part(cna_ctx* ctx, int first, int count, int total, const double* y_hint, int n_hint);
int  cna_assoc_finish(cna_ctx* ctx, const cna_assoc_args* args, cna_assoc_out* out);
int  cna_assoc_run(cna_ctx* ctx, int nsteps, const double* y_hint, int n_hint, const cna_assoc_args* args, cna_assoc_out* out);
int  cna_host_draw_join(void);
void cna_host_draw_times(double* out2);

int  cna_matrix_shape(cna_ctx* ctx, int which, int64_t* n_rows_local, int* n_cols);
int  cna_fetch_matrix(cna_ctx* ctx, int which, double* out, int transposed);
int  cna_fetch_rows(cna_ctx* ctx, int which, const int64_t* rows, int64_t n_out,
                    const int32_t* cols, int n_cols, double* out, int transposed);

int  cna_allgather_host(cna_ctx* ctx, const double* local, int64_t count_local, double* out_all,
                        int64_t count_total);

int  cna_host_legacy_randn(uint32_t* key, int* pos, int* has_gauss, double* gauss, int64_t n, double* out);
void cna_host_set_threads(int n);
int  cna_host_argsort_gather(const double* R, int m, int num, const double* y, double* out, int64_t ld_out,
                             const int64_t* rows);
int  cna_host_draw_start(uint32_t* key, int* pos, const double* y, int m, int num, int nlev, const int64_t* lev_off,
                         const int64_t* members, double* out, int64_t ld_out, int threads);
int  cna_host_draw_start_idx(uint32_t* key, int* pos, const double* y, int m, int num, int nlev, const int64_t* lev_off,
                             const int64_t* members, double* out, int64_t ld_out, int threads, int32_t* idx_out);
int  cna_host_gather_rows(const double* y, const int32_t* idx, int m, int num, double* out, int64_t ld_out, int nthreads);
int  cna_host_draw_then_condition(cna_ctx* ctx, const double* M, const double* table, int N, int cols, int* flag);
int  cna_host_draw_wait(void);

uint64_t cna_host_hash64(const void* p, int64_t nbytes, int nthreads);
int  cna_host_copy(void* dst, const void* src, int64_t nbytes, int nthreads);
int  cna_host_expand_u16(double* dst, const uint16_t* bins, int64_t n, const double* runmin, int T, int nthreads);
int64_t cna_host_cluster_order(int64_t n, const int64_t* indptr, const int32_t* indices, int B, int64_t* order_out);
int64_t cna_host_cluster_order_mt(int64_t n, const int64_t* indptr, const int32_t* indices, int B, int nthreads,
                                  int64_t* order_out);
int64_t cna_host_cluster_graph(int64_t n, const int64_t* indptr, const int32_t* indices, const int64_t* order, int B,
                               int64_t* ptr, int32_t* col, int64_t* cnt);
int64_t cna_host_permuted_nnz(const int64_t* perm, int64_t r0, int64_t r1, const int64_t* indptr);
int  cna_host_permute_rows(const int64_t* perm, int64_t r0, int64_t r1, const int64_t* indptr, const int32_t* indices,
                           const void* data, int vbytes, const int64_t* col_map, int64_t* out_indptr,
                           int32_t* out_indices, void* out_data, int nthreads);

int  cna_knn_graph(cna_ctx* ctx, const float* X, int64_t n, int d, int k, int64_t* indptr_out,
                   int32_t* indices_out, float* data_out, int64_t* nnz_out);


int  cna_expr_upload_dense(cna_ctx* ctx, const void* x, int64_t n_cells, int64_t n_genes, int is_f64);
int  cna_expr_upload_sparse(cna_ctx* ctx, const void* indptr, const void* indices, const void* data, int64_t n_cells,
                            int64_t n_genes, int64_t nnz, int index_bytes, int is_f64, int is_csc);
int  cna_expr_drop(cna_ctx* ctx);
int  cna_expr_shape(cna_ctx* ctx, int64_t* n_cells, int64_t* n_genes, int64_t* nnz, int* format, int* is_f64,
                    int64_t* n_uploads);
int  cna_gene_corr(cna_ctx* ctx, const double* V, int q, double* r_out);

int  cna_expr_to_bins(cna_ctx* ctx, const int32_t* codes, int n_bins, int what, double* sums_out, int64_t* counts_out);

int  cna_coef_strata(cna_ctx* ctx, const double* v, const double* fdr, const int32_t* codes, int64_t n_cells, int n_bins,
                     int points, int bw_kind, double bw_value, double fdr_thresh, int64_t* n_out, int64_t* n_kept_out,
                     int64_t* n_pos_out, int64_t* n_neg_out, double* mean_out, double* ssd_out, double* min_out,
                     double* median_out, double* max_out, double* vals_out);

int  cna_gene_corr_by(cna_ctx* ctx, const double* V, int q, const int32_t* codes, int n_bins, double* r_out,
                      double* within_out, int64_t* n_out);

int  cna_expr_cross(cna_ctx* ctx, const int64_t* xrow, int64_t n_cells, double* W_out, double* rho_out, double* sx_out,
                    double* sxx_out, int64_t* m_out);
int  cna_x_generation(cna_ctx* ctx, int64_t* gen);

int  cna_expr_cross_by(cna_ctx* ctx, const int64_t* xrow, const int32_t* codes, int64_t n_cells, int n_bins, int bin0, int nb,
                       double* W_out, double* sx_out, double* sxx_out, int64_t* m_out);
int  cna_gram_by(cna_ctx* ctx, const int64_t* xrow, const int32_t* codes, int64_t n_cells, int n_bins, double* gram_out,
                 int64_t* m_out);

int  cna_matrix_to_bins(cna_ctx* ctx, int which, const int32_t* codes, const double* W, int q, int64_t n_rows, int n_bins,
                        double* sums_out, int64_t* n_out);

int  cna_enrichment_extremes(cna_ctx* ctx, const double* R, int64_t n_cols, int64_t n_genes, const int64_t* set_ptr,
                             const int32_t* set_genes, int n_sets, int weight, double* up_out, double* down_out,
                             int32_t* size_out, int32_t* valid_out);

int  cna_prof_enable(cna_ctx* ctx, int on);
int  cna_prof_reset(cna_ctx* ctx);
int  cna_prof_get(cna_ctx* ctx, int kernel_id, double* total_ms, int64_t* launches);
const char* cna_kernel_name(int kernel_id);

int  cna_host_top_eig(const double* G, int n, int k, double* U_out, double* lam_out, double* resid_out, double* ortho_out);
int  cna_host_eig_check(const double* G, int n, int k, const double* U, const double* lam, double* resid_out, double* ortho_out);

#ifdef __cplusplus
}
#endif
#endif
```

Before: 112.4 billion.

## Fuse i8 null reduce with suffix sum and FDR table; prefill per-cell FDR output early

The i8 null reduction kernel becomes a last-block ticket kernel. It computes the histogram, the suffix sums and, on a single rank, the FDR table and its running minimum in one launch, so the separate suffix-sum and fdr_table launches and one host copy go away. On the host, the per-cell FDR output is prefilled with 1.0 while the null pass is still running, and the indices of 8-cell blocks with nonzero bins are recorded. Once the table arrives, only those blocks are patched, falling back to full expansion when they are dense. The cost is extra host memory and a new limit of T<=512, plus ticket-based cross-block synchronisation that relies on correct fences.

```diff
diff --git a/cna_amd/_ffi.py b/cna_amd/_ffi.py
--- a/cna_amd/_ffi.py
+++ b/cna_amd/_ffi.py
@@ -84,6 +84,9 @@
     'cna_host_hash64': (C.c_uint64, [C.c_void_p, C.c_int64, C.c_int]),
     'cna_host_copy': (C.c_int, [C.c_void_p, C.c_void_p, C.c_int64, C.c_int]),
     'cna_host_expand_u16': (C.c_int, [C.c_void_p, C.c_void_p, C.c_int64, C.c_void_p, C.c_int, C.c_int]),
+    'cna_host_expand_u16_prefill': (C.c_int, [C.c_void_p, C.c_void_p, C.c_int64, C.c_int, C.c_void_p, C.c_void_p, C.c_void_p]),
+    'cna_host_expand_u16_patch': (C.c_int, [C.c_void_p, C.c_void_p, C.c_int64, C.c_void_p, C.c_int, C.c_int, C.c_void_p, C.c_void_p,
+                                        C.c_void_p]),
     'cna_host_permuted_nnz': (C.c_int64, [C.c_void_p, C.c_int64, C.c_int64, C.c_void_p]),
     'cna_host_permute_rows': (C.c_int, [C.c_void_p, C.c_int64, C.c_int64, C.c_void_p, C.c_void_p, C.c_void_p, C.c_int, C.c_void_p,
                                         C.c_void_p, C.c_void_p, C.c_void_p, C.c_int]),
diff --git a/cna_amd/csrc/c_api.hip b/cna_amd/csrc/c_api.hip
--- a/cna_amd/csrc/c_api.hip
+++ b/cna_amd/csrc/c_api.hip
@@ -282,7 +282,8 @@
   if (c->halo_e1) (void)hipEventDestroy(c->halo_e1);
   if (c->halo_e2) (void)hipEventDestroy(c->halo_e2);
   if (c->cells.h_bins) (void)hipHostFree(c->cells.h_bins);
-  if (c->cells.h_tab) (void)hipHostFree(c->cells.h_tab);
+  free(c->cells.h_blocks);
+  free(c->cells.h_kept);
   if (c->h_res) (void)hipHostFree(c->h_res);
   if (c->h_scal) (void)hipHostFree(c->h_scal);
   if (c->h_gram) (void)hipHostFree(c->h_gram);
diff --git a/cna_amd/csrc/common.h b/cna_amd/csrc/common.h
--- a/cna_amd/csrc/common.h
+++ b/cna_amd/csrc/common.h
@@ -56,7 +56,7 @@
   unsigned long long *hist, *obs_hist;
   int64_t *tails, *sums, *obs_tails;
 };
-struct NullHostLayout { int64_t sums = 0, tails = 0, obs = 0, stage = 0, status = 0, bytes = 0; };
+struct NullHostLayout { int64_t status = 0, sums = 0, tab = 0, tails = 0, obs = 0, stage = 0, bytes = 0; };
 enum NullPhase : int { NULL_IDLE = 0, NULL_PREPARED, NULL_PENDING };
 struct NullPass {
   int P = 0, T = 0, col0 = 0, has_tails = 0, has_obs = 0;
@@ -78,7 +78,9 @@
   unsigned short* bins_dev = nullptr;
   unsigned short* h_bins = nullptr;
   bool bins_pending = false;
-  double* h_tab = nullptr;
+  uint32_t* h_blocks = nullptr;
+  uint16_t* h_kept = nullptr;
+  int64_t h_blocks_cap = 0, h_block_counts[16] = {};
   void* h_cell = nullptr;
   int64_t coef_dev_cap = 0, bins_cap = 0, h_bins_cap = 0, h_cell_cap = 0;
   hipEvent_t coef_ready = nullptr, coef_copied = nullptr, bins_copied = nullptr;
@@ -377,6 +379,10 @@
 int launch_percell_bins(cna_ctx* c, hipStream_t st, const double* coef_local, const double* thr_dev, int T, double thr0,
                         double inv_step, unsigned short* bins);
 extern "C" int cna_host_expand_u16(double* dst, const uint16_t* bins, int64_t n, const double* runmin, int T, int nthreads);
+extern "C" int cna_host_expand_u16_prefill(double* dst, const uint16_t* bins, int64_t n, int nthreads, uint32_t* blocks, uint16_t* kept,
+                                           int64_t* counts);
+extern "C" int cna_host_expand_u16_patch(double* dst, const uint16_t* bins, int64_t n, const double* runmin, int T, int nthreads,
+                                         const uint32_t* blocks, const uint16_t* kept, const int64_t* counts);
 int launch_unpermute2(cna_ctx* c, const double* a, const double* b, const int64_t* idx, int64_t n, double* oa,
                       double* ob);
 int launch_percell_fdr(cna_ctx* c, const double* thr_dev, const double* runmin_dev, int T, double thr0,
@@ -397,7 +403,8 @@
 bool null_i8_enabled();
 int ensure_xq(cna_ctx* c, int KS);
 int launch_null_local_i8(cna_ctx* c, const double* Yc_dev, int ldy, int P, const double* cuts_dev, int T, double cut0,
-                         double inv_step, double eps, int64_t** sums_out, int** status_out);
+                         double inv_step, double eps, int64_t** sums_out, int** status_out, const int64_t* ranks_dev = nullptr,
+                         double* fdr_dev = nullptr);
 
 int launch_condition(cna_ctx* c, hipStream_t st, const double* M_dev, const double* Y_dev, int N, int P,
                      double* Zc_dev, int ldy);
diff --git a/cna_amd/csrc/host_graph.c b/cna_amd/csrc/host_graph.c
--- a/cna_amd/csrc/host_graph.c
+++ b/cna_amd/csrc/host_graph.c
@@ -124,18 +124,26 @@
   expand_span(j->d, j->b, j->n, j->tab);
   return NULL;
 }
+static int expand_split(int64_t n, int nthreads, size_t* part) {
+  if (nthreads > 16) nthreads = 16;
+  if ((int64_t)nthreads > n / (1 << 17)) nthreads = (int)(n / (1 << 17));
+  if (nthreads < 1) nthreads = 1;
+  *part = (((size_t)n / nthreads) + 63) & ~(size_t)63;
+  return nthreads;
+}
+static void expand_table(double* t2, const double* runmin, int T) {
+  for (int h = 0; h < 1024; ++h) t2[h] = (h > 0 && h <= T && h <= 512) ? runmin[h - 1] : 1.0;
+}
 int cna_host_expand_u16(double* dst, const uint16_t* bins, int64_t n, const double* runmin, int T, int nthreads) {
   if (n <= 0) return 0;
   if (!dst || !bins || !runmin) return 1;
-  if (nthreads > 16) nthreads = 16;
-  if ((int64_t)nthreads > n / (1 << 17)) nthreads = (int)(n / (1 << 17));
-  if (nthreads < 1) nthreads = 1;
   struct expand_job jobs[16];
   pthread_t th[16];
   int started[16];
   double t2[1024];
-  for (int h = 0; h < 1024; ++h) t2[h] = (h > 0 && h <= T && h <= 512) ? runmin[h - 1] : 1.0;
-  const size_t part = (((size_t)n / nthreads) + 63) & ~(size_t)63;
+  expand_table(t2, runmin, T);
+  size_t part;
+  nthreads = expand_split(n, nthreads, &part);
   for (int t = 0; t < nthreads; ++t) {
     const size_t b = (size_t)t * part;
     jobs[t].d = dst + b; jobs[t].b = bins + b; jobs[t].tab = t2; jobs[t].T = T;
@@ -147,6 +155,122 @@
   for (int t = 1; t < nthreads; ++t) {
     if (started[t]) pthread_join(th[t], NULL);
     else expand_worker(&jobs[t]);
+  }
+  return 0;
+}
+
+struct prefill_job { double* d; const uint16_t* b; size_t i0, n; uint32_t* list; uint16_t* kept; int64_t* count; };
+#ifndef CNA_NO_CLONES
+__attribute__((target_clones("avx2", "default")))
+#endif
+static int64_t prefill_span(double* d, const uint16_t* b, size_t i0, size_t n, uint32_t* list, uint16_t* kept) {
+  int64_t k = 0;
+  const size_t nb = n / 8;
+  for (size_t g = 0; g < nb; ++g) {
+    uint64_t lo, hi;
+    memcpy(&lo, b + 8 * g, 8);
+    memcpy(&hi, b + 8 * g + 4, 8);
+    for (int j = 0; j < 8; ++j) d[8 * g + j] = 1.0;
+    list[k] = (uint32_t)(i0 / 8 + g);
+    memcpy(kept + 8 * k, &lo, 8);
+    memcpy(kept + 8 * k + 4, &hi, 8);
+    k += (lo | hi) != 0;
+  }
+  if (8 * nb < n) {
+    unsigned any = 0;
+    for (int j = 0; j < 8; ++j) kept[8 * k + j] = 0;
+    for (size_t i = 8 * nb; i < n; ++i) { d[i] = 1.0; any |= b[i]; kept[8 * k + (i - 8 * nb)] = b[i]; }
+    list[k] = (uint32_t)(i0 / 8 + nb);
+    k += any != 0;
+  }
+  return k;
+}
+static void* prefill_worker(void* a) {
+  struct prefill_job* j = (struct prefill_job*)a;
+  *j->count = j->n ? prefill_span(j->d, j->b, j->i0, j->n, j->list, j->kept) : 0;
+  return NULL;
+}
+int cna_host_expand_u16_prefill(double* dst, const uint16_t* bins, int64_t n, int nthreads, uint32_t* blocks, uint16_t* kept,
+                                int64_t* counts) {
+  if (!counts) return 1;
+  for (int t = 0; t < 16; ++t) counts[t] = 0;
+  if (n <= 0) return 0;
+  if (!dst || !bins || !blocks || !kept || n > ((int64_t)1 << 34)) return 1;
+  struct prefill_job jobs[16];
+  pthread_t th[16];
+  int started[16];
+  size_t part;
+  nthreads = expand_split(n, nthreads, &part);
+  for (int t = 0; t < nthreads; ++t) {
+    const size_t b = (size_t)t * part;
+    jobs[t].d = dst + b; jobs[t].b = bins + b; jobs[t].i0 = b; jobs[t].list = blocks + b / 8; jobs[t].kept = kept + b;
+    jobs[t].count = counts + t;
+    jobs[t].n = b >= (size_t)n ? 0 : ((size_t)n - b < part || t == nthreads - 1 ? (size_t)n - b : part);
+    started[t] = 0;
+  }
+  for (int t = 1; t < nthreads; ++t) started[t] = pthread_create(&th[t], NULL, prefill_worker, &jobs[t]) == 0;
+  prefill_worker(&jobs[0]);
+  for (int t = 1; t < nthreads; ++t) {
+    if (started[t]) pthread_join(th[t], NULL);
+    else prefill_worker(&jobs[t]);
+  }
+  return 0;
+}
+
+#ifndef CNA_PATCH_GRAIN
+#define CNA_PATCH_GRAIN 8192
+#endif
+struct patch_job { double* d; size_t n, part; const uint32_t* blocks; const uint16_t* kept; const int64_t* counts; int s0, s1; const double* tab; };
+static void* patch_worker(void* a) {
+  struct patch_job* j = (struct patch_job*)a;
+  for (int s = j->s0; s < j->s1; ++s) {
+    const uint32_t* list = j->blocks + (size_t)s * j->part / 8;
+    const uint16_t* kept = j->kept + (size_t)s * j->part;
+    const int64_t m = j->counts[s];
+    for (int64_t k = 0; k < m; ++k) {
+      if (k + 16 < m) __builtin_prefetch(j->d + 8 * (size_t)list[k + 16], 1, 0);
+      const size_t i0 = 8 * (size_t)list[k];
+      if (i0 + 8 <= j->n) {
+        for (int q = 0; q < 8; ++q) j->d[i0 + q] = j->tab[kept[8 * k + q] & 1023u];
+      } else {
+        for (size_t i = i0; i < j->n; ++i) j->d[i] = j->tab[kept[8 * k + (i - i0)] & 1023u];
+      }
+    }
+  }
+  return NULL;
+}
+int cna_host_expand_u16_patch(double* dst, const uint16_t* bins, int64_t n, const double* runmin, int T, int nthreads,
+                              const uint32_t* blocks, const uint16_t* kept, const int64_t* counts) {
+  if (n <= 0) return 0;
+  if (!dst || !bins || !runmin || !blocks || !kept || !counts || n > ((int64_t)1 << 34)) return 1;
+  size_t part;
+  const int spans = expand_split(n, nthreads, &part);
+  int64_t listed = 0;
+  for (int s = 0; s < spans; ++s) {
+    const size_t b = (size_t)s * part;
+    const size_t len = b >= (size_t)n ? 0 : ((size_t)n - b < part || s == spans - 1 ? (size_t)n - b : part);
+    if (counts[s] < 0 || (uint64_t)counts[s] > (len + 7) / 8) return 1;
+    listed += counts[s];
+  }
+  if (2 * listed > (n + 7) / 8) return cna_host_expand_u16(dst, bins, n, runmin, T, nthreads);
+  double t2[1024];
+  expand_table(t2, runmin, T);
+  int nt = (int)((listed + CNA_PATCH_GRAIN - 1) / CNA_PATCH_GRAIN);
+  if (nt > spans) nt = spans;
+  if (nt < 1) nt = 1;
+  struct patch_job jobs[16];
+  pthread_t th[16];
+  int started[16];
+  for (int t = 0; t < nt; ++t) {
+    jobs[t].d = dst; jobs[t].n = (size_t)n; jobs[t].part = part; jobs[t].blocks = blocks; jobs[t].kept = kept; jobs[t].counts = counts;
+    jobs[t].s0 = (int)((int64_t)spans * t / nt); jobs[t].s1 = (int)((int64_t)spans * (t + 1) / nt); jobs[t].tab = t2;
+    started[t] = 0;
+  }
+  for (int t = 1; t < nt; ++t) started[t] = pthread_create(&th[t], NULL, patch_worker, &jobs[t]) == 0;
+  patch_worker(&jobs[0]);
+  for (int t = 1; t < nt; ++t) {
+    if (started[t]) pthread_join(th[t], NULL);
+    else patch_worker(&jobs[t]);
   }
   return 0;
 }
diff --git a/cna_amd/csrc/local_null.hip b/cna_amd/csrc/local_null.hip
--- a/cna_amd/csrc/local_null.hip
+++ b/cna_amd/csrc/local_null.hip
@@ -83,11 +83,12 @@
 }
 static NullHostLayout null_host_layout(int P, int T, int want_tails) {
   NullHostLayout h;
-  h.tails = h.sums + 8 * (int64_t)T;
+  h.sums = h.status + 8;
+  h.tab = h.sums + 8 * (int64_t)T;
+  h.tails = h.tab + 8 * (int64_t)T;
   h.obs = h.tails + (want_tails ? 8 * (int64_t)P * T : 0);
   h.stage = h.obs + 16 * (int64_t)T;
-  h.status = h.stage + 24 * (int64_t)T;
-  h.bytes = h.status + 16;
+  h.bytes = h.stage + 24 * (int64_t)T;
   return h;
 }
 
@@ -178,30 +179,41 @@
   int* i8_status = nullptr;
   int64_t* sums = k.sums;
   np.i8_last = false;
+  double* tab = inline_fdr ? cc.coef_dev + 4 * c->n_pad : nullptr;
+  const bool one_rank = !(c->nranks > 1 || comm_active(c));
+  const bool table_in_pass = inline_fdr && one_rank;
   if (!np.has_tails && null_i8_eligible(c, P, T, np.cut0, np.inv_step, np.eps))
-    CNA_TRY(launch_null_local_i8(c, c->zc + col0, c->zc_ld, P, k.cuts, T, np.cut0, np.inv_step, np.eps, &sums, &i8_status));
+    CNA_TRY(launch_null_local_i8(c, c->zc + col0, c->zc_ld, P, k.cuts, T, np.cut0, np.inv_step, np.eps, &sums, &i8_status,
+                                 table_in_pass ? k.obs_tails : nullptr, table_in_pass ? tab : nullptr));
   np.i8_last = i8_status != nullptr;
   np.col0 = col0;
   np.status_off = -1;
+  bool table_sent = false;
   if (i8_status) {
-    CNA_TRY(comm_allreduce_i64_sum(c, sums, (size_t)T));
     int64_t* stw = (int64_t*)i8_status;
-    CNA_TRY(comm_allreduce_i64_sum(c, stw, 1));
     np.status_off = np.host.status;
-    HIP_TRY(hipMemcpyAsync(hr + np.host.status, stw, 8, hipMemcpyDeviceToHost, c->stream));
+    if (one_rank) {
+      HIP_TRY(hipMemcpyAsync(hr + np.host.status, stw, 8 + 8 * (size_t)T * (table_in_pass ? 2 : 1), hipMemcpyDeviceToHost, c->stream));
+      table_sent = table_in_pass;
+    } else {
+      CNA_TRY(comm_allreduce_i64_sum(c, sums, (size_t)T));
+      CNA_TRY(comm_allreduce_i64_sum(c, stw, 1));
+      HIP_TRY(hipMemcpyAsync(hr + np.host.status, stw, 8, hipMemcpyDeviceToHost, c->stream));
+      HIP_TRY(hipMemcpyAsync(hr + np.host.sums, sums, 8 * (size_t)T, hipMemcpyDeviceToHost, c->stream));
+    }
   } else {
     CNA_TRY(launch_null_local(c, c->zc + col0, c->zc_ld, P, k.cuts, T, np.cut0, np.inv_step, np.eps, k.hist, nullptr));
     if (np.has_tails) CNA_TRY(comm_allreduce_i64_sum(c, (int64_t*)k.hist, (size_t)P * T));
     CNA_TRY(launch_suffix_sum(c, k.hist, P, T, k.tails));
     CNA_TRY(launch_tail_sums(c, k.tails, P, T, sums));
     if (!np.has_tails) CNA_TRY(comm_allreduce_i64_sum(c, sums, (size_t)T));
-  }
-  HIP_TRY(hipMemcpyAsync(hr + np.host.sums, sums, 8 * (size_t)T, hipMemcpyDeviceToHost, c->stream));
+    HIP_TRY(hipMemcpyAsync(hr + np.host.sums, sums, 8 * (size_t)T, hipMemcpyDeviceToHost, c->stream));
+  }
   if (inline_fdr) {
-    double* tab = cc.coef_dev + 4 * c->n_pad;
-    CNA_TRY(launch_fdr_table(c, sums, k.obs_tails, T, P, tab, tab + 512));
-    if (!cc.h_tab) HIP_TRY(hipHostMalloc((void**)&cc.h_tab, 8 * 512, hipHostMallocDefault));
-    HIP_TRY(hipMemcpyAsync(cc.h_tab, tab + 512, 8 * (size_t)T, hipMemcpyDeviceToHost, c->stream));
+    if (!table_sent) {
+      CNA_TRY(launch_fdr_table(c, sums, k.obs_tails, T, P, tab, tab + 512));
+      HIP_TRY(hipMemcpyAsync(hr + np.host.tab, tab + 512, 8 * (size_t)T, hipMemcpyDeviceToHost, c->stream));
+    }
     cc.fdr_inline = true;
   }
   if (np.has_tails)
@@ -384,6 +396,8 @@
   return 0;
 }
 
+static const double* host_fdr_table(const cna_ctx* c) { return (const double*)((const char*)c->h_res + c->null.host.tab); }
+
 static int ensure_cell_pinned(cna_ctx* c, int64_t n_out) {
   const int64_t need = 16 * std::max<int64_t>(n_out, 1);
   if (need > c->cells.h_cell_cap) {
@@ -441,12 +455,26 @@
   if (!c->cells.coef_early || !c->cells.fdr_inline || c->null.phase != NULL_PENDING || !c->cells.h_cell || n != n_out) return 0;
   struct Flight { std::atomic<int>& f; Flight(std::atomic<int>& f_) : f(f_) { f.store(1); } ~Flight() { f.store(0); } } flight(c->cells.fdr_early_inflight);
   HIP_TRY(hipEventSynchronize(c->cells.bins_copied));
+  CellColumns& cc = c->cells;
+  const int64_t nblocks = (n + 7) / 8;
+  if (nblocks > cc.h_blocks_cap) {
+    free(cc.h_blocks);
+    free(cc.h_kept);
+    cc.h_blocks_cap = 0;
+    cc.h_blocks = (uint32_t*)malloc(4 * (size_t)nblocks);
+    cc.h_kept = (uint16_t*)malloc(16 * (size_t)nblocks);
+    if (!cc.h_blocks || !cc.h_kept) CNA_FAIL(CNA_ENOMEM, "cna_percell_fdr_copy_early: out of memory");
+    cc.h_blocks_cap = nblocks;
+  }
+  if (cna_host_expand_u16_prefill(dst, cc.h_bins, n, nthreads, cc.h_blocks, cc.h_kept, cc.h_block_counts) != 0)
+    CNA_FAIL(CNA_ESTATE, "cna_percell_fdr_copy_early: prefill failed");
   HIP_TRY(hipEventSynchronize(c->null_done));
   const int64_t status_off = c->null.status_off;
   if (status_off >= 0 && *(volatile int64_t*)((char*)c->h_res + status_off) != 0)
     return 0;
   if (!c->cells.fdr_inline) return 0;
-  if (cna_host_expand_u16(dst, c->cells.h_bins, n, c->cells.h_tab, c->null.T, nthreads) != 0)
+  if (cna_host_expand_u16_patch(dst, cc.h_bins, n, host_fdr_table(c), c->null.T, nthreads, cc.h_blocks, cc.h_kept,
+                                cc.h_block_counts) != 0)
     CNA_FAIL(CNA_ESTATE, "cna_percell_fdr_copy_early: expansion failed");
   c->cells.fdr_early_dst = dst;
   c->cells.fdr_early_copied = true;
@@ -479,7 +507,7 @@
     if (c->cells.fdr_early_copied && c->cells.fdr_early_dst) {
       *fdr_ptr = c->cells.fdr_early_dst;
     } else {
-      if (cna_host_expand_u16(hc + n_out, c->cells.h_bins, n_out, c->cells.h_tab, T, 4) != 0)
+      if (cna_host_expand_u16(hc + n_out, c->cells.h_bins, n_out, host_fdr_table(c), T, 4) != 0)
         CNA_FAIL(CNA_ESTATE, "cna_percell_fdr_pinned: expansion failed");
       *fdr_ptr = hc + n_out;
     }
diff --git a/cna_amd/csrc/null_i8.hip b/cna_amd/csrc/null_i8.hip
--- a/cna_amd/csrc/null_i8.hip
+++ b/cna_amd/csrc/null_i8.hip
@@ -365,18 +365,68 @@
   for (int i = threadIdx.x; i < TW; i += 256) partial[(size_t)blockIdx.x * TW + i] = rh[i];
 }
 
-__global__ __launch_bounds__(256) void k_i8_reduce(const unsigned int* __restrict__ partial, int nslabs, int nplain, int T,
-                                                   unsigned long long* __restrict__ hist) {
-  const int t = blockIdx.x * 4 + (threadIdx.x >> 6), lane = threadIdx.x & 63;
-  if (t >= T) return;
-  unsigned long long s = 0;
-  for (int b = lane; b < nslabs; b += 64) {
-    const unsigned v = partial[(size_t)b * (T + 1) + t + 1];
-    s += b < nplain ? (unsigned long long)v : (unsigned long long)(long long)(int)v;
-  }
-#pragma unroll
-  for (int o = 32; o > 0; o >>= 1) s += __shfl_xor(s, o);
-  if (lane == 0) hist[t] = s;
+__global__ __launch_bounds__(512) void k_i8_tail(const unsigned int* __restrict__ partial, int nslabs, int nplain, int T,
+                                                 unsigned long long* hist, unsigned int* ticket, int64_t* __restrict__ sums,
+                                                 const int64_t* __restrict__ ranks, int P, double* __restrict__ fdr,
+                                                 double* __restrict__ runmin) {
+  __shared__ long long buf[2][512];
+  const int t = blockIdx.x * 8 + (threadIdx.x >> 6), lane = threadIdx.x & 63;
+  if (t < T) {
+    unsigned long long s = 0;
+    for (int b = lane; b < nslabs; b += 64) {
+      const unsigned v = partial[(size_t)b * (T + 1) + t + 1];
+      s += b < nplain ? (unsigned long long)v : (unsigned long long)(long long)(int)v;
+    }
+#pragma unroll
+    for (int o = 32; o > 0; o >>= 1) s += __shfl_xor(s, o);
+    if (lane == 0) hist[t] = s;
+  }
+  asm volatile("s_waitcnt vmcnt(0)" ::: "memory");
+  __syncthreads();
+  if (threadIdx.x == 0) {
+    __builtin_amdgcn_fence(__ATOMIC_RELEASE, "agent");
+    asm volatile("s_waitcnt vmcnt(0)" ::: "memory");
+    const unsigned prev = __hip_atomic_fetch_add(ticket, 1u, __ATOMIC_RELAXED, __HIP_MEMORY_SCOPE_AGENT);
+    const bool last = prev == gridDim.x - 1;
+    if (last) {
+      __builtin_amdgcn_fence(__ATOMIC_ACQUIRE, "agent");
+      asm volatile("s_waitcnt vmcnt(0)" ::: "memory");
+    }
+    buf[0][0] = last ? 1 : 0;
+  }
+  __syncthreads();
+  const bool last = buf[0][0] != 0;
+  __syncthreads();
+  if (!last) return;
+  const int u = threadIdx.x;
+  int cur = 0;
+  buf[0][u] = u < T ? (long long)__hip_atomic_load(&hist[u], __ATOMIC_RELAXED, __HIP_MEMORY_SCOPE_AGENT) : 0;
+  __syncthreads();
+  for (int o = 1; o < 512; o <<= 1) {
+    buf[cur ^ 1][u] = buf[cur][u] + (u + o < 512 ? buf[cur][u + o] : 0);
+    cur ^= 1;
+    __syncthreads();
+  }
+  const long long mine = buf[cur][u];
+  if (u < T) sums[u] = mine;
+  if (!ranks) return;
+  double (*sh)[512] = reinterpret_cast<double (*)[512]>(buf);
+  double f = __builtin_nan("");
+  if (u < T) {
+    f = __ddiv_rn(__ddiv_rn((double)mine, (double)ranks[u]), (double)P);
+    if (fdr) fdr[u] = f;
+  }
+  __syncthreads();
+  cur = 0;
+  sh[0][u] = f;
+  __syncthreads();
+  for (int d = 1; d < 512; d <<= 1) {
+    const double v = u >= d ? fmin(sh[cur][u - d], sh[cur][u]) : sh[cur][u];
+    sh[cur ^ 1][u] = v;
+    cur ^= 1;
+    __syncthreads();
+  }
+  if (u < T) runmin[u] = sh[cur][u];
 }
 
 typedef int (*i8_launch_fn)(cna_ctx*, unsigned, size_t, const unsigned char*, const float2*, int64_t, const v4i*, int, int, int, int, float,
@@ -435,7 +485,9 @@
 }
 
 int launch_null_local_i8(cna_ctx* c, const double* Yc_dev, int ldy, int P, const double* cuts_dev, int T, double cut0,
-                         double inv_step, double eps, int64_t** sums_out, int** status_out) {
+                         double inv_step, double eps, int64_t** sums_out, int** status_out, const int64_t* ranks_dev,
+                         double* fdr_dev) {
+  if (T > 512) CNA_FAIL(CNA_EINVAL, "more than 512 FDR thresholds are not supported");
   const int N = c->Nx, KS = (N + 31) / 32;
   const int64_t ntiles = (c->nx + 31) / 32;
   const int nstrips = (P + 63) / 64, Ppad = nstrips * 64;
@@ -461,10 +513,10 @@
       (int64_t)8 * 32 * ntiles,
       (int64_t)16 * 3 * KS * 128 * nstages * G,
       (int64_t)8 * Ppad * ldt,
-      (int64_t)8 * Ppad + 64,
+      (int64_t)8 * (Ppad + 5 + 2 * T),
       (int64_t)8 * (int64_t)qcap,
       (int64_t)4 * nslabs * (T + 1),
-      (int64_t)8 * T, (int64_t)8 * T};
+      (int64_t)8 * T};
   int64_t need = 0;
   for (int64_t s : sizes) need += round_up64(s, 256);
   CNA_TRY(dev_reserve(c, &c->i8_buf, &c->i8_cap, need));
@@ -479,14 +531,16 @@
   double* Yt = (double*)take(3);
   unsigned long long* colL1 = (unsigned long long*)take(4);
   unsigned long long* scal = colL1 + Ppad;
-  unsigned long long* qcount = scal + 2;
-  int* status = (int*)(scal + 3);
+  unsigned int* ticket = (unsigned int*)(scal + 2);
+  unsigned long long* qcount = scal + 3;
+  int* status = (int*)(scal + 4);
+  int64_t* sums_dev = (int64_t*)(scal + 5);
+  double* runmin = (double*)(sums_dev + T);
   uint2* queue = (uint2*)take(5);
   unsigned int* slabs = (unsigned int*)take(6);
   unsigned long long* hist = (unsigned long long*)take(7);
-  int64_t* sums_dev = (int64_t*)take(8);
   ProfScope ps(c, CNA_K_NULL_LOCAL);
-  HIP_TRY(hipMemsetAsync(colL1, 0, (size_t)8 * Ppad + 64, c->stream));
+  HIP_TRY(hipMemsetAsync(colL1, 0, (size_t)8 * (Ppad + 5), c->stream));
   if (nstages * G > nstrips)
     HIP_TRY(hipMemsetAsync(Yq + (size_t)nstrips * 3 * KS * 128, 0, (size_t)16 * 3 * KS * 128 * (nstages * G - nstrips), c->stream));
   hipLaunchKernelGGL(k_y_absmax, dim3(16), dim3(1024), 0, c->stream, Yc_dev, ldy, N, P, scal);
@@ -507,9 +561,9 @@
   CNA_TRY(kI8[KS - 1](c, grid, i8_lds(KS, T), Xq, rowinfo, ntiles, Yq, nstages, nsplit, spp, T, bconst, slabs, queue, qcount, qcap, status));
   hipLaunchKernelGGL(k_null_recheck, dim3(nrecheck), dim3(256), (size_t)4 * (T + 1), c->stream, c->X, c->ldx, N, Yt, ldt, queue,
                      qcount, qcap, cuts_dev, T, cut0, inv_step, slabs + (size_t)grid * (T + 1));
-  hipLaunchKernelGGL(k_i8_reduce, dim3((unsigned)((T + 3) / 4)), dim3(256), 0, c->stream, slabs, nslabs, (int)grid, T, hist);
+  hipLaunchKernelGGL(k_i8_tail, dim3((unsigned)((T + 7) / 8)), dim3(512), 0, c->stream, slabs, nslabs, (int)grid, T, hist, ticket,
+                     sums_dev, ranks_dev, P, fdr_dev, runmin);
   HIP_TRY(hipGetLastError());
-  CNA_TRY(launch_suffix_sum(c, hist, 1, T, sums_dev));
   *sums_out = sums_dev;
   *status_out = status;
   c->i8_qcount = qcount;
diff --git a/include/cna_hip.h b/include/cna_hip.h
--- a/include/cna_hip.h
+++ b/include/cna_hip.h
@@ -218,6 +218,10 @@
 uint64_t cna_host_hash64(const void* p, int64_t nbytes, int nthreads);
 int  cna_host_copy(void* dst, const void* src, int64_t nbytes, int nthreads);
 int  cna_host_expand_u16(double* dst, const uint16_t* bins, int64_t n, const double* runmin, int T, int nthreads);
+int  cna_host_expand_u16_prefill(double* dst, const uint16_t* bins, int64_t n, int nthreads, uint32_t* blocks, uint16_t* kept,
+                                 int64_t* counts);
+int  cna_host_expand_u16_patch(double* dst, const uint16_t* bins, int64_t n, const double* runmin, int T, int nthreads,
+                               const uint32_t* blocks, const uint16_t* kept, const int64_t* counts);
 int64_t cna_host_cluster_order(int64_t n, const int64_t* indptr, const int32_t* indices, int B, int64_t* order_out);
 int64_t cna_host_cluster_order_mt(int64_t n, const int64_t* indptr, const int32_t* indices, int B, int nthreads,
                                   int64_t* order_out);
```

Result: faster. 114.1 billion, median of 6 (+1.5%).
